# cosmodesi/desilike

Hardware: AMD Instinct MI355X
Metric: log-likelihood evals/sec (full-shape P_ell, 3x40 bins) (higher is better)
Workload: dtype f64; 1 GPU; BASELINE configs[1]: ShapeFit+Kaiser P_ell ell=(0,2,4) x 40 k-bins, dense window 120x1200 (n_kin=400/ell), 120x120 precision, 1024 batched param points per GPU per step; batch_per_gpu=1024, n_params=6, parallelism=walkers x1, collective=none, ranks=1

## Files before the change

desilike_amd/csrc/dl_api.hip:

```cpp
#include <hip/hip_runtime.h>
#include <chrono>
#include <thread>

#include <algorithm>
#include <cmath>
#include <cstdio>
#include <cstdlib>
#include <string>
#include <vector>

#include "../../include/desilike_amd.h"
#include "dl_host.hpp"
#include "dl_kernels.h"
#include "dl_ens_fold.h"
#include "dl_prior.h"
#include "dl_sample_solved.h"
#include "dl_data_batch.h"

static thread_local std::string g_last_error;
void dl_set_last_error(const char* msg) { g_last_error = msg ? msg : ""; }

struct DlWhitenHost {
    int n = 0;
    std::vector<int64_t> col_ptr;
    std::vector<int> row;
    std::vector<double> val;
    std::vector<int> white_row;
    std::vector<double> bias_full;
    void apply(const double* flatdata, double* bias_white, double* bias_wh) const {
        for (int i = 0; i < n; ++i) {
            double bsum = 0., dsum = 0.;
            for (int64_t e = col_ptr[i]; e < col_ptr[i + 1]; ++e) {
                const int j = row[e];
                const double lji = val[e];
                bsum += lji * (bias_full[j] - flatdata[j]);
                dsum += lji * flatdata[j];
            }
            bias_white[white_row[i]] = bsum;
            if (bias_wh) bias_wh[white_row[i]] = -dsum;
        }
    }
};

struct dl_ctx {
    int device = 0;
    int n_params = 0, n_obs = 0, n_data = 0;
    int n_white = 0;
    int N_pad = 0, K_pad = 0, K_live = 0, max_n_t = 0;
    bool any_transform = false;
    bool priors_general = false;
    int n_solved = 0, n_var = 0;
    DlMargDev marg;
    double* tconst_dev = nullptr;
    std::vector<DlObsHost> obs;
    std::vector<int> obs_row0;
    double* arena_dev = nullptr;
    std::vector<DlObsDev> obs_kernarg;
    DlObsDev* obs_array_dev = nullptr;
    double* priors_dev = nullptr;
    int32_t* gemm_counters = nullptr;
    int32_t* step_ready = nullptr;
    double* wt_white_dev = nullptr;
    double* wt_frag_dev = nullptr;
    std::vector<uint8_t> panel_ranges;
    double* bias_white_dev = nullptr;
    double* wt_full_dev = nullptr;
    double* bias_full_dev = nullptr;
    double* wh_dev = nullptr;
    double* bias_wh_dev = nullptr;
    double* flatdata_dev = nullptr;
    int32_t* transform_dev = nullptr;
    bool feat_ok = false;
    int64_t feat_ld = 0;
    std::vector<double*> gfrag_dev;
    std::vector<int> stk_steps;
    bool any_stacked = false;
    double* feat_ws = nullptr;
    int64_t cap = 0;
    double* power_ws = nullptr;
    double* ws_scratch = nullptr;
    int64_t ws_ld = 0;
    double* delta_ws = nullptr;
    double* flat_ws = nullptr;
    double* stencil_ws = nullptr;
    int64_t stage_cap = 0;
    double* theta_stage = nullptr;
    double* out_stage = nullptr;
    int32_t* status_stage = nullptr;
    double* host_stage = nullptr;
    hipStream_t host_stream = nullptr;
    double* host_stage_dev = nullptr;
    uint64_t* host_flag = nullptr;
    uint64_t* host_flag_dev = nullptr;
    uint64_t host_seq = 0;
    hipEvent_t host_event = nullptr;
    double *grad_wtT = nullptr, *grad_zero = nullptr, *grad_delta = nullptr, *grad_y = nullptr, *grad_phys = nullptr;
    int32_t* grad_status = nullptr;
    int64_t grad_cap = 0;
    double *fa_resid = nullptr, *fa_jac = nullptr, *fa_rows = nullptr;
    int64_t fa_cap = 0, fa_slab_rows = 0;
    double *ej_basis = nullptr, *ej_u = nullptr, *ej_c = nullptr, *ej_dc = nullptr, *ej_resid = nullptr, *ej_rows = nullptr;
    int64_t ej_cap = 0;
    double *eg_gt = nullptr, *eg_u = nullptr, *eg_v = nullptr, *eg_q = nullptr, *eg_gb = nullptr;
    double* eg_wt[3] = {nullptr, nullptr, nullptr};
    int eg_ngt = 0;
    int64_t eg_cap = 0;
    double *ss_solved = nullptr, *ss_hessian = nullptr, *ss_loglike = nullptr, *ss_logprior = nullptr;
    int32_t* ss_status = nullptr;
    int64_t ss_cap = 0;
    DlWhitenHost whiten;
    int n_data_batch = 0;
    double* data_bias_dev = nullptr;
    int32_t* data_index_ws = nullptr;
    hipStream_t last_stream = nullptr;
    bool has_last_stream = false;
    hipEvent_t order_event = nullptr;
    bool profile = false;
    static const int NPOOL = 256;
    std::vector<int8_t> prof_phase_of;
    std::vector<hipEvent_t> ev;
    int64_t prof_calls = 0;
    int64_t eval_calls = 0;
    int prof_every = 1;
    bool prof_rotate = false;
    int prof_only = 0;
    std::string last_error;
};

#define DL_HIP_CHECK(ctx, call)                                                                                  \
    do {                                                                                                         \
        hipError_t err__ = (call);                                                                               \
        if (err__ != hipSuccess) {                                                                               \
            std::string msg__ = std::string(#call) + ": " + hipGetErrorString(err__);                            \
            if (ctx) (ctx)->last_error = msg__;                                                                  \
            g_last_error = msg__;                                                                                \
            return 1;                                                                                            \
        }                                                                                                        \
    } while (0)

static int dl_order_streams(dl_ctx* ctx, hipStream_t stream) {
    if (ctx->has_last_stream && ctx->last_stream != stream) {
        if (!ctx->order_event) DL_HIP_CHECK(ctx, hipEventCreateWithFlags(&ctx->order_event, hipEventDisableTiming));
// ... 289 lines not shown
        std::vector<double> tconst((size_t)std::max(ns, 1) * ctx->N_pad, 0.);
        for (int s_ = 0; s_ < ns; ++s_) {
            std::vector<double> dvec(K, 0.);
            for (auto& ob : ctx->obs) {
                const DlObsDev& od = ob.dev;
                double* dst = &dvec[od.col_offset];
                if (ob.marg_sn0 == s_ && od.theory == 4)
                    for (int idx = 0; idx < od.n_in; ++idx) dst[idx] += 1. / od.nd;
                else if (ob.marg_sn0 == s_ && od.ell0 >= 0)
                    for (int i = 0; i < od.n_kin; ++i) dst[(size_t)od.ell0 * od.n_kin + i] += 1. / od.nd;
                for (int c = 0; c < od.n_pass; ++c)
                    if (ob.marg_pass[c] == s_) dst[od.n_in + c] += 1.;
                const auto& snm = cfg->F("obs" + std::to_string(&ob - &ctx->obs[0]) + ".sn_matrix");
                for (int c = 0; c < od.n_sn; ++c)
                    if (ob.marg_sn[c] == s_)
                        for (int idx = 0; idx < od.n_in; ++idx) dst[idx] += snm[(size_t)idx * od.n_sn + c] / od.nd;
            }
            for (int i = 0; i < ctx->n_white; ++i) {
                double sum = 0.;
                const double* wrow = &wt_white[(size_t)i * ctx->K_pad];
                for (int k = 0; k < K; ++k) sum += wrow[k] * dvec[k];
                tconst[(size_t)s_ * ctx->N_pad + i] = sum;
            }
        }
        if (dl_upload(ctx, &ctx->tconst_dev, tconst)) { dl_destroy(ctx); return 1; }
        ctx->marg.tconst = ctx->tconst_dev;
    }
    if (dl_upload(ctx, &ctx->arena_dev, arena.data)) { dl_destroy(ctx); return 1; }
    for (auto& gf : gfrag_host) {
        double* dev = nullptr;
        if (dl_upload(ctx, &dev, gf)) { dl_destroy(ctx); return 1; }
        ctx->gfrag_dev.push_back(dev);
    }
    ctx->obs_kernarg.resize(ctx->n_obs);
    for (int i = 0; i < ctx->n_obs; ++i) { ctx->obs[i].rebase(ctx->arena_dev); ctx->obs_kernarg[i] = ctx->obs[i].dev; }
    if (dl_upload(ctx, &ctx->obs_array_dev, ctx->obs_kernarg)) { dl_destroy(ctx); return 1; }
    {
        size_t nbytes = (16384 / 32 + 8 + 64) * sizeof(int32_t);
        if (hipMalloc((void**)&ctx->gemm_counters, nbytes) != hipSuccess || hipMemset(ctx->gemm_counters, 0, nbytes) != hipSuccess) { dl_fail(ctx, "dl_create: counter allocation failed"); dl_destroy(ctx); return 1; }
        ctx->step_ready = ctx->gemm_counters + (16384 / 32 + 8);
    }
    {
        std::vector<double> frag((size_t)ctx->N_pad * ctx->K_pad);
        const int nks = ctx->K_pad / 4;
        for (int nt = 0; nt < ctx->N_pad / 16; ++nt)
            for (int ks = 0; ks < nks; ++ks)
                for (int lane = 0; lane < 64; ++lane)
                    frag[((size_t)nt * nks + ks) * 64 + lane] = wt_white[(size_t)(16 * nt + (lane & 15)) * ctx->K_pad + 4 * ks + (lane >> 4)];
        if (dl_upload(ctx, &ctx->wt_frag_dev, frag)) { dl_destroy(ctx); return 1; }
    }
    if (dl_upload(ctx, &ctx->priors_dev, priors) || dl_upload(ctx, &ctx->wt_white_dev, wt_white) ||
        dl_upload(ctx, &ctx->bias_white_dev, bias_white) || dl_upload(ctx, &ctx->wt_full_dev, wt_full) || dl_upload(ctx, &ctx->bias_full_dev, bias_full) ||
        dl_upload(ctx, &ctx->wh_dev, wh) || dl_upload(ctx, &ctx->bias_wh_dev, bias_wh) || dl_upload(ctx, &ctx->flatdata_dev, flatdata) ||
        dl_upload(ctx, &ctx->transform_dev, transform)) {
        dl_destroy(ctx);
        return 1;
    }
    if (hipDeviceSynchronize() != hipSuccess) { dl_fail(ctx, "dl_create: hipDeviceSynchronize failed"); dl_destroy(ctx); return 1; }
    *out = ctx;
    return 0;
}

static double* dl_stk_basis_ws(dl_ctx* ctx, int i) {
    const DlObsDev& d = ctx->obs_kernarg[i];
    if (d.eng[0].type != 2 || ctx->power_ws == nullptr) return nullptr;
    const int64_t ldk = (int64_t)d.stk.n_trunks * d.eng[0].widths[d.eng[0].n_layers];
    return ldk <= (int64_t)(1 + ctx->n_var) * ctx->K_pad ? ctx->power_ws : nullptr;
}

void dl_destroy(dl_ctx* ctx) {
    if (!ctx) return;
    (void)hipSetDevice(ctx->device);
    for (double* p : {ctx->grad_wtT, ctx->grad_zero, ctx->grad_delta, ctx->grad_y, ctx->grad_phys}) if (p) (void)hipFree(p);
    for (double* p : {ctx->fa_resid, ctx->fa_jac, ctx->fa_rows}) if (p) (void)hipFree(p);
    for (double* p : {ctx->ej_basis, ctx->ej_u, ctx->ej_c, ctx->ej_dc, ctx->ej_resid, ctx->ej_rows}) if (p) (void)hipFree(p);
    for (double* p : {ctx->eg_gt, ctx->eg_u, ctx->eg_v, ctx->eg_q, ctx->eg_gb, ctx->eg_wt[0], ctx->eg_wt[1], ctx->eg_wt[2]}) if (p) (void)hipFree(p);
    if (ctx->grad_status) (void)hipFree(ctx->grad_status);
    for (double* p : {ctx->ss_solved, ctx->ss_hessian, ctx->ss_loglike, ctx->ss_logprior}) if (p) (void)hipFree(p);
    if (ctx->ss_status) (void)hipFree(ctx->ss_status);
    if (ctx->data_bias_dev) (void)hipFree(ctx->data_bias_dev);
    if (ctx->data_index_ws) (void)hipFree(ctx->data_index_ws);
    void* ptrs[] = {ctx->arena_dev, ctx->priors_dev, ctx->wt_white_dev, ctx->wt_frag_dev, ctx->bias_white_dev, ctx->wt_full_dev, ctx->bias_full_dev, ctx->wh_dev,
                    ctx->bias_wh_dev, ctx->flatdata_dev, ctx->transform_dev, ctx->tconst_dev, ctx->power_ws, ctx->delta_ws, ctx->flat_ws, ctx->stencil_ws, ctx->theta_stage, ctx->out_stage,
                    ctx->status_stage, ctx->gemm_counters, ctx->obs_array_dev, ctx->ws_scratch};
    for (void* p : ptrs) if (p) (void)hipFree(p);
    for (double* p : ctx->gfrag_dev) if (p) (void)hipFree(p);
    for (auto& ob : ctx->obs) if (ob.tns) { dl_tns_destroy(ob.tns); ob.tns = nullptr; }
    if (ctx->feat_ws) (void)hipFree(ctx->feat_ws);
    for (hipEvent_t e : ctx->ev) if (e) (void)hipEventDestroy(e);
    if (ctx->order_event) (void)hipEventDestroy(ctx->order_event);
    if (ctx->host_stage) (void)hipHostFree(ctx->host_stage);
    if (ctx->host_flag) (void)hipHostFree(ctx->host_flag);
    if (ctx->host_event) (void)hipEventDestroy(ctx->host_event);
    if (ctx->host_stream) (void)hipStreamDestroy(ctx->host_stream);
    delete ctx;
}

static bool dl_fisher_emu_in_scope(const dl_ctx* ctx);
static int64_t dl_fisher_emu_per_pass(const dl_ctx* ctx);

int64_t dl_info(const dl_ctx* ctx, const char* key) {
    if (!ctx || !key) return -1;
    std::string k(key);
    if (k == "fisher_analytic_pass") return dl_fisher_emu_in_scope(ctx) ? dl_fisher_emu_per_pass(ctx) : -1;
    if (k == "n_params") return ctx->n_params;
    if (k == "n_data") return ctx->n_data;
    if (k == "n_obs") return ctx->n_obs;
    if (k == "n_in_total") { int64_t t = 0; for (auto& o : ctx->obs) t += o.n_cols(); return t; }
    if (k == "K_pad") return ctx->K_pad;
    if (k == "N_pad") return ctx->N_pad;
    if (k == "n_solved") return ctx->n_solved;
    if (k == "n_data_batch") return ctx->n_data_batch;
    if (k == "device") return ctx->device;
    if (k == "ws_ld") return ctx->ws_ld;
    for (int i = 0; i < ctx->n_obs; ++i) {
        if (k == "n_in_obs" + std::to_string(i)) return ctx->obs[i].dev.n_in;
        if (k == "n_out_obs" + std::to_string(i)) return ctx->obs[i].n_out;
        if (k == "n_ell_obs" + std::to_string(i)) return ctx->obs[i].dev.n_ell;
        if (k == "n_kin_obs" + std::to_string(i)) return ctx->obs[i].dev.n_kin;
        if (k == "moment_form_obs" + std::to_string(i)) return ctx->obs[i].dev.moment_form;
    }
    return -1;
}

static const int64_t DL_CHUNK = 32768;

static int dl_reserve(dl_ctx* ctx, int64_t B) {
    int64_t need = std::min<int64_t>(B, DL_CHUNK);
    if (need <= ctx->cap) return 0;
    need = std::min<int64_t>(std::max<int64_t>(need, 1024), DL_CHUNK);
    if (ctx->cap > 0) DL_HIP_CHECK(ctx, hipDeviceSynchronize());
    for (double** p : {&ctx->power_ws, &ctx->delta_ws, &ctx->flat_ws, &ctx->feat_ws, &ctx->stencil_ws, &ctx->ws_scratch}) if (*p) { (void)hipFree(*p); *p = nullptr; }
    ctx->cap = 0;
    const size_t R = 1 + ctx->n_var;
    DL_HIP_CHECK(ctx, hipMalloc((void**)&ctx->power_ws, (size_t)need * R * ctx->K_pad * sizeof(double)));
    DL_HIP_CHECK(ctx, hipMalloc((void**)&ctx->delta_ws, std::max<size_t>(2 * (size_t)need * R, (size_t)need * R + 16384 + 2048) * ctx->N_pad * sizeof(double)));
    DL_HIP_CHECK(ctx, hipMalloc((void**)&ctx->flat_ws, (size_t)need * ctx->N_pad * sizeof(double)));
    if (ctx->feat_ok) DL_HIP_CHECK(ctx, hipMalloc((void**)&ctx->feat_ws, (size_t)need * ctx->feat_ld * sizeof(double)));
    DL_HIP_CHECK(ctx, hipMalloc((void**)&ctx->stencil_ws, (size_t)need * ctx->n_params * sizeof(double)));
    if (ctx->ws_ld > 0) {
        DL_HIP_CHECK(ctx, hipMalloc((void**)&ctx->ws_scratch, (size_t)need * ctx->ws_ld * sizeof(double)));
        DL_HIP_CHECK(ctx, hipMemset(ctx->ws_scratch, 0, (size_t)need * ctx->ws_ld * sizeof(double)));
        for (int i = 0; i < ctx->n_obs; ++i) {
            if (ctx->obs[i].dev.templ != 5) continue;
            ctx->obs_kernarg[i].coef_w = ctx->ws_scratch + ctx->obs[i].ws_col;
            ctx->obs_kernarg[i].n_band = (int32_t)ctx->ws_ld;
        }
        DL_HIP_CHECK(ctx, hipMemcpy(ctx->obs_array_dev, ctx->obs_kernarg.data(), ctx->obs_kernarg.size() * sizeof(DlObsDev), hipMemcpyHostToDevice));
    }
    DL_HIP_CHECK(ctx, hipMemset(ctx->power_ws, 0, (size_t)need * R * ctx->K_pad * sizeof(double)));
    DL_HIP_CHECK(ctx, hipMemset(ctx->delta_ws, 0, std::max<size_t>(2 * (size_t)need * R, (size_t)need * R + 16384 + 2048) * ctx->N_pad * sizeof(double)));
    DL_HIP_CHECK(ctx, hipMemset(ctx->flat_ws, 0, (size_t)need * ctx->N_pad * sizeof(double)));
    if (ctx->feat_ok) DL_HIP_CHECK(ctx, hipMemset(ctx->feat_ws, 0, (size_t)need * ctx->feat_ld * sizeof(double)));
    DL_HIP_CHECK(ctx, hipMemset(ctx->stencil_ws, 0, (size_t)need * ctx->n_params * sizeof(double)));
    DL_HIP_CHECK(ctx, hipDeviceSynchronize());
    ctx->cap = need;
    return 0;
}

struct DlDataEval {
    const int32_t* index;
    double* out;
};

static int dl_eval_impl(dl_ctx* ctx, const double* theta_dev, int64_t B, double* loglike_dev, double* logprior_dev, double* flattheory_dev, int32_t* status_dev,
                        double* solved_dev, void* hip_stream, int post_mode, double* hessian_dev = nullptr, const DlDataEval* data = nullptr) {
    if (!ctx) { g_last_error = "dl_eval_batch: null context"; return 1; }
    if (B < 0 || (B > 0 && !theta_dev)) return dl_fail(ctx, "dl_eval_batch: invalid batch");
    if (B == 0) return 0;
    hipStream_t stream = (hipStream_t)hip_stream;
    dl_prof_events.start = dl_prof_events.stop = nullptr;
    DL_HIP_CHECK(ctx, hipSetDevice(ctx->device));
    if (dl_order_streams(ctx, stream)) return 1;
    if (dl_reserve(ctx, B)) return 1;
    const int n = ctx->n_data, P = ctx->n_params, R = 1 + ctx->n_var;
    for (int64_t b0 = 0; b0 < B; b0 += DL_CHUNK) {
        int64_t nb = std::min<int64_t>(DL_CHUNK, B - b0);
        const double* th = theta_dev + (size_t)b0 * P;
        bool prof = ctx->profile && b0 == 0 && (ctx->eval_calls % ctx->prof_every == ctx->prof_every / 2);
        hipEvent_t* ev = prof ? &ctx->ev[(size_t)(ctx->prof_calls % dl_ctx::NPOOL) * 6] : nullptr;
        const int64_t pc = ctx->prof_calls;
        const int only = !ctx->prof_rotate ? -1 : ctx->prof_only;
        if (prof) ctx->prof_phase_of[(size_t)(pc % dl_ctx::NPOOL)] = (int8_t)only;
        auto prof_phase = [&](int k) {
            const bool on = ev && k >= 0 && (only < 0 || only == k);
            dl_prof_events.start = on ? ev[2 * k] : nullptr;
            dl_prof_events.stop = on ? ev[2 * k + 1] : nullptr;
        };
        bool need_flat = ctx->any_transform || flattheory_dev != nullptr;
        const bool feat_path = ctx->feat_ok && !need_flat;
        const bool emu_fused_env = !dl_options().no_emu_fused;
        const bool emu_fused = emu_fused_env || ctx->any_stacked;
        const int64_t chi2_max_rows = dl_options().chi2_max_rows;
        const bool chi2_path = !data && !feat_path && !ctx->any_transform && ctx->n_solved == 0 && nb <= chi2_max_rows;
        const int xcd_local = dl_options().xcd_local;
        const bool chi2_fused_env_early = dl_options().chi2_fused;
        const bool chi2_fused_early = chi2_fused_env_early && !ctx->priors_general;
        const int xcd_block = !xcd_local ? 0 : chi2_path ? (chi2_fused_early ? 32 : dl_chi2_gemm_row_tile(nb, ctx->N_pad)) : (xcd_local > 1 && !feat_path && !ctx->any_transform && ctx->n_solved == 0 && ctx->N_pad == 128) ? 64 : 0;
        const bool step_kernel_allowed = dl_options().step_kernel;
        if (step_kernel_allowed && chi2_path && !need_flat && ctx->n_obs == 1 && !ctx->priors_general && ctx->K_pad % 128 == 0 &&
            dl_step_lds_bytes(ctx->obs_kernarg[0], nb, ctx->N_pad) != 0) {
            prof_phase(0);
            dl_launch_step(ctx->obs_kernarg[0], th, P, nb, ctx->power_ws, ctx->K_pad, ctx->wt_white_dev, ctx->K_pad, ctx->bias_white_dev, ctx->delta_ws, ctx->K_pad, ctx->K_live,
                           ctx->gemm_counters, ctx->step_ready, 8, ctx->priors_dev, loglike_dev ? loglike_dev + b0 : nullptr, logprior_dev ? logprior_dev + b0 : nullptr,
                           status_dev ? status_dev + b0 : nullptr, post_mode, stream, ctx->panel_ranges.empty() ? nullptr : ctx->panel_ranges.data());
            prof_phase(-1);
            if (prof) ctx->prof_calls++;
            continue;
        }
        prof_phase(0);
        if (!(feat_path && emu_fused))
            dl_launch_fullshape(ctx->obs_kernarg.data(), ctx->n_obs, th, P, nb, ctx->power_ws, ctx->K_pad, nullptr, 0, stream, feat_path ? ctx->feat_ws : nullptr, ctx->feat_ld,
                                xcd_block, ctx->obs_array_dev);
        prof_phase(1);
        int n_slabs = 1, cps = 0;
        int64_t slab_stride = 0;
        const double* fin_bias = nullptr;
        if (need_flat) {
            dl_launch_window_gemm(ctx->power_ws, (int64_t)R * ctx->K_pad, ctx->wt_full_dev, ctx->K_pad, ctx->bias_full_dev, ctx->flat_ws, ctx->N_pad, nb, ctx->N_pad,
                                  ctx->N_pad, ctx->K_pad, 1, stream);
            if (ctx->any_transform) dl_launch_transform(ctx->flat_ws, ctx->N_pad, ctx->flatdata_dev, ctx->transform_dev, n, nb, stream);
            if (flattheory_dev)
                DL_HIP_CHECK(ctx, hipMemcpy2DAsync(flattheory_dev + (size_t)b0 * n, (size_t)n * sizeof(double), ctx->flat_ws, (size_t)ctx->N_pad * sizeof(double),
                                                   (size_t)n * sizeof(double), (size_t)nb, hipMemcpyDeviceToDevice, stream));
        }
        bool gram_done = false, finalized_in_kernel = false, stacked_rows_done = false;
        const bool gram_epilogue = !dl_options().no_gram_epilogue;
        if (!data && feat_path && emu_fused && gram_epilogue && ctx->n_obs == 1 && ctx->N_pad == 128) {
            DlGramFinalize fin = {ctx->priors_dev, loglike_dev ? loglike_dev + b0 : nullptr, logprior_dev ? logprior_dev + b0 : nullptr, status_dev ? status_dev + b0 : nullptr,
                                  solved_dev ? solved_dev + (size_t)b0 * ctx->n_solved : nullptr, hessian_dev ? hessian_dev + (size_t)b0 * ctx->n_solved * ctx->n_solved : nullptr,
                                  post_mode, false};
            if (ctx->stk_steps[0]) {
                prof_phase(0);
                const bool chains_done = dl_launch_stk_chains(ctx->obs_kernarg[0], th, P, nb, dl_stk_basis_ws(ctx, 0), stream);
                prof_phase(1);
                dl_launch_emulated_stacked(ctx->obs_kernarg[0], th, P, nb, ctx->gfrag_dev[0], ctx->delta_ws, ctx->N_pad, ctx->N_pad, 0, ctx->stk_steps[0], stream, &fin, ctx->bias_white_dev,
                                           &ctx->marg, ctx->n_white, dl_stk_basis_ws(ctx, 0), chains_done);
                gram_done = fin.done;
                stacked_rows_done = !fin.done;
            } else gram_done = dl_launch_emulated_feature_gram(ctx->obs_kernarg[0], th, P, nb, ctx->gfrag_dev[0], ctx->bias_white_dev, ctx->marg, ctx->n_white, ctx->delta_ws, stream, &fin);
            if (gram_done) fin_bias = ctx->bias_white_dev;
            finalized_in_kernel = gram_done && fin.done;
        }
        if (feat_path && !gram_done) {
            for (int i = 0; i < ctx->n_obs; ++i) {
                if (i == 0 && stacked_rows_done) continue;
                if (ctx->stk_steps[i]) dl_launch_emulated_stacked(ctx->obs_kernarg[i], th, P, nb, ctx->gfrag_dev[i], ctx->delta_ws, ctx->N_pad, ctx->N_pad, i > 0, ctx->stk_steps[i], stream, nullptr, nullptr, nullptr, 0, dl_stk_basis_ws(ctx, i));
                else if (emu_fused) dl_launch_emulated_feature(ctx->obs_kernarg[i], th, P, nb, ctx->gfrag_dev[i], ctx->delta_ws, ctx->N_pad, ctx->N_pad, i > 0, stream);
                else dl_launch_feature_gemm(ctx->feat_ws, ctx->feat_ld, ctx->obs_kernarg[i].feat_off, ctx->obs_kernarg[i].nb_pad, R, ctx->gfrag_dev[i], ctx->delta_ws, ctx->N_pad,
                                            ctx->N_pad, nb, i > 0, stream);
            }
            fin_bias = ctx->bias_white_dev;
        }
        int cps_probe = 0;
        const bool chi2_big_allowed = !dl_options().no_chi2_big;
        const bool chi2_big = !data && !feat_path && !ctx->any_transform && ctx->n_solved == 0 && !chi2_path && ctx->K_pad % 32 == 0 && chi2_big_allowed &&
                              dl_gemm_tiled_splits(nb, ctx->N_pad, ctx->K_pad, &cps_probe) == 1;
        int part_tiles = ctx->N_pad / 16;
        const bool chi2_fused_env = dl_options().chi2_fused;
        const bool chi2_fused = chi2_fused_env && !ctx->priors_general;
        if (chi2_path) {
            if (nb > 16384) { prof_phase(-1); return dl_fail(ctx, "dl_eval_batch: DL_CHI2_GEMM_MAX above 16384 rows"); }
            dl_launch_chi2_gemm(ctx->power_ws, ctx->K_pad, ctx->wt_white_dev, ctx->K_pad, ctx->bias_white_dev, ctx->delta_ws, nb, ctx->N_pad, ctx->K_pad,
                                chi2_fused ? ctx->gemm_counters : nullptr, th, P, ctx->priors_dev, loglike_dev ? loglike_dev + b0 : nullptr,
                                logprior_dev ? logprior_dev + b0 : nullptr, status_dev ? status_dev + b0 : nullptr, post_mode, stream,
                                ctx->panel_ranges.empty() ? nullptr : ctx->panel_ranges.data(), ctx->K_live, nullptr, 0, ctx->wt_frag_dev);
        } else if (chi2_big) {
            dl_launch_window_gemm_dma_chi2(ctx->power_ws, ctx->K_pad, ctx->wt_white_dev, ctx->K_pad, ctx->bias_white_dev, ctx->delta_ws, nb, ctx->N_pad, ctx->K_pad, stream, ctx->n_white);
            part_tiles = dl_gemm_dma_chi2_parts(ctx->N_pad);
        } else if (feat_path) {
        } else if (ctx->any_transform) {
            dl_launch_window_gemm(ctx->flat_ws, ctx->N_pad, ctx->wh_dev, ctx->N_pad, ctx->bias_wh_dev, ctx->delta_ws, ctx->N_pad, nb, ctx->N_pad, ctx->N_pad, ctx->N_pad,
                                  1, stream);
        } else {
            n_slabs = dl_gemm_tiled_splits(nb * R, ctx->N_pad, ctx->K_pad, &cps);
            slab_stride = (int64_t)nb * R * ctx->N_pad;
            fin_bias = ctx->bias_white_dev;
            dl_launch_window_gemm_tiled(ctx->power_ws, ctx->K_pad, ctx->wt_white_dev, ctx->K_pad, ctx->delta_ws, slab_stride, ctx->N_pad, nb * R, ctx->N_pad, ctx->K_pad, n_slabs, cps,
                                        stream, ctx->n_white);
        }
        prof_phase(2);
        if (data)
            dl_launch_data_finalize(ctx->delta_ws, ctx->N_pad, ctx->n_white, n_slabs, slab_stride, ctx->data_bias_dev, ctx->N_pad, ctx->n_data_batch,
                                    data->index ? data->index + b0 : nullptr, th, P, ctx->priors_dev, nb, data->out + (size_t)b0 * (data->index ? 1 : ctx->n_data_batch),
                                    status_dev ? status_dev + b0 : nullptr, stream);
        else if (chi2_path && chi2_fused) {
        } else if (finalized_in_kernel) {
        } else if (chi2_path || chi2_big)
            dl_launch_finalize_part(ctx->delta_ws, part_tiles, th, P, ctx->priors_dev, nb, loglike_dev ? loglike_dev + b0 : nullptr, logprior_dev ? logprior_dev + b0 : nullptr,
                                    status_dev ? status_dev + b0 : nullptr, post_mode, stream);
        else if (ctx->n_solved > 0)
            dl_launch_finalize_marg(ctx->delta_ws, ctx->N_pad, ctx->n_white, R, n_slabs, slab_stride, fin_bias, ctx->marg, th, P, ctx->priors_dev, nb, loglike_dev ? loglike_dev + b0 : nullptr,
                                    logprior_dev ? logprior_dev + b0 : nullptr, status_dev ? status_dev + b0 : nullptr,
                                    solved_dev ? solved_dev + (size_t)b0 * ctx->n_solved : nullptr,
                                    hessian_dev ? hessian_dev + (size_t)b0 * ctx->n_solved * ctx->n_solved : nullptr, post_mode, stream, feat_path && ctx->n_obs == 1,
                                    gram_done ? ctx->delta_ws : nullptr);
        else
            dl_launch_finalize(ctx->delta_ws, ctx->N_pad, ctx->n_white, n_slabs, slab_stride, fin_bias, th, P, ctx->priors_dev, nb, loglike_dev ? loglike_dev + b0 : nullptr, logprior_dev ? logprior_dev + b0 : nullptr,
                               status_dev ? status_dev + b0 : nullptr, post_mode, stream);
        prof_phase(-1);
        if (prof) ctx->prof_calls++;
    }
    if (ctx->profile) ctx->eval_calls++;
    DL_HIP_CHECK(ctx, hipGetLastError());
    return 0;
}

int dl_eval_batch(dl_ctx* ctx, const double* theta_dev, int64_t B, double* loglike_dev, double* logprior_dev, double* flattheory_dev, int32_t* status_dev,
                  double* solved_dev, void* hip_stream) {
    return dl_eval_impl(ctx, theta_dev, B, loglike_dev, logprior_dev, flattheory_dev, status_dev, solved_dev, hip_stream, 0);
}

int dl_eval_batch_derived(dl_ctx* ctx, const double* theta_dev, int64_t B, double* loglike_dev, double* logprior_dev, int32_t* status_dev, double* solved_dev,
                          double* hessian_dev, void* hip_stream) {
    if (ctx && hessian_dev && ctx->n_solved == 0) return dl_fail(ctx, "dl_eval_batch_derived: no analytically solved parameter in this likelihood");
    return dl_eval_impl(ctx, theta_dev, B, loglike_dev, logprior_dev, nullptr, status_dev, solved_dev, hip_stream, 0, hessian_dev);
}

int dl_sample_solved(dl_ctx* ctx, const double* theta_dev, int64_t B, int64_t index0, int32_t size, uint64_t seed, double* solved_dev, double* loglike_dev,
                     double* logprior_dev, int32_t* status_dev, void* hip_stream) {
    if (!ctx) { g_last_error = "dl_sample_solved: null context"; return 1; }
    if (ctx->n_solved == 0) return 2;
    if (B < 0 || (B > 0 && !theta_dev) || index0 < 0) return dl_fail(ctx, "dl_sample_solved: invalid batch");
    if (size < 1) return dl_fail(ctx, "dl_sample_solved: size must be at least 1");
    if (B > 0 && (!solved_dev || !loglike_dev || !logprior_dev)) return dl_fail(ctx, "dl_sample_solved: null output");
    if (B == 0) return 0;
    hipStream_t stream = (hipStream_t)hip_stream;
    DL_HIP_CHECK(ctx, hipSetDevice(ctx->device));
    const int ns = ctx->n_solved, P = ctx->n_params;
    const int64_t need = std::min<int64_t>(B, DL_CHUNK);
    if (need > ctx->ss_cap) {
        if (ctx->ss_cap > 0) DL_HIP_CHECK(ctx, hipDeviceSynchronize());
        for (double** p : {&ctx->ss_solved, &ctx->ss_hessian, &ctx->ss_loglike, &ctx->ss_logprior}) if (*p) { (void)hipFree(*p); *p = nullptr; }
        if (ctx->ss_status) { (void)hipFree(ctx->ss_status); ctx->ss_status = nullptr; }
        ctx->ss_cap = 0;
        const int64_t cap = std::min<int64_t>(std::max<int64_t>(need, 1024), DL_CHUNK);
        DL_HIP_CHECK(ctx, hipMalloc((void**)&ctx->ss_solved, (size_t)cap * ns * sizeof(double)));
        DL_HIP_CHECK(ctx, hipMalloc((void**)&ctx->ss_hessian, (size_t)cap * ns * ns * sizeof(double)));
        DL_HIP_CHECK(ctx, hipMalloc((void**)&ctx->ss_loglike, (size_t)cap * sizeof(double)));
        DL_HIP_CHECK(ctx, hipMalloc((void**)&ctx->ss_logprior, (size_t)cap * sizeof(double)));
        DL_HIP_CHECK(ctx, hipMalloc((void**)&ctx->ss_status, (size_t)cap * sizeof(int32_t)));
        DL_HIP_CHECK(ctx, hipDeviceSynchronize());
        ctx->ss_cap = cap;
    }
    for (int64_t b0 = 0; b0 < B; b0 += DL_CHUNK) {
        const int64_t nb = std::min<int64_t>(DL_CHUNK, B - b0);
        if (dl_eval_impl(ctx, theta_dev + (size_t)b0 * P, nb, ctx->ss_loglike, ctx->ss_logprior, nullptr, ctx->ss_status, ctx->ss_solved, hip_stream, 0, ctx->ss_hessian))
            return 1;
        dl_launch_sample_solved(ctx->marg, ctx->ss_hessian, ctx->ss_solved, ctx->ss_loglike, ctx->ss_logprior, ctx->ss_status, nb, index0 + b0, size, seed,
                                solved_dev + (size_t)b0 * size * ns, loglike_dev + (size_t)b0 * size, logprior_dev + (size_t)b0 * size,
                                status_dev ? status_dev + b0 : nullptr, stream);
    }
    DL_HIP_CHECK(ctx, hipGetLastError());
    return 0;
}

int dl_eval_logposterior(dl_ctx* ctx, const double* theta_dev, int64_t B, double* logposterior_dev, int32_t* status_dev, void* hip_stream) {
    if (ctx && B > 0 && !logposterior_dev) return dl_fail(ctx, "dl_eval_logposterior: null output");
    return dl_eval_impl(ctx, theta_dev, B, logposterior_dev, nullptr, nullptr, status_dev, nullptr, hip_stream, 1);
}

static int dl_eval_fisher_impl(dl_ctx* ctx, const double* centers_dev, const double* steps_dev, int64_t B, const int32_t* data_index_dev, double* hessian_dev, double* gradient_dev,
                               double* offset_dev, void* hip_stream) {
    if (!ctx) { g_last_error = "dl_eval_fisher: null context"; return 1; }
    if (B < 0 || (B > 0 && (!centers_dev || !steps_dev))) return dl_fail(ctx, "dl_eval_fisher: invalid argument");
    if (ctx->n_solved > 0) return dl_fail(ctx, "dl_eval_fisher: the context has analytically solved parameters: create it with these parameters varied (the reference does the same, fisher.py:688-695)");
    const int P = ctx->n_params, n = ctx->n_data, S = 1 + 2 * P;
    if (P > 31) return dl_fail(ctx, "dl_eval_fisher: at most 31 varied parameters");
    if (dl_fisher_waves(ctx->n_white, P, nullptr, nullptr) < 1) return dl_fail(ctx, "dl_eval_fisher: too many parameters for the LDS-resident Gram product");
    if (B == 0) return 0;
    hipStream_t stream = (hipStream_t)hip_stream;
// ... 100 lines not shown
static int64_t dl_fisher_emu_per_pass(const dl_ctx* ctx) {
    const int64_t per_centre = std::max<int64_t>((int64_t)(1 + dl_emu_jac_n_xv(ctx->obs_kernarg[0])) * DL_FG_NM * ctx->N_pad, (int64_t)(1 + ctx->n_params) * ctx->N_pad);
    return std::max<int64_t>(64, std::min<int64_t>(2048, ((int64_t)16 << 20) / per_centre) / 64 * 64);
}

static int dl_eval_fisher_analytic_emu(dl_ctx* ctx, const double* centers_dev, int64_t B, double* hessian_dev, double* gradient_dev, double* offset_dev, hipStream_t stream) {
    const int P = ctx->n_params, Np = ctx->N_pad;
    const DlObsDev& o = ctx->obs_kernarg[0];
    const int64_t R = 1 + dl_emu_jac_n_xv(o), K = (int64_t)DL_FG_NM * Np;
    dl_prof_events.start = dl_prof_events.stop = nullptr;
    const int64_t per_pass = dl_fisher_emu_per_pass(ctx);
    const int64_t need = std::min<int64_t>(B, per_pass);
    if (need > ctx->ej_cap) {
        if (ctx->ej_cap > 0) DL_HIP_CHECK(ctx, hipDeviceSynchronize());
        for (double** p : {&ctx->ej_basis, &ctx->ej_u, &ctx->ej_c, &ctx->ej_dc, &ctx->ej_resid, &ctx->ej_rows}) if (*p) { (void)hipFree(*p); *p = nullptr; }
        ctx->ej_cap = 0;
        const int64_t cap = std::min<int64_t>(std::max<int64_t>((need + 63) / 64 * 64, 256), per_pass);
        DL_HIP_CHECK(ctx, hipMalloc((void**)&ctx->ej_basis, (size_t)cap * R * o.nb_pad * sizeof(double)));
        DL_HIP_CHECK(ctx, hipMalloc((void**)&ctx->ej_u, (size_t)cap * R * K * sizeof(double)));
        DL_HIP_CHECK(ctx, hipMalloc((void**)&ctx->ej_c, (size_t)cap * DL_FG_MONO_LD * sizeof(double)));
        DL_HIP_CHECK(ctx, hipMalloc((void**)&ctx->ej_dc, (size_t)cap * P * DL_FG_MONO_LD * sizeof(double)));
        DL_HIP_CHECK(ctx, hipMalloc((void**)&ctx->ej_resid, (size_t)cap * Np * sizeof(double)));
        DL_HIP_CHECK(ctx, hipMalloc((void**)&ctx->ej_rows, (size_t)cap * P * Np * sizeof(double)));
        DL_HIP_CHECK(ctx, hipDeviceSynchronize());
        ctx->ej_cap = cap;
    }
    for (int64_t b0 = 0; b0 < B; b0 += per_pass) {
        const int64_t nc = std::min<int64_t>(per_pass, B - b0);
        const double* th = centers_dev + (size_t)b0 * P;
        dl_launch_emu_jac_tangent(o, th, P, nc, ctx->ej_basis, ctx->ej_c, ctx->ej_dc, stream);
        dl_launch_emu_grad_u(ctx->ej_basis, o.nb_pad, 0, o.nb_pad, ctx->gfrag_dev[0], ctx->ej_u, Np, Np, nc * R, stream);
        dl_launch_emu_jac_rows(o, ctx->ej_u, Np, ctx->ej_c, ctx->ej_dc, ctx->bias_white_dev, P, ctx->n_white, Np, ctx->ej_resid, Np, ctx->ej_rows, Np, nc, stream);
        dl_launch_fisher_rows(ctx->ej_resid, Np, ctx->ej_rows, Np, ctx->n_white, 1, 0, P, nc, hessian_dev ? hessian_dev + (size_t)b0 * P * P : nullptr,
                              gradient_dev ? gradient_dev + (size_t)b0 * P : nullptr, offset_dev ? offset_dev + b0 : nullptr, stream);
    }
    DL_HIP_CHECK(ctx, hipGetLastError());
    return 0;
}

int dl_eval_fisher_analytic(dl_ctx* ctx, const double* centers_dev, int64_t B, double* hessian_dev, double* gradient_dev, double* offset_dev, void* hip_stream) {
    if (!ctx) { g_last_error = "dl_eval_fisher_analytic: null context"; return 1; }
    if (B < 0 || (B > 0 && !centers_dev)) return dl_fail(ctx, "dl_eval_fisher_analytic: invalid argument");
    const int P = ctx->n_params, Np = ctx->N_pad, Kp = ctx->K_pad;
    if (dl_fisher_emu_in_scope(ctx)) {
        if (B == 0) return 0;
        DL_HIP_CHECK(ctx, hipSetDevice(ctx->device));
        if (dl_order_streams(ctx, (hipStream_t)hip_stream)) return 1;
        return dl_eval_fisher_analytic_emu(ctx, centers_dev, B, hessian_dev, gradient_dev, offset_dev, (hipStream_t)hip_stream);
    }
    if (ctx->feat_ok || ctx->any_transform || ctx->n_solved != 0 || P > 31 || !dl_grad_applicable(ctx->obs_kernarg.data(), ctx->n_obs) ||
        dl_fisher_waves(ctx->n_white, P, nullptr, nullptr) < 1) return 2;
    if (B == 0) return 0;
    hipStream_t stream = (hipStream_t)hip_stream;
    dl_prof_events.start = dl_prof_events.stop = nullptr;
    DL_HIP_CHECK(ctx, hipSetDevice(ctx->device));
    if (dl_order_streams(ctx, stream)) return 1;
    const int64_t per_pass = std::max<int64_t>(64, std::min<int64_t>(2048, ((int64_t)16 << 20) / ((int64_t)(1 + P) * std::max(Kp, Np))) / 64 * 64);
    const int64_t need = std::min<int64_t>(B, per_pass);
    if (dl_reserve(ctx, need)) return 1;
    if (need > ctx->fa_cap) {
        if (ctx->fa_cap > 0) DL_HIP_CHECK(ctx, hipDeviceSynchronize());
        for (double** p : {&ctx->fa_resid, &ctx->fa_jac, &ctx->fa_rows}) if (*p) { (void)hipFree(*p); *p = nullptr; }
        ctx->fa_cap = 0;
        const int64_t cap = std::min<int64_t>(std::max<int64_t>((need + 63) / 64 * 64, 256), per_pass);
        const size_t rows = ((size_t)cap * P + 63) / 64 * 64, slab_rows = std::max<size_t>(2 * rows, rows + 16384 + 2048);
        DL_HIP_CHECK(ctx, hipMalloc((void**)&ctx->fa_resid, (size_t)cap * Np * sizeof(double)));
        DL_HIP_CHECK(ctx, hipMalloc((void**)&ctx->fa_jac, rows * Kp * sizeof(double)));
        DL_HIP_CHECK(ctx, hipMalloc((void**)&ctx->fa_rows, slab_rows * Np * sizeof(double)));
        DL_HIP_CHECK(ctx, hipMemset(ctx->fa_jac, 0, rows * Kp * sizeof(double)));
        DL_HIP_CHECK(ctx, hipDeviceSynchronize());
        ctx->fa_cap = cap;
        ctx->fa_slab_rows = (int64_t)slab_rows;
    }
    const int xcd_local = dl_options().xcd_local;
    for (int64_t b0 = 0; b0 < B; b0 += per_pass) {
        int cps = 0;
        const int64_t nr = std::min<int64_t>(per_pass, B - b0) * P;
        if ((int64_t)dl_gemm_tiled_splits(nr, Np, Kp, &cps) * nr > ctx->fa_slab_rows) return dl_fail(ctx, "dl_eval_fisher_analytic: the split-K slabs of the window product exceed their buffer");
    }
    for (int64_t b0 = 0; b0 < B; b0 += per_pass) {
        const int64_t nc = std::min<int64_t>(per_pass, B - b0), nr = nc * P;
        const double* th = centers_dev + (size_t)b0 * P;
        dl_launch_fullshape(ctx->obs_kernarg.data(), ctx->n_obs, th, P, nc, ctx->power_ws, Kp, nullptr, 0, stream, nullptr, 0, xcd_local ? dl_chi2_gemm_row_tile(nc, Np) : 0, ctx->obs_array_dev);
        dl_launch_chi2_gemm(ctx->power_ws, Kp, ctx->wt_white_dev, Kp, ctx->bias_white_dev, ctx->delta_ws, nc, Np, Kp, nullptr, th, P, ctx->priors_dev, nullptr, nullptr, nullptr, 1, stream,
                            ctx->panel_ranges.empty() ? nullptr : ctx->panel_ranges.data(), ctx->K_live, ctx->fa_resid, Np, ctx->wt_frag_dev);
        dl_launch_fullshape_jac(ctx->obs_kernarg.data(), ctx->n_obs, ctx->obs_array_dev, th, P, nc, ctx->K_live, Kp, ctx->fa_jac, Kp, stream);
        int cps = 0;
        const int n_slabs = dl_gemm_tiled_splits(nr, Np, Kp, &cps);
        const int64_t slab_stride = nr * (int64_t)Np;
        dl_launch_window_gemm_tiled(ctx->fa_jac, Kp, ctx->wt_white_dev, Kp, ctx->fa_rows, slab_stride, Np, nr, Np, Kp, n_slabs, cps, stream, ctx->n_white);
        dl_launch_fisher_rows(ctx->fa_resid, Np, ctx->fa_rows, Np, ctx->n_white, n_slabs, slab_stride, P, nc, hessian_dev ? hessian_dev + (size_t)b0 * P * P : nullptr,
                              gradient_dev ? gradient_dev + (size_t)b0 * P : nullptr, offset_dev ? offset_dev + b0 : nullptr, stream);
    }
    DL_HIP_CHECK(ctx, hipGetLastError());
    return 0;
}

static int dl_eval_logposterior_grad_emu(dl_ctx* ctx, const double* theta_dev, int64_t B, double* logposterior_dev, double* grad_dev, int32_t* status_dev, hipStream_t stream) {
    const int64_t per_pass = 2048;
    const int P = ctx->n_params, Np = ctx->N_pad;
    const DlObsDev& o = ctx->obs_kernarg[0];
    dl_prof_events.start = dl_prof_events.stop = nullptr;
    const int64_t K = (int64_t)DL_FG_NM * Np;
    if (!ctx->eg_gt) {
        const int Kp = ctx->K_pad, ngt = (o.n_basis + 127) / 128 * 128;
        std::vector<double> w((size_t)Np * Kp), gt((size_t)ngt * K, 0.);
        DL_HIP_CHECK(ctx, hipMemcpy(w.data(), ctx->wt_white_dev, w.size() * sizeof(double), hipMemcpyDeviceToHost));
        for (int h = 0; h < o.n_basis; ++h)
            for (int m = 0; m < DL_FG_NM; ++m)
                for (int j = 0; j < Np; ++j) gt[(size_t)h * K + (size_t)m * Np + j] = w[(size_t)j * Kp + o.col_offset + (size_t)h * DL_N_MONO + m];
        DL_HIP_CHECK(ctx, hipMalloc((void**)&ctx->eg_gt, gt.size() * sizeof(double)));
        DL_HIP_CHECK(ctx, hipMemcpy(ctx->eg_gt, gt.data(), gt.size() * sizeof(double), hipMemcpyHostToDevice));
        ctx->eg_ngt = ngt;
        for (int ie = 0; ie < 3; ++ie) {
            const DlObsDev::Engine& e = o.eng[ie];
            if (e.type != 0) continue;
            size_t n = 0, nt = 0;
            for (int l = 0; l < e.n_layers; ++l) { n += (size_t)e.widths[l] * e.widths[l + 1] + e.widths[l + 1]; nt += (size_t)e.widths[l] * e.widths[l + 1]; }
            std::vector<double> wh(n), wt(nt);
            DL_HIP_CHECK(ctx, hipMemcpy(wh.data(), e.weights, n * sizeof(double), hipMemcpyDeviceToHost));
            size_t off = 0, offt = 0;
            for (int l = 0; l < e.n_layers; ++l) {
                const int nin = e.widths[l], nout = e.widths[l + 1];
                for (int i = 0; i < nin; ++i)
                    for (int q = 0; q < nout; ++q) wt[offt + (size_t)q * nin + i] = wh[off + (size_t)i * nout + q];
                off += (size_t)nin * nout + nout;
                offt += (size_t)nin * nout;
            }
            DL_HIP_CHECK(ctx, hipMalloc((void**)&ctx->eg_wt[ie], nt * sizeof(double)));
            DL_HIP_CHECK(ctx, hipMemcpy(ctx->eg_wt[ie], wt.data(), nt * sizeof(double), hipMemcpyHostToDevice));
        }
    }
    const int64_t need = std::min<int64_t>(B, per_pass);
    if (dl_reserve(ctx, need)) return 1;
    if (need > ctx->eg_cap || !ctx->grad_status) {
        DL_HIP_CHECK(ctx, hipDeviceSynchronize());
        for (double** p : {&ctx->eg_u, &ctx->eg_v, &ctx->eg_q, &ctx->eg_gb}) if (*p) { (void)hipFree(*p); *p = nullptr; }
        if (ctx->grad_status) { (void)hipFree(ctx->grad_status); ctx->grad_status = nullptr; }
        ctx->eg_cap = 0;
        ctx->grad_cap = 0;
        const int64_t cap = std::max<int64_t>((need + 63) / 64 * 64, 256);
        DL_HIP_CHECK(ctx, hipMalloc((void**)&ctx->eg_u, (size_t)cap * K * sizeof(double)));
        DL_HIP_CHECK(ctx, hipMalloc((void**)&ctx->eg_v, (size_t)cap * K * sizeof(double)));
        DL_HIP_CHECK(ctx, hipMalloc((void**)&ctx->eg_q, (size_t)cap * (1 + ctx->n_var) * DL_N_MONO * sizeof(double)));
        DL_HIP_CHECK(ctx, hipMalloc((void**)&ctx->eg_gb, std::max<size_t>(2 * (size_t)cap, (size_t)cap + 16384 + 2048) * ctx->eg_ngt * sizeof(double)));
        DL_HIP_CHECK(ctx, hipMalloc((void**)&ctx->grad_status, (size_t)cap * sizeof(int32_t)));
        DL_HIP_CHECK(ctx, hipMemset(ctx->eg_v, 0, (size_t)cap * K * sizeof(double)));
        DL_HIP_CHECK(ctx, hipDeviceSynchronize());
        ctx->eg_cap = cap;
    }
    for (int64_t b0 = 0; b0 < B; b0 += per_pass) {
        const int64_t nb = std::min<int64_t>(per_pass, B - b0);
        const double* th = theta_dev + (size_t)b0 * P;
        int32_t* st = status_dev ? status_dev + b0 : ctx->grad_status;
        dl_launch_fullshape(ctx->obs_kernarg.data(), 1, th, P, nb, ctx->power_ws, ctx->K_pad, nullptr, 0, stream, ctx->feat_ws, ctx->feat_ld, 0, nullptr);
        dl_launch_emu_grad_u(ctx->feat_ws, ctx->feat_ld, o.feat_off, o.nb_pad, ctx->gfrag_dev[0], ctx->eg_u, Np, Np, nb, stream);
        dl_launch_emu_grad_adjoint(ctx->feat_ws, ctx->feat_ld, o.feat_off, o.nb_pad, ctx->n_var, ctx->eg_u, Np, Np, ctx->bias_white_dev, ctx->marg, th, P, ctx->priors_dev,
                                   logposterior_dev + b0, st, ctx->eg_v, ctx->eg_q, nb, stream);
        int cps = 0;
        const int n_slabs = dl_gemm_tiled_splits(nb, ctx->eg_ngt, (int)K, &cps);
        const int64_t slab_stride = nb * (int64_t)ctx->eg_ngt;
        dl_launch_window_gemm_tiled(ctx->eg_v, K, ctx->eg_gt, K, ctx->eg_gb, slab_stride, ctx->eg_ngt, nb, ctx->eg_ngt, (int)K, n_slabs, cps, stream, 0);
        dl_launch_emu_grad_backprop(o, th, P, ctx->priors_dev, ctx->eg_gb, ctx->eg_ngt, n_slabs, slab_stride, ctx->eg_q, st, ctx->eg_wt, grad_dev + (size_t)b0 * P, nb, stream);
    }
    DL_HIP_CHECK(ctx, hipGetLastError());
    return 0;
}

int dl_eval_logposterior_grad(dl_ctx* ctx, const double* theta_dev, int64_t B, double* logposterior_dev, double* grad_dev, int32_t* status_dev, void* hip_stream) {
    if (!ctx) { g_last_error = "dl_eval_logposterior_grad: null context"; return 1; }
    if (B < 0 || (B > 0 && (!theta_dev || !logposterior_dev || !grad_dev))) return dl_fail(ctx, "dl_eval_logposterior_grad: invalid argument");
    const bool emu = ctx->feat_ok && !ctx->any_transform && !ctx->priors_general && ctx->n_obs == 1 && !ctx->any_stacked &&
                     dl_emu_grad_applicable(ctx->obs_kernarg[0], ctx->N_pad, ctx->n_solved);
    if (emu) {
        if (B == 0) return 0;
        DL_HIP_CHECK(ctx, hipSetDevice(ctx->device));
        if (dl_order_streams(ctx, (hipStream_t)hip_stream)) return 1;
        return dl_eval_logposterior_grad_emu(ctx, theta_dev, B, logposterior_dev, grad_dev, status_dev, (hipStream_t)hip_stream);
    }
    if (ctx->feat_ok || ctx->any_transform || ctx->n_solved != 0 || ctx->priors_general || !dl_grad_applicable(ctx->obs_kernarg.data(), ctx->n_obs)) return 2;
    if (B == 0) return 0;
    hipStream_t stream = (hipStream_t)hip_stream;
    dl_prof_events.start = dl_prof_events.stop = nullptr;
    DL_HIP_CHECK(ctx, hipSetDevice(ctx->device));
    if (dl_order_streams(ctx, stream)) return 1;
    const int64_t per_pass = 2048;
    if (dl_reserve(ctx, std::min<int64_t>(B, per_pass))) return 1;
    const int P = ctx->n_params, Np = ctx->N_pad, Kp = ctx->K_pad;
    if (!ctx->grad_wtT) {
        std::vector<double> w((size_t)Np * Kp), wt((size_t)Kp * Np);
        DL_HIP_CHECK(ctx, hipMemcpy(w.data(), ctx->wt_white_dev, w.size() * sizeof(double), hipMemcpyDeviceToHost));
        for (int j = 0; j < Np; ++j) for (int k = 0; k < Kp; ++k) wt[(size_t)k * Np + j] = -w[(size_t)j * Kp + k];
        DL_HIP_CHECK(ctx, hipMalloc((void**)&ctx->grad_wtT, wt.size() * sizeof(double)));
        DL_HIP_CHECK(ctx, hipMemcpy(ctx->grad_wtT, wt.data(), wt.size() * sizeof(double), hipMemcpyHostToDevice));
        DL_HIP_CHECK(ctx, hipDeviceSynchronize());
    }
    const int64_t need = std::min<int64_t>(B, per_pass);
    if (need > ctx->grad_cap) {
        if (ctx->grad_cap > 0) DL_HIP_CHECK(ctx, hipDeviceSynchronize());
        for (double** p : {&ctx->grad_delta, &ctx->grad_y, &ctx->grad_phys}) if (*p) { (void)hipFree(*p); *p = nullptr; }
        if (ctx->grad_status) { (void)hipFree(ctx->grad_status); ctx->grad_status = nullptr; }
        ctx->grad_cap = 0;
        const int64_t cap = std::max<int64_t>((need + 63) / 64 * 64, 256);
        DL_HIP_CHECK(ctx, hipMalloc((void**)&ctx->grad_delta, (size_t)cap * Np * sizeof(double)));
        DL_HIP_CHECK(ctx, hipMalloc((void**)&ctx->grad_y, (size_t)cap * Kp * sizeof(double)));
        DL_HIP_CHECK(ctx, hipMalloc((void**)&ctx->grad_phys, (size_t)cap * ctx->n_obs * 8 * sizeof(double)));
        DL_HIP_CHECK(ctx, hipMalloc((void**)&ctx->grad_status, (size_t)cap * sizeof(int32_t)));
        DL_HIP_CHECK(ctx, hipMemset(ctx->grad_delta, 0, (size_t)cap * Np * sizeof(double)));
        DL_HIP_CHECK(ctx, hipDeviceSynchronize());
        ctx->grad_cap = cap;
    }
    const int xcd_local = dl_options().xcd_local;
    for (int64_t b0 = 0; b0 < B; b0 += per_pass) {
        const int64_t nb = std::min<int64_t>(per_pass, B - b0);
        const double* th = theta_dev + (size_t)b0 * P;
        int32_t* st = status_dev ? status_dev + b0 : ctx->grad_status;
        dl_launch_fullshape(ctx->obs_kernarg.data(), ctx->n_obs, th, P, nb, ctx->power_ws, ctx->K_pad, nullptr, 0, stream, nullptr, 0, xcd_local ? dl_chi2_gemm_row_tile(nb, Np) : 0, ctx->obs_array_dev,
                            false);
        dl_launch_chi2_gemm(ctx->power_ws, Kp, ctx->wt_white_dev, Kp, ctx->bias_white_dev, ctx->delta_ws, nb, Np, Kp, nullptr, th, P, ctx->priors_dev, nullptr, nullptr, nullptr, 1, stream,
                            ctx->panel_ranges.empty() ? nullptr : ctx->panel_ranges.data(), ctx->K_live, ctx->grad_delta, Np, ctx->wt_frag_dev);
        dl_launch_finalize_part(ctx->delta_ws, Np / 16, th, P, ctx->priors_dev, nb, logposterior_dev + b0, nullptr, st, 1, stream);
        dl_launch_window_gemm_tiled(ctx->grad_delta, Np, ctx->grad_wtT, Np, ctx->grad_y, 0, Kp, nb, Kp, Np, 1, Np / 16, stream, 0);
        dl_launch_fullshape_grad(ctx->obs_kernarg.data(), ctx->n_obs, ctx->obs_array_dev, th, P, nb, ctx->grad_y, Kp, ctx->grad_phys, ctx->priors_dev, st, grad_dev + (size_t)b0 * P, stream);
    }
    DL_HIP_CHECK(ctx, hipGetLastError());
    return 0;
}

int dl_eval_theory(dl_ctx* ctx, const double* theta_dev, int64_t B, int32_t iobs, double* power_dev, double* tables_dev, void* hip_stream) {
    if (!ctx) { g_last_error = "dl_eval_theory: null context"; return 1; }
    if (iobs < 0 || iobs >= ctx->n_obs) return dl_fail(ctx, "dl_eval_theory: observable index out of range");
    if (B < 0 || (B > 0 && (!theta_dev || !power_dev))) return dl_fail(ctx, "dl_eval_theory: invalid argument");
    if (B == 0) return 0;
    hipStream_t stream = (hipStream_t)hip_stream;
    DL_HIP_CHECK(ctx, hipSetDevice(ctx->device));
    const bool ws = ctx->obs_kernarg[iobs].templ == 5;
    if (ws && dl_reserve(ctx, B)) return 1;
    DlObsDev tmp = ctx->obs_kernarg[iobs];
    tmp.col_offset = 0;
    tmp.n_pass = 0;
    tmp.n_var = 0;
    for (int c = 0; c < DL_N_VPARS; ++c) tmp.vp_slot[c] = -1;
    for (int c = 0; c < DL_MAX_EFT; ++c) tmp.marg_ct_slot[c][0] = tmp.marg_ct_slot[c][1] = -1;
    if (dl_order_streams(ctx, stream)) return 1;
    for (int64_t b0 = 0, step = ws ? ctx->cap : B; b0 < B; b0 += step)
        dl_launch_fullshape(&tmp, 1, theta_dev + (size_t)b0 * ctx->n_params, ctx->n_params, std::min(step, B - b0), power_dev + (size_t)b0 * tmp.n_in, tmp.n_in,
                            tables_dev ? tables_dev + (size_t)b0 * 3 * tmp.n_in : nullptr, 3 * (int64_t)tmp.n_in, stream);
    DL_HIP_CHECK(ctx, hipGetLastError());
    return 0;
}

int dl_eval_tns_tables(dl_ctx* ctx, const double* theta_dev, int64_t B, int32_t iobs, double* tables_dev, void* hip_stream) {
    if (!ctx) { g_last_error = "dl_eval_tns_tables: null context"; return 1; }
    if (iobs < 0 || iobs >= ctx->n_obs) return dl_fail(ctx, "dl_eval_tns_tables: observable index out of range");
    if (ctx->obs[iobs].dev.theory != 4) return dl_fail(ctx, "dl_eval_tns_tables: the observable's theory is not the TNS model");
    if (B < 0 || (B > 0 && (!theta_dev || !tables_dev))) return dl_fail(ctx, "dl_eval_tns_tables: invalid argument");
    if (B == 0) return 0;
    hipStream_t stream = (hipStream_t)hip_stream;
    DL_HIP_CHECK(ctx, hipSetDevice(ctx->device));
    if (dl_order_streams(ctx, stream)) return 1;
    if (dl_tns_tables(ctx->obs_kernarg[iobs], theta_dev, ctx->n_params, B, tables_dev, stream)) return dl_fail(ctx, std::string("dl_eval_tns_tables: ") + dl_last_error(nullptr));
    DL_HIP_CHECK(ctx, hipGetLastError());
    return 0;
}

static int dl_stage_reserve(dl_ctx* ctx, int64_t B) {
    if (!ctx->host_stream) DL_HIP_CHECK(ctx, hipStreamCreateWithFlags(&ctx->host_stream, hipStreamNonBlocking));
    if (B <= ctx->stage_cap) return 0;
    for (void* p : {(void*)ctx->theta_stage, (void*)ctx->out_stage}) if (p) (void)hipFree(p);
    if (ctx->host_stage) (void)hipHostFree(ctx->host_stage);
    ctx->theta_stage = ctx->out_stage = ctx->host_stage = nullptr; ctx->status_stage = nullptr; ctx->stage_cap = 0;
    int64_t cap = std::max<int64_t>(B, 64);
    DL_HIP_CHECK(ctx, hipMalloc((void**)&ctx->theta_stage, (size_t)cap * ctx->n_params * sizeof(double)));
    DL_HIP_CHECK(ctx, hipMalloc((void**)&ctx->out_stage, (size_t)cap * 3 * sizeof(double)));
    DL_HIP_CHECK(ctx, hipHostMalloc((void**)&ctx->host_stage, (size_t)cap * (ctx->n_params + 3) * sizeof(double), hipHostMallocMapped));
    DL_HIP_CHECK(ctx, hipHostGetDevicePointer((void**)&ctx->host_stage_dev, ctx->host_stage, 0));
    if (!ctx->host_flag) {
        DL_HIP_CHECK(ctx, hipHostMalloc((void**)&ctx->host_flag, 64, hipHostMallocMapped));
        DL_HIP_CHECK(ctx, hipHostGetDevicePointer((void**)&ctx->host_flag_dev, ctx->host_flag, 0));
        *ctx->host_flag = 0;
        DL_HIP_CHECK(ctx, hipEventCreateWithFlags(&ctx->host_event, hipEventDisableTiming));
    }
    ctx->stage_cap = cap;
    return 0;
}

__global__ void dl_host_flag_kernel(uint64_t* flag, uint64_t seq) {
    __threadfence_system();
    __hip_atomic_store(flag, seq, __ATOMIC_RELEASE, __HIP_MEMORY_SCOPE_SYSTEM);
}

static int dl_host_mode() { return dl_options().host_mode >= 0 ? dl_options().host_mode : 3; }

static int dl_eval_host_impl(dl_ctx* ctx, const double* theta, int64_t B, double* loglike, double* logprior, double* flattheory, int32_t* status, double* solved,
                             double* logposterior) {
    DL_HIP_CHECK(ctx, hipSetDevice(ctx->device));
    if (dl_stage_reserve(ctx, B)) return 1;
    hipStream_t stream = ctx->host_stream;
    const int P = ctx->n_params;
    int mode = dl_host_mode();
    if (mode == 3 && ctx->host_seq && (ctx->host_seq & 7) == 0) (void)hipStreamQuery(stream);
    double *flat_dev = nullptr, *solved_dev = nullptr;
// ... 114 lines not shown
int dl_profile_enable(dl_ctx* ctx, int enable) {
    if (!ctx) { g_last_error = "dl_profile_enable: null context"; return 1; }
    DL_HIP_CHECK(ctx, hipSetDevice(ctx->device));
    if ((enable & 0xffff) && ctx->ev.empty()) {
        ctx->ev.assign((size_t)dl_ctx::NPOOL * 6, nullptr);
        for (auto& e : ctx->ev) DL_HIP_CHECK(ctx, hipEventCreate(&e));
    }
    ctx->prof_phase_of.assign(dl_ctx::NPOOL, -1);
    ctx->prof_rotate = (enable & (1 << 16)) != 0;
    ctx->prof_only = (enable >> 17) & 3;
    if (ctx->prof_only > 2) ctx->prof_only = 0;
    enable &= 0xffff;
    ctx->profile = enable != 0;
    ctx->prof_every = enable > 1 ? enable : 1;
    ctx->prof_calls = 0;
    ctx->eval_calls = 0;
    return 0;
}

int dl_profile_read(dl_ctx* ctx, double* ms, int32_t n) {
    if (!ctx || !ms || n < 4) return dl_fail(ctx, "dl_profile_read: need room for 4 values");
    if (ctx->ev.empty() || ctx->prof_calls == 0) return dl_fail(ctx, "dl_profile_read: no profiled call recorded");
    int64_t ncalls = std::min<int64_t>(ctx->prof_calls, dl_ctx::NPOOL);
    std::vector<double> samples[4];
    for (int64_t c = 0; c < ncalls; ++c) {
        hipEvent_t* ev = &ctx->ev[(size_t)c * 6];
        const int only = ctx->prof_phase_of.empty() ? -1 : ctx->prof_phase_of[(size_t)c];
        int first = -1, last = -1;
        for (int k = 0; k < 3; ++k) {
            if (only >= 0 && only != k) continue;
            (void)hipEventSynchronize(ev[2 * k + 1]);
            float t = 0;
            if (hipEventElapsedTime(&t, ev[2 * k], ev[2 * k + 1]) != hipSuccess) { (void)hipGetLastError(); continue; }
            if (first < 0) first = k;
            last = k;
            samples[k].push_back(t);
        }
        float t = 0;
        if (only < 0 && first >= 0 && hipEventElapsedTime(&t, ev[2 * first], ev[2 * last + 1]) == hipSuccess) samples[3].push_back(t);
        else (void)hipGetLastError();
    }
    for (int i = 0; i < 4; ++i) if (samples[i].empty()) samples[i].push_back(0.);
    if (n >= 9) for (int i = 0; i < 3; ++i) ms[6 + i] = (samples[i].size() == 1 && samples[i][0] == 0.) ? 0. : (double)samples[i].size();
    for (int i = 0; i < 4; ++i) {
        std::sort(samples[i].begin(), samples[i].end());
        const size_t m = samples[i].size();
        ms[i] = (m & 1) ? samples[i][m / 2] : 0.5 * (samples[i][m / 2 - 1] + samples[i][m / 2]);
    }
    if (n >= 5) ms[4] = 0.;
    if (n >= 6) ms[5] = (double)ncalls;
    return 0;
}

}

static bool dl_fold_applicable(const dl_ctx* ctx, int64_t B) {
    const int64_t chi2_max_rows = dl_options().chi2_max_rows;
    if (ctx->feat_ok || ctx->any_transform || ctx->n_solved != 0 || B > chi2_max_rows || B > DL_CHUNK || ctx->n_params > 32) return false;
    for (auto& ob : ctx->obs) {
        const DlObsDev& oh = ob.dev;
        const bool generic = !oh.uniform_knots || !(oh.toeplitz || oh.fixed_spline);
        if (oh.theory >= 2 || generic || oh.n_ct > 0 || oh.n_sn > 0 || (oh.n_ell <= 3) != (ctx->obs[0].dev.n_ell <= 3)) return false;
    }
    return ctx->n_obs >= 1 && ctx->n_obs <= 8;
}

int dl_internal_fold_info(dl_ctx* ctx, int64_t B, int* n_tiles, const double** priors) {
    if (!ctx || !n_tiles || !priors || B <= 0) return 1;
    if (!dl_fold_applicable(ctx, B)) return 2;
    *n_tiles = ctx->N_pad / 16;
    *priors = ctx->priors_dev;
    return 0;
}

int dl_internal_eval_fold(dl_ctx* ctx, const DlEnsFold& fold, int64_t B, double* part_out, hipStream_t stream) {
    if (!ctx || !part_out || B <= 0) return 1;
    if (!dl_fold_applicable(ctx, B)) return 2;
    dl_prof_events.start = dl_prof_events.stop = nullptr;
    DL_HIP_CHECK(ctx, hipSetDevice(ctx->device));
    if (dl_order_streams(ctx, stream)) return 1;
    if (dl_reserve(ctx, B)) return 1;
    const int xcd_local = dl_options().xcd_local;
    if (!dl_launch_fullshape_ens(ctx->obs_kernarg.data(), ctx->n_obs, ctx->obs_array_dev, fold, B, ctx->power_ws, ctx->K_pad, xcd_local ? dl_chi2_gemm_row_tile(B, ctx->N_pad) : 0, stream)) return 2;
    dl_launch_chi2_gemm(ctx->power_ws, ctx->K_pad, ctx->wt_white_dev, ctx->K_pad, ctx->bias_white_dev, part_out, B, ctx->N_pad, ctx->K_pad, nullptr, nullptr, ctx->n_params,
                        ctx->priors_dev, nullptr, nullptr, nullptr, 1, stream, ctx->panel_ranges.empty() ? nullptr : ctx->panel_ranges.data(), ctx->K_live, nullptr, 0, ctx->wt_frag_dev);
    DL_HIP_CHECK(ctx, hipGetLastError());
    return 0;
}

int dl_internal_eval_partials(dl_ctx* ctx, const double* theta_dev, int64_t B, const double** part, int* n_tiles, const double** priors, hipStream_t stream) {
    if (!ctx || !theta_dev || !part || !n_tiles || !priors || B <= 0) return 1;
    const int64_t chi2_max_rows = dl_options().chi2_max_rows;
    if (ctx->feat_ok || ctx->any_transform || ctx->n_solved != 0 || B > chi2_max_rows || B > DL_CHUNK) return 2;
    for (auto& ob : ctx->obs) if (ob.dev.theory == 3) return 2;
    dl_prof_events.start = dl_prof_events.stop = nullptr;
    DL_HIP_CHECK(ctx, hipSetDevice(ctx->device));
    if (dl_order_streams(ctx, stream)) return 1;
    if (dl_reserve(ctx, B)) return 1;
    const int xcd_local = dl_options().xcd_local;
    dl_launch_fullshape(ctx->obs_kernarg.data(), ctx->n_obs, theta_dev, ctx->n_params, B, ctx->power_ws, ctx->K_pad, nullptr, 0, stream, nullptr, 0, xcd_local ? dl_chi2_gemm_row_tile(B, ctx->N_pad) : 0, ctx->obs_array_dev);
    dl_launch_chi2_gemm(ctx->power_ws, ctx->K_pad, ctx->wt_white_dev, ctx->K_pad, ctx->bias_white_dev, ctx->delta_ws, B, ctx->N_pad, ctx->K_pad, nullptr, theta_dev, ctx->n_params,
                        ctx->priors_dev, nullptr, nullptr, nullptr, 1, stream, ctx->panel_ranges.empty() ? nullptr : ctx->panel_ranges.data(), ctx->K_live, nullptr, 0, ctx->wt_frag_dev);
    *part = ctx->delta_ws;
    *n_tiles = ctx->N_pad / 16;
    *priors = ctx->priors_dev;
    DL_HIP_CHECK(ctx, hipGetLastError());
    return 0;
}
```

desilike_amd/csrc/dl_chi2_gemm.h:

```cpp
#pragma once
#include "dl_scalar_prefetch.h"
#include <hip/hip_runtime.h>
#include <stdint.h>

typedef double dl_cg_double2 __attribute__((ext_vector_type(2)));
typedef double dl_cg_double4 __attribute__((ext_vector_type(4)));

#define DL_CG_M 32
#define DL_CG_N 16
#define DL_CG_KP 128
#define DL_CG_LD (DL_CG_KP + 2)
#define DL_CG_ROWS (DL_CG_M + DL_CG_N)
#ifndef DL_CG_WAVES
#define DL_CG_WAVES 16
#endif
#define DL_CG_VPT (DL_CG_ROWS / DL_CG_WAVES)
#define DL_CG_NBUF 3
#define DL_CG_LDS_BYTES (DL_CG_NBUF * DL_CG_ROWS * DL_CG_LD * 8)

struct DlChi2Fin {
    int32_t* counters;
    const double* theta;
    const double* priors;
    double* loglike;
    double* logprior;
    int32_t* status;
    int32_t n_params, post_mode;
    unsigned long long* stamps;
    int32_t* ready;
};

#define DL_CG_MAX_TILES 32
struct DlChi2Panels {
    uint32_t range[DL_CG_MAX_TILES];
};

#define DL_CG_STAMP(slot, fn) if (fin.stamps != nullptr && tid == 0) fin.stamps[(size_t)blockIdx.x * 8 + (slot)] = fn();
template <int MT, bool RESID>
__device__ __forceinline__ void dl_chi2_gemm_finish(dl_cg_double4 acc0, dl_cg_double4 acc1, double bj, double* __restrict__ part, int M, int n_tiles, const DlChi2Fin& fin,
                                                    double* __restrict__ resid, int64_t ldr, double* lds, int mb, int nt, double fin_lp, int fin_nan) {
    const int tid = threadIdx.x, lane = tid & 63, wave = __builtin_amdgcn_readfirstlane(tid >> 6);
    const int r16 = lane & 15, g = lane >> 4;
    constexpr int MTILES = MT / 16;
    const int m0 = mb * MT, n0 = nt * DL_CG_N;
    DL_CG_STAMP(2, __builtin_amdgcn_s_memtime)
    __syncthreads();
    double* red = lds;
#pragma unroll
    for (int r = 0; r < 4; ++r) { red[((wave * 2 + 0) * 4 + r) * 64 + lane] = acc0[r]; if (MTILES > 1) red[((wave * 2 + 1) * 4 + r) * 64 + lane] = acc1[r]; }
    __syncthreads();
    if (wave < 4 * MTILES) {
        const int t = wave % MTILES, r = wave / MTILES;
        double v = bj;
#pragma unroll
        for (int w = 0; w < DL_CG_WAVES; ++w) v += red[((w * 2 + t) * 4 + r) * 64 + lane];
        if (RESID) { const int rrow = m0 + 16 * t + g + 4 * r; if (rrow < M) resid[(size_t)rrow * ldr + n0 + r16] = v; }
        double sq = v * v;
        sq += __shfl_xor(sq, 1, 64);
        sq += __shfl_xor(sq, 2, 64);
        sq += __shfl_xor(sq, 4, 64);
        sq += __shfl_xor(sq, 8, 64);
        const int row = m0 + 16 * t + g + 4 * r;
        if (r16 == 0 && row < M) __hip_atomic_store(part + (size_t)row * n_tiles + nt, sq, __ATOMIC_RELAXED, __HIP_MEMORY_SCOPE_AGENT);
    }
    DL_CG_STAMP(3, __builtin_amdgcn_s_memtime) DL_CG_STAMP(4, __builtin_amdgcn_s_memtime) DL_CG_STAMP(5, __builtin_amdgcn_s_memtime) DL_CG_STAMP(7, __builtin_amdgcn_s_memrealtime)
    if (fin.counters == nullptr) return;
    __asm__ volatile("s_waitcnt vmcnt(0)" : : : "memory");
    __syncthreads();
    if (wave != 0) return;
    int done = 0;
    if (lane == 0) done = __hip_atomic_fetch_add(fin.counters + mb, 1, __ATOMIC_RELAXED, __HIP_MEMORY_SCOPE_AGENT);
    done = __builtin_amdgcn_readfirstlane(done);
    if (done != n_tiles - 1) return;
    if (lane == 0) __hip_atomic_store(fin.counters + mb, 0, __ATOMIC_RELAXED, __HIP_MEMORY_SCOPE_AGENT);
    if (lane == 0 && fin.ready != nullptr) __hip_atomic_store(fin.ready + mb, 0, __ATOMIC_RELAXED, __HIP_MEMORY_SCOPE_AGENT);
    const int row = m0 + lane;
    if (lane < MT && row < M) {
        double chi2 = 0.;
        for (int t = 0; t < n_tiles; ++t) chi2 += __hip_atomic_load(part + (size_t)row * n_tiles + t, __ATOMIC_RELAXED, __HIP_MEMORY_SCOPE_AGENT);
        const double inf = __builtin_huge_val();
        const double lp = fin_lp, ll = -0.5 * chi2;
        int st = 0;
        if (fin_nan) st = 3;
        else if (lp == -inf) st = 1;
        else if (!(ll == ll) || ll == inf || ll == -inf) st = 2;
        if (fin.loglike) fin.loglike[row] = fin.post_mode ? (st == 0 ? ll + lp : -inf) : ll;
        if (fin.logprior) fin.logprior[row] = lp;
        if (fin.status) fin.status[row] = st;
    }
}

template <bool DO_LOAD, bool DO_MMA, int MT, bool RESID, class Wait>
__device__ __forceinline__ void dl_chi2_gemm_tile(const double* __restrict__ A, int64_t lda, const double* __restrict__ Wt, int64_t ldw, const double* __restrict__ bias,
                                                  double* __restrict__ part, int M, int K_pad, int n_tiles, const DlChi2Fin& fin, const DlChi2Panels& panels, int k_live,
                                                  double* __restrict__ resid, int64_t ldr, double* lds, int mb, int nt, Wait&& wait) {
    const int tid = threadIdx.x, lane = tid & 63, wave = __builtin_amdgcn_readfirstlane(tid >> 6);
    const int r16 = lane & 15, g = lane >> 4;
    constexpr int ROWS = MT + DL_CG_N, VPT = ROWS / DL_CG_WAVES, MTILES = MT / 16;
    const int m0 = mb * MT, n0 = nt * DL_CG_N;
    if (m0 >= M) return;
    DL_CG_STAMP(0, __builtin_amdgcn_s_memtime) DL_CG_STAMP(6, __builtin_amdgcn_s_memrealtime)
    int p_lo = 0, p_hi = K_pad / DL_CG_KP;
    const uint32_t range = panels.range[nt < DL_CG_MAX_TILES ? nt : 0];
    if (nt < DL_CG_MAX_TILES && (range >> 8) != 0) { p_lo = (int)(range & 0xffu); p_hi = (int)(range >> 8); }
    const char* src[VPT];
#pragma unroll
    for (int i = 0; i < VPT; ++i) {
        int row = wave + DL_CG_WAVES * i;
        const double* base;
        if (row < MT) { int ar = m0 + row; if (ar > M - 1) ar = M - 1; base = A + (size_t)ar * lda; }
        else base = Wt + (size_t)(n0 + row - MT) * ldw;
        src[i] = reinterpret_cast<const char*>(base) + 16 * lane + (size_t)p_lo * (DL_CG_KP * 8);
    }
    const double bj = bias[n0 + r16];
    const int n_panels = p_hi - p_lo;
    constexpr int BUF = ROWS * DL_CG_LD, NJ = DL_CG_KP / 4 / DL_CG_WAVES;
#define DL_CG_DMA(p)                                                                                                                 \
    {   const size_t off = (size_t)(p) * (DL_CG_KP * 8);                                                                             \
        double* dst = lds + ((p) % DL_CG_NBUF) * BUF + wave * DL_CG_LD;                                                              \
        _Pragma("unroll") for (int i = 0; i < VPT; ++i)                                                                               \
            __builtin_amdgcn_global_load_lds((const __attribute__((address_space(1))) void*)(src[i] + off),                          \
                                             (__attribute__((address_space(3))) void*)(dst + DL_CG_WAVES * i * DL_CG_LD), 16, 0, 0); }
    dl_cg_double4 acc0 = {0., 0., 0., 0.}, acc1 = {0., 0., 0., 0.};
    const double* la = lds + r16 * DL_CG_LD + g;
    wait();
    if (DO_LOAD) { DL_CG_DMA(0) if (n_panels > 1) { DL_CG_DMA(1) } }
    double fin_lp = 0.;
    int fin_nan = 0;
    if (fin.counters != nullptr && wave == 0 && lane < MT && m0 + lane < M) {
        const double inf = __builtin_huge_val();
        for (int p = 0; p < fin.n_params; ++p) {
            double x = fin.theta[(size_t)(m0 + lane) * fin.n_params + p];
            const double* pr = fin.priors + 5 * p;
            if (x != x) fin_nan = 1;
            bool isin = (pr[1] <= x) && (x <= pr[2]);
            double v = 0.;
            if (pr[0] == 1.) { double t = x - pr[3]; v = -0.5 * (t * t) / (pr[4] * pr[4]); }
            fin_lp += isin ? v : -inf;
        }
    }
    if (n_panels > 1) __asm__ volatile("s_waitcnt vmcnt(%0)" : : "n"(VPT) : "memory");
    else __asm__ volatile("s_waitcnt vmcnt(0)" : : : "memory");
    __builtin_amdgcn_s_barrier();
    DL_CG_STAMP(1, __builtin_amdgcn_s_memtime)
#define DL_CG_MULTIPLY(p)                                                                                                            \
    {   const double* lb = la + ((p) % DL_CG_NBUF) * BUF;                                                                            \
        double a0[NJ], a1[NJ], bb[NJ];                                                                                               \
        _Pragma("unroll") for (int j = 0; j < NJ; ++j) {                                                                             \
            const int ks = wave + DL_CG_WAVES * j; a0[j] = lb[4 * ks]; a1[j] = MTILES > 1 ? lb[16 * DL_CG_LD + 4 * ks] : 0.; bb[j] = lb[MT * DL_CG_LD + 4 * ks]; } \
        if (DO_MMA) { _Pragma("unroll") for (int j = 0; j < NJ; ++j) {                                                               \
            acc0 = __builtin_amdgcn_mfma_f64_16x16x4f64(a0[j], bb[j], acc0, 0, 0, 0);                                                \
            if (MTILES > 1) acc1 = __builtin_amdgcn_mfma_f64_16x16x4f64(a1[j], bb[j], acc1, 0, 0, 0); } } }
#define DL_CG_MULTIPLY_LIM(p, lim)                                                                                                   \
    {   const double* lb = la + ((p) % DL_CG_NBUF) * BUF;                                                                            \
        _Pragma("unroll") for (int j = 0; j < NJ; ++j) {                                                                             \
            const int ks = wave + DL_CG_WAVES * j;                                                                                   \
            if (DO_MMA && ks < (lim)) {                                                                                              \
                const double a0 = lb[4 * ks], a1 = MTILES > 1 ? lb[16 * DL_CG_LD + 4 * ks] : 0., bb = lb[MT * DL_CG_LD + 4 * ks];    \
                acc0 = __builtin_amdgcn_mfma_f64_16x16x4f64(a0, bb, acc0, 0, 0, 0);                                                  \
                if (MTILES > 1) acc1 = __builtin_amdgcn_mfma_f64_16x16x4f64(a1, bb, acc1, 0, 0, 0); } } }
    int p = 0;
    for (; p + 2 < n_panels; ++p) {
        if (DO_LOAD) { DL_CG_DMA(p + 2) }
        DL_CG_MULTIPLY(p)
        __asm__ volatile("s_waitcnt vmcnt(%0) lgkmcnt(0)" : : "n"(VPT) : "memory");
        __builtin_amdgcn_s_barrier();
    }
    if (p + 1 < n_panels) {
        DL_CG_MULTIPLY(p)
        __asm__ volatile("s_waitcnt vmcnt(0) lgkmcnt(0)" : : : "memory");
        __builtin_amdgcn_s_barrier();
        ++p;
    }
    {
        int lim = (k_live - (p_lo + p) * DL_CG_KP + 3) / 4;
        lim = lim < 0 ? 0 : (lim > DL_CG_KP / 4 ? DL_CG_KP / 4 : lim);
        DL_CG_MULTIPLY_LIM(p, lim)
    }
#undef DL_CG_MULTIPLY
#undef DL_CG_MULTIPLY_LIM
#undef DL_CG_DMA
    dl_chi2_gemm_finish<MT, RESID>(acc0, acc1, bj, part, M, n_tiles, fin, resid, ldr, lds, mb, nt, fin_lp, fin_nan);
}

#define DL_CG_PMAX 12
template <bool DO_LOAD, bool DO_MMA, int MT, bool RESID>
__device__ __forceinline__ void dl_chi2_gemm_tile_bf(const double* __restrict__ A, int64_t lda, const double* __restrict__ wfrag, const double* __restrict__ bias,
                                                     double* __restrict__ part, int M, int K_pad, int n_tiles, const DlChi2Fin& fin, const DlChi2Panels& panels, int k_live,
                                                     double* __restrict__ resid, int64_t ldr, double* lds, int mb, int nt) {
    const int tid = threadIdx.x, lane = tid & 63, wave = __builtin_amdgcn_readfirstlane(tid >> 6);
    const int r16 = lane & 15, g = lane >> 4;
    constexpr int VPT = MT / DL_CG_WAVES, MTILES = MT / 16;
    static_assert(VPT >= 1 && DL_CG_KP / 4 / DL_CG_WAVES == 2, "16 waves: one or two row pieces and two k-steps per wave and panel");
    const int m0 = mb * MT, n0 = nt * DL_CG_N;
    if (m0 >= M) return;
    DL_CG_STAMP(0, __builtin_amdgcn_s_memtime) DL_CG_STAMP(6, __builtin_amdgcn_s_memrealtime)
    int p_lo = 0, p_hi = K_pad / DL_CG_KP;
    const uint32_t range = panels.range[nt < DL_CG_MAX_TILES ? nt : 0];
    if (nt < DL_CG_MAX_TILES && (range >> 8) != 0) { p_lo = (int)(range & 0xffu); p_hi = (int)(range >> 8); }
    const int n_panels = p_hi - p_lo;
    const double* bsrc = wfrag + ((size_t)nt * (K_pad / 4) + (size_t)p_lo * (DL_CG_KP / 4) + wave) * 64 + lane;
    double bq[DL_CG_PMAX][2];
#pragma unroll
    for (int q = 0; q < DL_CG_PMAX; ++q) {
        const double* bp = bsrc + (size_t)(q < n_panels ? q : n_panels - 1) * (DL_CG_KP / 4 * 64);
        bq[q][0] = bp[0]; bq[q][1] = bp[DL_CG_WAVES * 64];
    }
    const char* src[VPT];
#pragma unroll
    for (int i = 0; i < VPT; ++i) {
        int ar = m0 + wave + DL_CG_WAVES * i; if (ar > M - 1) ar = M - 1;
        src[i] = reinterpret_cast<const char*>(A + (size_t)ar * lda) + 16 * lane + (size_t)p_lo * (DL_CG_KP * 8);
    }
    const double bj = bias[n0 + r16];
    constexpr int BUF = MT * DL_CG_LD;
#define DL_CG_DMA_A(p)                                                                                                               \
    {   const size_t off = (size_t)(p) * (DL_CG_KP * 8);                                                                             \
        double* dst = lds + ((p) % DL_CG_NBUF) * BUF + wave * DL_CG_LD;                                                              \
        _Pragma("unroll") for (int i = 0; i < VPT; ++i)                                                                               \
            __builtin_amdgcn_global_load_lds((const __attribute__((address_space(1))) void*)(src[i] + off),                          \
                                             (__attribute__((address_space(3))) void*)(dst + DL_CG_WAVES * i * DL_CG_LD), 16, 0, 0); }
    dl_cg_double4 acc0 = {0., 0., 0., 0.}, acc1 = {0., 0., 0., 0.};
    const double* la = lds + r16 * DL_CG_LD + g;
    if (DO_LOAD) { DL_CG_DMA_A(0) if (n_panels > 1) { DL_CG_DMA_A(1) } }
    double fin_lp = 0.;
    int fin_nan = 0;
    if (fin.counters != nullptr && wave == 0 && lane < MT && m0 + lane < M) {
        const double inf = __builtin_huge_val();
        for (int p = 0; p < fin.n_params; ++p) {
            double x = fin.theta[(size_t)(m0 + lane) * fin.n_params + p];
            const double* pr = fin.priors + 5 * p;
            if (x != x) fin_nan = 1;
            bool isin = (pr[1] <= x) && (x <= pr[2]);
            double v = 0.;
            if (pr[0] == 1.) { double t = x - pr[3]; v = -0.5 * (t * t) / (pr[4] * pr[4]); }
            fin_lp += isin ? v : -inf;
        }
    }
    if (n_panels > 1) __asm__ volatile("s_waitcnt vmcnt(%0)" : : "n"(VPT) : "memory");
    else __asm__ volatile("s_waitcnt vmcnt(0)" : : : "memory");
    __builtin_amdgcn_s_barrier();
    DL_CG_STAMP(1, __builtin_amdgcn_s_memtime)
    int lim = (k_live - (p_lo + n_panels - 1) * DL_CG_KP + 3) / 4;
    lim = lim < 0 ? 0 : (lim > DL_CG_KP / 4 ? DL_CG_KP / 4 : lim);
#pragma unroll
    for (int p = 0; p < DL_CG_PMAX; ++p) {
        if (p < n_panels) {
        if (DO_LOAD && p + 2 < n_panels) { DL_CG_DMA_A(p + 2) }
        const double* lb = la + (p % DL_CG_NBUF) * BUF;
        const int klim = p + 1 < n_panels ? DL_CG_KP / 4 : lim;
#pragma unroll
        for (int j = 0; j < 2; ++j) {
            const int ks = wave + DL_CG_WAVES * j;
            if (DO_MMA && ks < klim) {
                const double a0 = lb[4 * ks], a1 = MTILES > 1 ? lb[16 * DL_CG_LD + 4 * ks] : 0.;
                acc0 = __builtin_amdgcn_mfma_f64_16x16x4f64(a0, bq[p][j], acc0, 0, 0, 0);
                if (MTILES > 1) acc1 = __builtin_amdgcn_mfma_f64_16x16x4f64(a1, bq[p][j], acc1, 0, 0, 0);
            }
        }
        if (p + 1 < n_panels) {
            if (p + 2 < n_panels) __asm__ volatile("s_waitcnt vmcnt(%0) lgkmcnt(0)" : : "n"(VPT) : "memory");
            else __asm__ volatile("s_waitcnt vmcnt(0) lgkmcnt(0)" : : : "memory");
            __builtin_amdgcn_s_barrier();
        }
        }
    }
#undef DL_CG_DMA_A
    dl_chi2_gemm_finish<MT, RESID>(acc0, acc1, bj, part, M, n_tiles, fin, resid, ldr, lds, mb, nt, fin_lp, fin_nan);
}

template <bool DO_LOAD, bool DO_MMA, int MT = DL_CG_M, bool RESID = false>
__global__ __launch_bounds__(64 * DL_CG_WAVES) void dl_chi2_gemm_bf_kernel(const double* __restrict__ A, int64_t lda, const double* __restrict__ wfrag, const double* __restrict__ bias,
                                                              double* __restrict__ part, int M, int K_pad, int n_tiles, DlChi2Fin fin, DlChi2Panels panels, int k_live,
                                                              double* __restrict__ resid, int64_t ldr) {
    extern __shared__ __attribute__((aligned(16))) double lds[];
    dl_kernarg_prefetch<256>();
    const int L = blockIdx.x;
    const int xcd = L & 7, rest = L >> 3;
    const int nt = rest % n_tiles, mb = xcd + 8 * (rest / n_tiles);
    dl_chi2_gemm_tile_bf<DO_LOAD, DO_MMA, MT, RESID>(A, lda, wfrag, bias, part, M, K_pad, n_tiles, fin, panels, k_live, resid, ldr, lds, mb, nt);
}

template <bool DO_LOAD, bool DO_MMA, int MT = DL_CG_M, bool RESID = false>
__global__ __launch_bounds__(64 * DL_CG_WAVES) void dl_chi2_gemm_kernel(const double* __restrict__ A, int64_t lda, const double* __restrict__ Wt, int64_t ldw,
                                                           const double* __restrict__ bias, double* __restrict__ part, int M, int K_pad, int n_tiles, DlChi2Fin fin,
                                                           DlChi2Panels panels, int k_live, double* __restrict__ resid, int64_t ldr) {
    extern __shared__ __attribute__((aligned(16))) double lds[];
    dl_kernarg_prefetch<256>();
    const int L = blockIdx.x;
    const int xcd = L & 7, rest = L >> 3;
    const int nt = rest % n_tiles, mb = xcd + 8 * (rest / n_tiles);
    dl_chi2_gemm_tile<DO_LOAD, DO_MMA, MT, RESID>(A, lda, Wt, ldw, bias, part, M, K_pad, n_tiles, fin, panels, k_live, resid, ldr, lds, mb, nt, []() {});
}
```

desilike_amd/csrc/dl_kernels.h:

```cpp
#pragma once
#include <hip/hip_runtime.h>
#include <hip/hip_ext.h>
#include <stdint.h>

#include "dl_fullshape.h"

struct DlProfEvents { hipEvent_t start = nullptr, stop = nullptr; };
extern thread_local DlProfEvents dl_prof_events;
#define DL_LAUNCH(kernel, grid, block, shm, stream, ...)                                                                                       \
    do {                                                                                                                                       \
        if (dl_prof_events.start) hipExtLaunchKernelGGL(kernel, grid, block, shm, stream, dl_prof_events.start, dl_prof_events.stop, 0, __VA_ARGS__); \
        else hipLaunchKernelGGL(kernel, grid, block, shm, stream, __VA_ARGS__);                                                                \
    } while (0)

struct DlOptions {
    bool no_merged_theory, no_emu_batch, no_fused_solve, no_gram_plain, no_scaled_row0, ef_no_early_theta, fm_no_lane_solve;
    bool chi2_bfrag;
    bool no_stk_split;
    int stk_overlap;
    bool ens_global, ens_force_comm, ens_no_defer, ens_no_fold, ens_stamps, ens_fold_stamps;
    bool no_emu_fused, no_gram_epilogue, step_kernel, chi2_fused, no_chi2_big;
    bool fs_no_moments;
    bool fs_mu_prio;
    int xcd_local;
    long long chi2_max_rows;
    int cg_mt;
    int host_mode;
};
const DlOptions& dl_options();

#define DL_ST_OK 0
#define DL_ST_OUT_OF_PRIOR 1
#define DL_ST_NONFINITE 2
#define DL_ST_NAN_INPUT 3

void dl_launch_fullshape(const DlObsDev* obs_host, int n_obs, const double* theta, int n_params, int64_t B, double* power, int64_t ld_power, double* tables,
                         int64_t ld_tables, hipStream_t stream, double* feat = nullptr, int64_t feat_ld = 0, int xcd_block = 0,
                         const DlObsDev* obs_dev = nullptr,
                         bool moments = true);
void dl_launch_window_gemm(const double* A, int64_t lda, const double* Wt, int64_t ldw, const double* bias, double* C, int64_t ldc, int64_t M, int N_valid, int N_pad,
                           int K_pad, int bias_period, hipStream_t stream);

#define DL_MARG_NJ 8
struct DlMargDev {
    int32_t n_s, n_marg;
    int32_t is_marg[DL_MAX_SOLVED];
    int32_t var_slot[DL_MAX_SOLVED];
    double x0[DL_MAX_SOLVED], loc[DL_MAX_SOLVED], prec[DL_MAX_SOLVED];
    const double* tconst;
};
void dl_launch_finalize_marg(const double* dtilde, int64_t ld, int n, int rows_per_point, int n_slabs, int64_t slab_stride, const double* bias, const DlMargDev& mg,
                             const double* theta, int n_params, const double* priors, int64_t B, double* loglike, double* logprior, int32_t* status, double* solved,
                             double* hessian , int post_mode, hipStream_t stream, bool xcd_tile16 = false,
                             const double* gram = nullptr);
void dl_launch_transform(double* flat, int64_t ld, const double* data, const int32_t* transform, int n, int64_t B, hipStream_t stream);
int dl_gemm_tiled_splits(int64_t M, int N_pad, int K_pad, int* chunks_per_split);
void dl_launch_window_gemm_tiled(const double* A, int64_t lda, const double* Wt, int64_t ldw, double* slabs, int64_t slab_stride, int64_t ldc, int64_t M, int N_pad, int K_pad,
                                 int n_splits, int chunks_per_split, hipStream_t stream, int n_live = 0);
void dl_launch_finalize(const double* dtilde, int64_t ld, int n, int n_slabs, int64_t slab_stride, const double* bias, const double* theta, int n_params,
                        const double* priors, int64_t B, double* loglike, double* logprior, int32_t* status, int post_mode, hipStream_t stream);
int dl_chi2_gemm_row_tile(int64_t M, int N_pad);
void dl_launch_chi2_gemm(const double* A, int64_t lda, const double* Wt, int64_t ldw, const double* bias, double* part, int64_t M, int N_pad, int K_pad, int32_t* counters,
                         const double* theta, int n_params, const double* priors, double* loglike, double* logprior, int32_t* status, int post_mode, hipStream_t stream,
                         const uint8_t* panel_ranges = nullptr, int k_live = 0, double* resid = nullptr, int64_t ldr = 0, const double* wfrag = nullptr);
void dl_launch_finalize_part(const double* part, int n_tiles, const double* theta, int n_params, const double* priors, int64_t B, double* loglike, double* logprior,
                             int32_t* status, int post_mode, hipStream_t stream);
#ifndef DL_FG_NM
#define DL_FG_NM 19
#define DL_FG_MONO_LD 20
#endif
void dl_launch_feature_gemm(const double* feat, int64_t feat_ld, int64_t feat_off, int nb_pad, int R, const double* gfrag, double* out, int64_t ldo, int N_pad, int64_t B,
                            int accumulate, hipStream_t stream);
int dl_gemm_dma_chi2_parts(int N_pad);
void dl_launch_window_gemm_dma_chi2(const double* A, int64_t lda, const double* Wt, int64_t ldw, const double* bias, double* part, int64_t M, int N_pad, int K_pad, hipStream_t stream, int n_live = 0);
void dl_launch_emulated_feature(const DlObsDev& obs, const double* theta, int n_params, int64_t B, const double* gfrag, double* out, int64_t ldo, int N_pad, int accumulate,
                                hipStream_t stream);
size_t dl_step_lds_bytes(const DlObsDev& obs, int64_t B, int N_pad);
void dl_launch_step(const DlObsDev& obs, const double* theta, int n_params, int64_t B, double* power, int64_t ld_power, const double* Wt, int64_t ldw, const double* bias,
                    double* part, int K_pad, int k_live, int32_t* counters, int32_t* ready, int32_t target, const double* priors, double* loglike, double* logprior, int32_t* status,
                    int post_mode, hipStream_t stream, const uint8_t* panel_ranges);
bool dl_emulated_stacked_ok(const DlObsDev& obs);
struct DlGramFinalize;
void dl_launch_emulated_stacked(const DlObsDev& obs, const double* theta, int n_params, int64_t B, const double* gfrag, double* out, int64_t ldo, int N_pad, int accumulate,
                                int steps_per_block, hipStream_t stream, DlGramFinalize* fin = nullptr, const double* bias = nullptr, const DlMargDev* mg = nullptr, int n_valid = 0,
                                double* basis_ws = nullptr, bool chains_done = false);
bool dl_launch_stk_chains(const DlObsDev& obs, const double* theta, int n_params, int64_t B, double* basis_ws, hipStream_t stream);
struct DlGramFinalize {
    const double* priors;
    double *loglike, *logprior;
    int32_t* status;
    double *solved, *hessian;
    int post_mode;
    bool done;
};
bool dl_launch_emulated_feature_gram(const DlObsDev& obs, const double* theta, int n_params, int64_t B, const double* gfrag, const double* bias, const DlMargDev& mg, int n_valid,
                                     double* gram, hipStream_t stream, DlGramFinalize* fin = nullptr);
void dl_launch_fisher_stencil(const double* centers, const double* steps, int P, int64_t B, double* theta, hipStream_t stream);
int dl_fisher_waves(int n, int P, size_t* shm_bytes, int* chunk);
void dl_launch_fisher(const double* rows, int64_t ld, int n, int n_slabs, int64_t slab_stride, const double* bias, const double* steps, int P, int64_t B, double* hessian,
                      double* gradient, double* offset, hipStream_t stream,
                      const int32_t* data_index = nullptr, int64_t ldb = 0);
struct dl_ctx;
int dl_internal_eval_partials(dl_ctx* ctx, const double* theta_dev, int64_t B, const double** part, int* n_tiles, const double** priors, hipStream_t stream);
struct DlEnsFold;
int dl_internal_fold_info(dl_ctx* ctx, int64_t B, int* n_tiles, const double** priors);
int dl_internal_eval_fold(dl_ctx* ctx, const DlEnsFold& fold, int64_t B, double* part_out, hipStream_t stream);
bool dl_launch_fullshape_ens(const DlObsDev* obs_host, int n_obs, const DlObsDev* obs_dev, const DlEnsFold& f, int64_t B, double* power, int64_t ld_power, int xcd_block, hipStream_t stream);
bool dl_grad_applicable(const DlObsDev* obs_host, int n_obs);
void dl_launch_fullshape_grad(const DlObsDev* obs_host, int n_obs, const DlObsDev* obs_dev, const double* theta, int n_params, int64_t B, const double* Y, int64_t ldy, double* gphys,
                              const double* priors, const int32_t* status, double* grad, hipStream_t stream);
void dl_launch_fullshape_jac(const DlObsDev* obs_host, int n_obs, const DlObsDev* obs_dev, const double* theta, int n_params, int64_t B, int k_live, int k_pad, double* jac, int64_t ldj,
                             hipStream_t stream);
void dl_launch_fisher_rows(const double* resid, int64_t ldr, const double* drows, int64_t ld, int n, int n_slabs, int64_t slab_stride, int P, int64_t B, double* hessian,
                           double* gradient, double* offset, hipStream_t stream);
bool dl_emu_grad_applicable(const DlObsDev& obs, int N_pad, int n_solved);
void dl_launch_emu_grad_u(const double* feat, int64_t feat_ld, int64_t feat_off, int nb_pad, const double* gfrag, double* U, int64_t ldu, int N_pad, int64_t B, hipStream_t stream);
void dl_launch_emu_grad_adjoint(const double* feat, int64_t feat_ld, int64_t feat_off, int nb_pad, int n_var, const double* U, int64_t ldu, int N_pad, const double* bias,
                                const DlMargDev& mg, const double* theta, int n_params, const double* priors, double* logpost, int32_t* status, double* V, double* Q,
                                int64_t B, hipStream_t stream);
void dl_launch_emu_grad_backprop(const DlObsDev& obs, const double* theta, int n_params, const double* priors, const double* gb, int64_t ldg, int n_slabs, int64_t slab_stride,
                                 const double* Q, const int32_t* status, const double* const* wT , double* grad, int64_t B,
                                 hipStream_t stream);
bool dl_emu_jac_applicable(const DlObsDev& obs, int N_pad, int n_params);
int dl_emu_jac_n_xv(const DlObsDev& obs);
void dl_launch_emu_jac_tangent(const DlObsDev& obs, const double* theta, int n_params, int64_t B, double* basis_rows, double* cmono, double* dmono, hipStream_t stream);
void dl_launch_emu_jac_rows(const DlObsDev& obs, const double* U, int64_t ldu, const double* cmono, const double* dmono, const double* bias, int n_params, int n_live, int N_pad,
                            double* resid, int64_t ldr, double* rows, int64_t ld, int64_t B, hipStream_t stream);
void dl_set_last_error(const char* msg);
```

desilike_amd/csrc/dl_kernels.hip:

```cpp
#include <hip/hip_runtime.h>

#include <algorithm>
#include <cstdio>
#include <cstdlib>
#include <cstring>
#include <vector>

#include "dl_fullshape.h"
#include "dl_wigglesplit.h"
#include <mutex>
#include "dl_kernels.h"
#include "dl_tns.h"
#include "dl_emu_batch.h"
#include "dl_emu_stacked.h"
#include "dl_emu_stacked_ov.h"
#include "dl_emu_stacked_split.h"
#include "dl_finalize_part.h"
#include "dl_marg_solve.h"
#include "dl_scalar_prefetch.h"
#include "dl_ens_fold.h"
#include "dl_fullshape_grad.h"
#include "dl_fullshape_jac.h"

thread_local DlProfEvents dl_prof_events;

__device__ __forceinline__ void dl_obs_prefetch(const void* p) {
    if (__builtin_amdgcn_readfirstlane(threadIdx.x) >= 64) return;
    dl_scalar_prefetch<0, (offsetof(DlObsDev, ct_in) + 63) / 64 * 64, offsetof(DlObsDev, coef_w) / 64 * 64, (sizeof(DlObsDev) + 63) / 64 * 64>(p);
}

static DlOptions g_options;
static std::once_flag g_options_once;
static void dl_options_read() {
    auto on = [](const char* name) { return std::getenv(name) != nullptr; };
    DlOptions& o = g_options;
    o.no_merged_theory = on("DL_NO_MERGED_THEORY"); o.no_emu_batch = on("DL_NO_EMU_BATCH"); o.no_fused_solve = on("DL_NO_FUSED_SOLVE"); o.no_gram_plain = on("DL_NO_GRAM_PLAIN");
    o.no_scaled_row0 = on("DL_NO_SCALED_ROW0"); o.ef_no_early_theta = on("DL_EF_NO_EARLY_THETA"); o.fm_no_lane_solve = on("DL_FM_NO_LANE_SOLVE");
    o.no_stk_split = on("DL_NO_STK_SPLIT");
    o.stk_overlap = std::getenv("DL_STK_OVERLAP") ? atoi(std::getenv("DL_STK_OVERLAP")) : 0;
    o.ens_global = on("DL_ENS_GLOBAL"); o.ens_force_comm = on("DL_ENS_FORCE_COMM"); o.ens_no_defer = on("DL_ENS_NO_DEFER"); o.ens_no_fold = on("DL_ENS_NO_FOLD");
    o.ens_stamps = on("DL_ENS_STAMPS"); o.ens_fold_stamps = on("DL_ENS_FOLD_STAMPS");
    o.cg_mt = std::getenv("DL_CG_MT") ? atoi(std::getenv("DL_CG_MT")) : 0;
    o.host_mode = std::getenv("DL_HOST_MODE") ? atoi(std::getenv("DL_HOST_MODE")) : -1;
    auto flag = [](const char* name) { const char* v = std::getenv(name); return v != nullptr && atoi(v) != 0; };
    o.no_emu_fused = on("DL_NO_EMU_FUSED"); o.no_gram_epilogue = on("DL_NO_GRAM_EPILOGUE"); o.no_chi2_big = on("DL_NO_CHI2_BIG");
    o.fs_no_moments = flag("DL_FS_NO_MOMENTS");
    o.fs_mu_prio = std::getenv("DL_FS_MU_PRIO") ? atoi(std::getenv("DL_FS_MU_PRIO")) != 0 : true;
    o.step_kernel = flag("DL_STEP_KERNEL"); o.chi2_fused = flag("DL_CHI2_FUSED"); o.chi2_bfrag = flag("DL_CHI2_BFRAG");
    o.xcd_local = std::getenv("DL_XCD_LOCAL") ? atoi(std::getenv("DL_XCD_LOCAL")) : 1;
    o.chi2_max_rows = std::getenv("DL_CHI2_GEMM_MAX") ? atoll(std::getenv("DL_CHI2_GEMM_MAX")) : 2048;
}
const DlOptions& dl_options() {
    std::call_once(g_options_once, dl_options_read);
    return g_options;
}
extern "C" void dl_options_refresh(void) { (void)dl_options(); dl_options_read(); }

__device__ __forceinline__ int dl_fs_point_of_wg(int wg, int xblk) { return xblk ? xblk * ((wg & 7) + 8 * ((wg >> 3) / xblk)) + ((wg >> 3) % xblk) : wg; }

#define DL_FS_FLAG_PRIO (1 << 16)
#define DL_FS_STAMP_SLOTS 10
#define DL_HWREG_HW_ID ((31 << 11) | 4)
#define DL_HWREG_XCC_ID ((31 << 11) | 20)
static int dl_fs_launch_flags(int xblk, int stop_after) { return stop_after != 0 ? stop_after : (xblk << 8) | (dl_options().fs_mu_prio ? DL_FS_FLAG_PRIO : 0); }

template <bool FAST, int NL, bool EFT, bool DENSE, bool TH_ROW = false, bool SUB = false, int NT = DL_FS_THREADS, bool MOM = false>
__device__ __forceinline__ void dl_fullshape_body(const DlObsDev& o, const double* __restrict__ theta, int n_params, double* __restrict__ power,
                                                  int64_t ld_power, double* __restrict__ tables, int64_t ld_tables, int stop_after, unsigned long long* __restrict__ stamps,
                                                  const double* th_row = nullptr,
                                                  double* lds_sub = nullptr, int tid_sub = 0, int b_sub = 0) {
    extern __shared__ __attribute__((aligned(16))) double lds_wg[];
    double* lds = SUB ? lds_sub : lds_wg;
    const int flags = (SUB || (stop_after & ~0xff) == 0 || stop_after < 0) ? 0 : stop_after;
    const int xblk = (flags >> 8) & 0xff;
    stop_after = (SUB || flags) ? 0 : stop_after;
    const int b = SUB ? b_sub : dl_fs_point_of_wg(blockIdx.x, xblk);
    const int tid = SUB ? tid_sub : (int)threadIdx.x, nthr = NT;
#define DL_STAMP(slot) if (stamps != nullptr && tid == 0) stamps[(size_t)blockIdx.x * DL_FS_STAMP_SLOTS + (slot)] = __builtin_amdgcn_s_memtime();
#define DL_STAMP_HWID(slot) stamps[(size_t)blockIdx.x * DL_FS_STAMP_SLOTS + (slot)] = ((unsigned long long)__builtin_amdgcn_s_getreg(DL_HWREG_XCC_ID) << 32) | __builtin_amdgcn_s_getreg(DL_HWREG_HW_ID);
    DL_STAMP(0)
    if (stamps != nullptr && tid == 0) { stamps[(size_t)blockIdx.x * DL_FS_STAMP_SLOTS + 6] = __builtin_amdgcn_s_memrealtime(); DL_STAMP_HWID(8) }
    if (FAST && stamps != nullptr && tid == NT - 64) { DL_STAMP_HWID(9) }
    const bool toep = !o.fixed_spline && (FAST || o.toeplitz);
    static_assert(!MOM || (FAST && !EFT && !DENSE), "the moment form belongs to the pair evaluation");
    const DlFsShared s = MOM ? dl_fs_shared_carve_mom(lds, o) : dl_fs_shared_carve(lds, o.n_t, o.n_in, dl_fs_n_dd0(o), toep);
    const bool direct = MOM && dl_fs_mom_direct(o);
    const double* th = TH_ROW ? th_row : theta + (size_t)b * n_params;
    if (stop_after == -1) return;
    double lk_pref[DL_P3_PREF];
#pragma unroll
    for (int it = 0; it < DL_P3_PREF; ++it) lk_pref[it] = (tid + it * nthr < o.n_kin) ? o.lkin[tid + it * nthr] : 0.;
    if (FAST) {
        constexpr int KT = NT - 64;
        const bool mu_wave = tid >= KT;
        constexpr bool PRIO = !SUB && !EFT && !DENSE && NT == DL_FS_THREADS;
        const bool mu_prio = PRIO && (flags & DL_FS_FLAG_PRIO) && __builtin_amdgcn_readfirstlane(tid) >= KT;
        if (mu_prio) __builtin_amdgcn_s_setprio(2);
        const int m = tid - KT;
        const bool mu_lane = mu_wave && m < o.n_mu, scalar_lane = (tid == nthr - 1);
        DlMuCarry c;
        double dlt_pref[DL_TOEP_PREF];
#pragma unroll
        for (int it = 0; it < DL_TOEP_PREF; ++it) dlt_pref[it] = (!MOM && toep && !mu_wave && tid + it * KT < o.n_t - 1) ? o.dlt[tid + it * KT] : 0.;
        const bool knot_rec = MOM && (o.moment_form & 2);
        double kr[DL_KNOT_PREF][2];
#pragma unroll
        for (int it = 0; it < DL_KNOT_PREF; ++it) {
            const bool live = knot_rec && !mu_wave && tid + it * KT < o.n_t;
            const double2 r = live ? *reinterpret_cast<const double2*>(o.knot_rec + 2 * (size_t)(tid + it * KT)) : make_double2(0., 0.);
            kr[it][0] = r.x; kr[it][1] = r.y;
        }
        if (mu_wave) dl_fs_mu_partA(o, th, mu_lane ? m : 0, c);
        else if (knot_rec) dl_fs_knots_rec(tid, KT, o, th, s, kr);
        else dl_fs_knots<!MOM>(tid, KT, o, th, s, b);
        if (o.fixed_spline && mu_wave) {
            dl_fs_mu_partB(c);
            if (mu_lane) dl_fs_mu_partC(o, s, m, c, false);
            if (scalar_lane) dl_fs_scalars(o, th, s, c, false);
        }
        __syncthreads();
        DL_STAMP(1)
        if (stop_after == 1) return;
        if (toep) {
            if (mu_wave) dl_fs_mu_partB(c);
            else dl_fs_phase2_fir<MOM>(tid, KT, o, s);
            __syncthreads();
            DL_STAMP(2)
            if (stop_after == 2) return;
            if (mu_wave) {
                if (mu_lane) dl_fs_mu_partC(o, s, m, c, false);
                if (scalar_lane) dl_fs_scalars(o, th, s, c, false);
            } else if (MOM) { if (tid < 64) dl_fs_mom_fixup(tid, o, s); }
            else dl_fs_phase2d_toep(tid, KT, o, s, dlt_pref);
            __syncthreads();
            DL_STAMP(3)
            if (stop_after == 5) return;
        }
        if (mu_prio) __builtin_amdgcn_s_setprio(0);
    } else {
        dl_fs_phase01<true>(tid, nthr, o, th, s, b);
        __syncthreads();
        if (stop_after == 1) return;
        if (toep) {
            double dlt_pref[DL_TOEP_PREF];
#pragma unroll
            for (int it = 0; it < DL_TOEP_PREF; ++it) dlt_pref[it] = (tid + it * nthr < o.n_t - 1) ? o.dlt[tid + it * nthr] : 0.;
            dl_fs_phase2_fir(tid, nthr, o, s);
            __syncthreads();
            if (stop_after == 2) return;
            dl_fs_phase2d_toep(tid, nthr, o, s, dlt_pref);
            __syncthreads();
            if (stop_after == 5) return;
        } else if (!o.fixed_spline) {
            dl_fs_phase2a(tid, nthr, o, s);
            __syncthreads();
            if (stop_after == 2) return;
            dl_fs_phase2b_dot(tid, nthr, o, s);
            __syncthreads();
            dl_fs_phase2b(tid, nthr, o, s);
            __syncthreads();
            if (stop_after == 3) return;
            dl_fs_phase2c_dot(tid, nthr, o, s);
            __syncthreads();
            dl_fs_phase2c(tid, nthr, o, s);
            __syncthreads();
            if (stop_after == 4) return;
            dl_fs_phase2d(tid, nthr, o, s);
            __syncthreads();
            if (stop_after == 5) return;
        }
    }
    double* prow = power + (size_t)b * (1 + o.n_var) * ld_power + o.col_offset;
    double* trow = tables ? tables + (size_t)b * ld_tables : nullptr;
    if (FAST && !EFT && !DENSE) dl_fs_phase3_pair<NL, EFT, MOM>(tid, nthr, o, s, lk_pref, direct ? prow : nullptr);
    else dl_fs_phase3<FAST, NL, EFT>(tid, nthr, o, s, trow, lk_pref);
    if (!direct) {
        __syncthreads();
        DL_STAMP(4)
        dl_fs_phase4(tid, nthr, o, s, th, prow, ld_power);
    } else {
        DL_STAMP(4)
    }
    DL_STAMP(5)
    if (stamps != nullptr && tid == 0) stamps[(size_t)blockIdx.x * DL_FS_STAMP_SLOTS + 7] = __builtin_amdgcn_s_memrealtime();
#undef DL_STAMP
#undef DL_STAMP_HWID
}

template <bool FAST, int NL, bool EFT, bool DENSE = false, bool MOM = false>
__global__ __launch_bounds__(DL_FS_THREADS, DENSE ? 5 : 4) void dl_fullshape_kernel(const DlObsDev o, const double* __restrict__ theta, int n_params, double* __restrict__ power,
                                                                     int64_t ld_power, double* __restrict__ tables, int64_t ld_tables, int stop_after, unsigned long long* __restrict__ stamps) {
    dl_obs_prefetch((const void*)__builtin_amdgcn_kernarg_segment_ptr());
    dl_fullshape_body<FAST, NL, EFT, DENSE, false, false, DL_FS_THREADS, MOM>(o, theta, n_params, power, ld_power, tables, ld_tables, stop_after, stamps);
}

static bool dl_fs_use_moments(const DlObsDev* obs_host, int n_obs) {
    if (dl_options().fs_no_moments) return false;
    for (int i = 0; i < n_obs; ++i)
        if (!(obs_host[i].moment_form & 1) || obs_host[i].n_ct > 0 || obs_host[i].n_sn > 0) return false;
    return true;
}
static size_t dl_fs_fast_shared_bytes(const DlObsDev& oh, bool mom) { return (mom ? dl_fs_mom_shared_doubles(oh) : dl_fs_shared_doubles_obs(oh, true)) * sizeof(double); }

template <int NL, bool MOM = false>
__global__ __launch_bounds__(512, 2) void dl_fullshape_wide_kernel(const DlObsDev o, const double* __restrict__ theta, int n_params, double* __restrict__ power,
                                                                 int64_t ld_power, int stop_after, unsigned long long* __restrict__ stamps) {
    dl_obs_prefetch((const void*)__builtin_amdgcn_kernarg_segment_ptr());
    dl_fullshape_body<true, NL, false, false, false, false, 512, MOM>(o, theta, n_params, power, ld_power, nullptr, 0, stop_after, stamps);
}


__device__ __forceinline__ void dl_png_build_moments(int tid, int nthr, const DlObsDev& o, const DlFsShared& s, bool toep) {
    if (toep) {
        dl_fs_phase2_fir(tid, nthr, o, s);
    } else {
        dl_fs_phase2a(tid, nthr, o, s);
        __syncthreads();
        dl_fs_phase2b_dot(tid, nthr, o, s);
        __syncthreads();
        dl_fs_phase2b(tid, nthr, o, s);
        __syncthreads();
        dl_fs_phase2c_dot(tid, nthr, o, s);
        __syncthreads();
        dl_fs_phase2c(tid, nthr, o, s);
    }
    __syncthreads();
}

__global__ __launch_bounds__(DL_FS_THREADS, 2) void dl_png_kernel(DlObsDev o, const double* __restrict__ theta, int n_params, double* __restrict__ power, int64_t ld_power) {
    extern __shared__ __attribute__((aligned(16))) double lds[];
    const int tid = threadIdx.x, nthr = DL_FS_THREADS, n_t = o.n_t;
    const int64_t b = blockIdx.x;
    const double* th = theta + (size_t)b * n_params;
    const bool toep = o.toeplitz;
    const DlFsShared s = dl_fs_shared_carve(lds, n_t, o.n_in, -1, toep);
    double* tabs = s.coef;
    double* murec = lds + dl_fs_shared_doubles(n_t, o.n_in);
    double* sc = murec + 8 * DL_PNG_MAX_MU;
    dl_png_setup(tid, nthr, o, th, murec, sc);
    dl_png_knots(tid, nthr, o, th, s, true);
    __syncthreads();
    dl_png_build_moments(tid, nthr, o, s, toep);
    dl_png_keep_spline(tid, nthr, o, s, toep, tabs, tabs + n_t);
    __syncthreads();
    dl_png_knots(tid, nthr, o, th, s, false);
    __syncthreads();
    dl_png_build_moments(tid, nthr, o, s, toep);
    dl_png_keep_spline(tid, nthr, o, s, toep, tabs + 2 * n_t, tabs + 3 * n_t);
    __syncthreads();
    dl_png_eval(tid, nthr, o, tabs, murec, sc, s.out);
    __syncthreads();
    double* prow = power + (size_t)b * (1 + o.n_var) * ld_power + o.col_offset;
    for (int idx = tid; idx < o.n_in; idx += nthr) prow[idx] = s.out[idx];
}

template <bool FAST, int NL, bool EFT, bool DENSE = false, bool MOM = false>
__global__ __launch_bounds__(DL_FS_THREADS, DENSE ? 5 : 4) void dl_fullshape_multi_kernel(const DlObsDev* __restrict__ obs, const double* __restrict__ theta, int n_params,
                                                                           double* __restrict__ power, int64_t ld_power, int stop_after) {
    dl_fullshape_body<FAST, NL, EFT, DENSE, false, false, DL_FS_THREADS, MOM>(obs[blockIdx.y], theta, n_params, power, ld_power, nullptr, 0, stop_after, nullptr);
}

#define DL_ENS_MAXP 32
#define DL_ENS_SLOTS_PER_WG 8
#define DL_EF_STAMP(slot) if (f.stamps != nullptr && publish && threadIdx.x == 0) { __builtin_amdgcn_s_waitcnt(0); f.stamps[(size_t)b * 8 + (slot)] = __builtin_amdgcn_s_memtime(); }
__device__ __forceinline__ void dl_ens_propose(const DlEnsFold& f, int b, bool publish, double* __restrict__ th_out, double* __restrict__ scratch) {
#pragma clang fp contract(off)
    const int lane = threadIdx.x & 63;
    DL_EF_STAMP(1)
    const int half = f.nw / 2, P = f.P;
    const DlPhilox r = dl_philox4x32((uint32_t)f.it_prop, (uint32_t)((unsigned long long)f.it_prop >> 32), (uint32_t)b, DL_ENS_STREAM_MOVE + f.half_prop, f.k0, f.k1);
    const double u = dl_uniform53(r.x[0], r.x[1]);
    const double t = (f.a - 1.) * u + 1.;
    const double zz = (t * t) / f.a;
    const int ic = dl_ens_split_at(f.split_prop, (1 - f.half_prop) * half + (int)(r.x[2] % (uint32_t)half));
    const int is = dl_ens_split_at(f.split_prop, f.half_prop * half + b);
    const int sA = dl_ens_pending_slot(f.pend, is, half), sB = dl_ens_pending_slot(f.pend, ic, half);
    const int p = lane < P ? lane : P - 1;
    DL_EF_STAMP(2)
    const double x_old = f.coords[(size_t)is * P + p], c_old = f.coords[(size_t)ic * P + p];
    const double x_new = f.pend.half >= 0 ? f.pend.prop[(size_t)(sA >= 0 ? sA : 0) * P + p] : 0., c_new = f.pend.half >= 0 ? f.pend.prop[(size_t)(sB >= 0 ? sB : 0) * P + p] : 0.;
    bool ax = false, ac = false;
    if (sA >= 0 || sB >= 0) {
        const DlEnsDecision2 d = dl_ens_decide2(f.pend, f.priors, P, f.n_tiles, f.offset, f.k0, f.k1, sA, f.logp[is], sB, f.logp[ic], scratch);
        ax = d.acc[0]; ac = d.acc[1];
    }
    DL_EF_STAMP(3)
    if (lane < P) {
        const double c = ac ? c_new : c_old, x = ax ? x_new : x_old;
        const double q = c - (c - x) * zz;
        th_out[lane] = q;
        if (publish) f.prop_out[(size_t)b * P + lane] = q;
    }
    if (publish && lane == 0) f.factors_out[b] = (P - 1.) * log(zz);
    DL_EF_STAMP(4)
}

__device__ __forceinline__ void dl_ens_write_state(const DlEnsFold& f, int e, double* __restrict__ scratch) {
#pragma clang fp contract(off)
    const int lane = threadIdx.x & 63, wave = threadIdx.x >> 6;
    const int half = f.nw / 2, P = f.P, hl = lane & 31, hb = lane >> 5;
    const int s0 = DL_ENS_SLOTS_PER_WG * e + 2 * wave, s1 = s0 + 1;
    if (s0 >= half) return;
    const bool two = s1 < half;
    const int w0 = dl_ens_split_at(f.pend.split, f.pend.half * half + s0), w1 = two ? dl_ens_split_at(f.pend.split, f.pend.half * half + s1) : w0;
    const double lw0 = f.logp[w0], lw1 = f.logp[w1];
    const int s = hb ? s1 : s0, w = hb ? w1 : w0;
    const int n = dl_ens_split_at(f.pend.split, (1 - f.pend.half) * half + (hb && !two ? s0 : s));
    const int p = hl < P ? hl : P - 1;
    const double v_old = f.coords[(size_t)w * P + p], v_new = f.pend.prop[(size_t)(hb && !two ? s0 : s) * P + p], v_n = f.coords[(size_t)n * P + p];
    const double ln = f.logp[n];
    const DlEnsDecision2 d = dl_ens_decide2(f.pend, f.priors, P, f.n_tiles, f.offset, f.k0, f.k1, s0, lw0, two ? s1 : -1, lw1, scratch + DL_ENS_SCRATCH * wave);
    if (hb && !two) return;
    const bool acc = hb ? d.acc[1] : d.acc[0];
    const double lp = hb ? d.lp[1] : d.lp[0], lw = hb ? lw1 : lw0;
    if (hl < P) {
        const double v = acc ? v_new : v_old;
        f.coords_out[(size_t)w * P + hl] = v; f.coords_out[(size_t)n * P + hl] = v_n;
        if (f.chain != nullptr) { f.chain[(size_t)w * P + hl] = v; f.chain[(size_t)n * P + hl] = v_n; }
    }
    if (hl == 0) {
        const double lv = acc ? lp : lw;
        f.logp_out[w] = lv; f.logp_out[n] = ln;
        if (acc) f.nacc[w] += 1;
        if (f.chain_logp != nullptr) { f.chain_logp[w] = lv; f.chain_logp[n] = ln; }
    }
}

template <int NL, bool DENSE = false, bool MOM = false>
__global__ __launch_bounds__(DL_FS_THREADS, DENSE ? 5 : 3) void dl_fullshape_ens_kernel(const DlObsDev* __restrict__ obs, const DlEnsFold f, double* __restrict__ power, int64_t ld_power,
                                                                         int flags, int B) {
    __shared__ double dl_ens_theta[DL_ENS_MAXP];
    __shared__ double dl_ens_scratch[DL_ENS_SCRATCH * (DL_FS_THREADS / 64)];
    const unsigned long long t_entry = __builtin_amdgcn_s_memtime();
    dl_kernarg_prefetch<(sizeof(DlEnsFold) + 8 + 63) / 64 * 64 + 64>();
    if ((int)blockIdx.x >= B) {
        if (blockIdx.y == 0 && f.pend.half >= 0) dl_ens_write_state(f, (int)blockIdx.x - B, dl_ens_scratch);
        return;
    }
    if (threadIdx.x < 64) dl_ens_propose(f, dl_fs_point_of_wg(blockIdx.x, (flags >> 8) & 0xff), blockIdx.y == 0, dl_ens_theta, dl_ens_scratch);
    else if (threadIdx.x < 128) {
        dl_scalar_prefetch<0, (offsetof(DlObsDev, ct_in) + 63) / 64 * 64, offsetof(DlObsDev, coef_w) / 64 * 64, (sizeof(DlObsDev) + 63) / 64 * 64>((const void*)(obs + blockIdx.y));
    }
// ... 179 lines not shown

void dl_launch_fullshape_jac(const DlObsDev* obs_host, int n_obs, const DlObsDev* obs_dev, const double* theta, int n_params, int64_t B, int k_live, int k_pad, double* jac, int64_t ldj,
                             hipStream_t stream) {
    size_t shm = 0;
    bool nl3 = true;
    for (int i = 0; i < n_obs; ++i) { shm = std::max(shm, dl_fs_jac_shared_doubles(obs_host[i], n_params) * sizeof(double)); nl3 = nl3 && obs_host[i].n_ell <= 3; }
    auto launch = [&](auto kernel) {
        if (shm > 48 * 1024) (void)hipFuncSetAttribute((const void*)kernel, hipFuncAttributeMaxDynamicSharedMemorySize, (int)shm);
        DL_LAUNCH(kernel, dim3((unsigned)B, (unsigned)n_obs), dim3(DL_FS_THREADS), shm, stream, obs_dev, theta, n_params, k_live, k_pad, jac, ldj);
    };
    if (nl3) launch(dl_fullshape_jac_kernel<3, 2>); else launch(dl_fullshape_jac_kernel<DL_MAX_ELL, 1>);
}

template <int MODEL, bool PS = false>
__global__ __launch_bounds__(512) void dl_bao_kernel(const DlObsDev o, const double* __restrict__ theta, int n_params, double* __restrict__ power, int64_t ld_power) {
    extern __shared__ __attribute__((aligned(16))) double lds[];
    const int b = blockIdx.x, tid = threadIdx.x, nthr = blockDim.x;
    const double* th = theta + (size_t)b * n_params;
    dl_bao_phaseA(tid, nthr, o, th, lds);
    if (PS) {
        const DlPsShared ps = dl_bao_ps_carve(lds, o.n_t, o.n_in);
        dl_bao_ps_knots(tid, nthr, o, th, ps);
        __syncthreads();
        dl_bao_ps_fir(tid, nthr, o, ps);
        __syncthreads();
        const double end = dl_bao_ps_end_moment(tid, o, ps);
        __syncthreads();
        dl_bao_ps_end_store(tid, o, ps, end);
        __syncthreads();
        dl_bao_ps_end_relations(tid, o, ps);
    }
    __syncthreads();
    dl_bao_phaseB_m<MODEL, PS>(tid, nthr, o, lds);
    __syncthreads();
    dl_store_with_pass(tid, nthr, o, th, lds + DL_BAO_PT, power + (size_t)b * (1 + o.n_var) * ld_power + o.col_offset);
}

static int dl_bao_threads(int n_kin, int64_t B) {
    static const int forced = getenv("DL_BAO_THREADS") ? atoi(getenv("DL_BAO_THREADS")) : 0;
    if (forced >= 64 && forced <= 512 && forced % 64 == 0) return forced;
    int t = (n_kin + 63) / 64 * 64;
    t = t > 256 ? 256 : t;
    if (B >= 4096) t = 64;
    else if (B >= 2048 && t > 128) t = 128;
    return t;
}

__global__ __launch_bounds__(DL_FS_THREADS) void dl_emulated_kernel(const DlObsDev o, const double* __restrict__ theta, int n_params, double* __restrict__ power, int64_t ld_power,
                                                                   double* __restrict__ feat, int64_t feat_ld) {
    extern __shared__ __attribute__((aligned(16))) double lds[];
    const int b = blockIdx.x;
    dl_emu_point(o, theta + (size_t)b * n_params, lds, power + (size_t)b * (1 + o.n_var) * ld_power + o.col_offset, ld_power,
                 feat ? feat + (size_t)b * feat_ld + o.feat_off : nullptr);
}

__global__ __launch_bounds__(DL_WS_THREADS) void dl_ws_template_kernel(const double* __restrict__ tab, const DlInput qbao_in, const DlInput dm_in, const double* __restrict__ theta,
                                                                       int n_params, double* __restrict__ scratch, int64_t ld) {
    extern __shared__ __attribute__((aligned(16))) double lds[];
    const int tid = threadIdx.x;
    const double* th = theta + (size_t)blockIdx.x * n_params;
    const double qbao = dl_get(qbao_in, th), dm = dl_get(dm_in, th);
    const DlWsTab t = dl_ws_open(tab);
    const DlWsShared s = dl_ws_carve(lds, t.n_i, DL_WS_THREADS);
    double carry = 0.;
    for (int phase = 0; phase < DL_WS_PHASES; ++phase) {
        dl_ws_point_phase(phase, tid, DL_WS_THREADS, qbao, dm, t, s, carry, scratch + (size_t)blockIdx.x * ld);
        __syncthreads();
    }
}

static void dl_launch_ws_templates(const DlObsDev* obs_host, int n_obs, const double* theta, int n_params, int64_t B, hipStream_t stream) {
    for (int i = 0; i < n_obs; ++i) {
        if (obs_host[i].templ != 5) continue;
        bool done = false;
        for (int j = 0; j < i; ++j) done = done || (obs_host[j].templ == 5 && dl_ws_scratch(obs_host[j]) == dl_ws_scratch(obs_host[i]));
        if (done) continue;
        const size_t shm = dl_ws_shared_doubles(dl_ws_n_inner(obs_host[i]), DL_WS_THREADS) * sizeof(double);
        if (shm > 48 * 1024) (void)hipFuncSetAttribute((const void*)dl_ws_template_kernel, hipFuncAttributeMaxDynamicSharedMemorySize, (int)shm);
        DL_LAUNCH(dl_ws_template_kernel, dim3((unsigned)B), dim3(DL_WS_THREADS), shm, stream, dl_ws_tab(obs_host[i]), dl_ws_qbao(obs_host[i]), obs_host[i].dm, theta, n_params,
                  const_cast<double*>(dl_ws_scratch(obs_host[i])), dl_ws_scratch_ld(obs_host[i]));
    }
}

void dl_launch_fullshape(const DlObsDev* obs_host, int n_obs, const double* theta, int n_params, int64_t B, double* power, int64_t ld_power, double* tables,
                         int64_t ld_tables, hipStream_t stream, double* feat, int64_t feat_ld, int xcd_block, const DlObsDev* obs_dev, bool moments) {
    dl_launch_ws_templates(obs_host, n_obs, theta, n_params, B, stream);
    static const int stop_after = getenv("DL_FS_STOP") ? atoi(getenv("DL_FS_STOP")) : 0;
    static const char* stamp_file = getenv("DL_FS_STAMPS");
    static unsigned long long* stamps_dev = nullptr;
    static int stamp_launches = 0;
    if (stamp_file && !stamps_dev) { (void)hipMalloc((void**)&stamps_dev, (size_t)65536 * DL_FS_STAMP_SLOTS * sizeof(unsigned long long)); }
    unsigned long long* stamps = (stamp_file && B >= 256 && B <= 65536 && stamp_launches >= 30 && stamp_launches < 34) ? stamps_dev : nullptr;
    if (stamp_file && B >= 256) stamp_launches++;
    const bool merge = !dl_options().no_merged_theory;
    if (merge && obs_dev != nullptr && n_obs > 1 && n_obs <= 8 && tables == nullptr && feat == nullptr && stop_after == 0 && !stamp_file) {
        bool same = true, eft0 = obs_host[0].n_ct > 0 || obs_host[0].n_sn > 0, nl3 = obs_host[0].n_ell <= 3;
        size_t shmem = 0;
        for (int i = 0; i < n_obs && same; ++i) {
            const DlObsDev& oh = obs_host[i];
            const bool generic = !oh.uniform_knots || !(oh.toeplitz || oh.fixed_spline);
            if (oh.theory >= 2 || generic || (oh.n_ct > 0 || oh.n_sn > 0) != eft0 || (oh.n_ell <= 3) != nl3) same = false;
        }
        if (same && !eft0) {
            static const int64_t dense_min = getenv("DL_FS_DENSE_MIN") ? atoll(getenv("DL_FS_DENSE_MIN")) : 4096;
            const bool dense = B * n_obs > dense_min, mom = moments && !dense && dl_fs_use_moments(obs_host, n_obs);
            for (int i = 0; i < n_obs; ++i) shmem = std::max(shmem, dl_fs_fast_shared_bytes(obs_host[i], mom));
            auto launch = [&](auto kernel) {
                if (shmem > 48 * 1024) (void)hipFuncSetAttribute((const void*)kernel, hipFuncAttributeMaxDynamicSharedMemorySize, (int)shmem);
                const int flags = dl_fs_launch_flags((xcd_block > 0 && B % (8 * xcd_block) == 0) ? xcd_block : 0, 0);
                DL_LAUNCH(kernel, dim3((unsigned)B, (unsigned)n_obs), dim3(DL_FS_THREADS), shmem, stream, obs_dev, theta, n_params, power, ld_power, flags);
            };
            if (nl3) { if (dense) launch(dl_fullshape_multi_kernel<true, 3, false, true>); else if (mom) launch(dl_fullshape_multi_kernel<true, 3, false, false, true>); else launch(dl_fullshape_multi_kernel<true, 3, false>); }
            else { if (dense) launch(dl_fullshape_multi_kernel<true, 5, false, true>); else if (mom) launch(dl_fullshape_multi_kernel<true, 5, false, false, true>); else launch(dl_fullshape_multi_kernel<true, 5, false>); }
            return;
        }
    }
    for (int i = 0; i < n_obs; ++i) {
        if (obs_host[i].theory == 5) {
            const size_t shm = dl_png_shared_doubles(obs_host[i].n_t, obs_host[i].n_in) * sizeof(double);
            if (shm > 48 * 1024) (void)hipFuncSetAttribute((const void*)dl_png_kernel, hipFuncAttributeMaxDynamicSharedMemorySize, (int)shm);
            DL_LAUNCH(dl_png_kernel, dim3((unsigned)B), dim3(DL_FS_THREADS), shm, stream, obs_host[i], theta, n_params, power, ld_power);
            continue;
        }
        if (obs_host[i].theory == 4) {
            dl_launch_tns(obs_host[i], theta, n_params, B, power, ld_power, stream);
            continue;
        }
        if (obs_host[i].theory == 3 && feat != nullptr && !dl_options().no_emu_batch) {
            size_t shm = dl_eb_shared_doubles(obs_host[i]) * sizeof(double);
            if (shm > 48 * 1024) (void)hipFuncSetAttribute((const void*)dl_emulated_batch_kernel, hipFuncAttributeMaxDynamicSharedMemorySize, (int)shm);
            DL_LAUNCH(dl_emulated_batch_kernel, dim3((unsigned)((B + DL_EB_PTS - 1) / DL_EB_PTS)), dim3(256), shm, stream, obs_host[i], theta, n_params, B, feat, feat_ld);
            continue;
        }
        if (obs_host[i].theory == 3) {
            size_t shm = dl_emu_shared_doubles_obs(obs_host[i]) * sizeof(double);
            DL_LAUNCH(dl_emulated_kernel, dim3((unsigned)B), dim3(DL_FS_THREADS), shm, stream, obs_host[i], theta, n_params, power, ld_power, feat, feat_ld);
            continue;
        }
        if (obs_host[i].theory == 2) {
            const bool ps = obs_host[i].templ == 4;
            size_t shm = (ps ? dl_bao_ps_shared_doubles(obs_host[i].n_t, obs_host[i].n_in) : dl_bao_shared_doubles(obs_host[i].n_in)) * sizeof(double);
            auto launch_bao = [&](auto kernel) {
                if (shm > 48 * 1024) (void)hipFuncSetAttribute((const void*)kernel, hipFuncAttributeMaxDynamicSharedMemorySize, (int)shm);
                DL_LAUNCH(kernel, dim3((unsigned)B), dim3((unsigned)dl_bao_threads(obs_host[i].n_kin, B)), shm, stream, obs_host[i], theta, n_params, power, ld_power);
            };
            const int model = obs_host[i].bao_mode >> 4;
            if (ps) {
                if (model == 0) launch_bao(dl_bao_kernel<0, true>);
                else if (model & 32) launch_bao(dl_bao_kernel<3, true>);
                else if (model & 16) launch_bao(dl_bao_kernel<2, true>);
                else launch_bao(dl_bao_kernel<1, true>);
            }
            else if (model == 0) launch_bao(dl_bao_kernel<0>);
            else if (model & 32) launch_bao(dl_bao_kernel<3>);
            else if (model & 16) launch_bao(dl_bao_kernel<2>);
            else launch_bao(dl_bao_kernel<1>);
            continue;
        }
        const DlObsDev& oh = obs_host[i];
        const bool generic = tables || !oh.uniform_knots || !(oh.toeplitz || oh.fixed_spline);
        static const int64_t dense_min = getenv("DL_FS_DENSE_MIN") ? atoll(getenv("DL_FS_DENSE_MIN")) : 4096;
        bool nl3 = oh.n_ell <= 3, eft = oh.n_ct > 0 || oh.n_sn > 0;
        static const int wide_env = getenv("DL_FS_WIDE") ? atoi(getenv("DL_FS_WIDE")) : -1;
        const bool wide = !generic && !eft && tables == nullptr && (wide_env == 1 || (wide_env != 0 && B * n_obs <= 256));
        const bool mom = moments && !generic && !eft && (wide || B <= dense_min) && dl_fs_use_moments(&oh, 1);
        size_t shmem = generic ? dl_fs_shared_doubles_obs(oh, false) * sizeof(double) : dl_fs_fast_shared_bytes(oh, mom);
        auto launch = [&](auto kernel) {
            if (shmem > 48 * 1024) (void)hipFuncSetAttribute((const void*)kernel, hipFuncAttributeMaxDynamicSharedMemorySize, (int)shmem);
            const int flags = dl_fs_launch_flags((xcd_block > 0 && B % (8 * xcd_block) == 0) ? xcd_block : 0, stop_after);
            DL_LAUNCH(kernel, dim3((unsigned)B), dim3(DL_FS_THREADS), shmem, stream, obs_host[i], theta, n_params, power, ld_power, tables, ld_tables, flags, stamps);
            if (stamps) {
                (void)hipStreamSynchronize(stream);
                std::vector<unsigned long long> h((size_t)B * DL_FS_STAMP_SLOTS);
                (void)hipMemcpy(h.data(), stamps, h.size() * sizeof(unsigned long long), hipMemcpyDeviceToHost);
                if (FILE* f = fopen(stamp_file, "a")) {
                    for (int64_t w = 0; w < B; ++w) { for (int q = 0; q < DL_FS_STAMP_SLOTS; ++q) fprintf(f, "%llu ", h[(size_t)w * DL_FS_STAMP_SLOTS + q]); fprintf(f, "\n"); }
                    fprintf(f, "#\n");
                    fclose(f);
                }
            }
        };
        if (wide) {
            auto launch_wide = [&](auto kernel) {
                if (shmem > 48 * 1024) (void)hipFuncSetAttribute((const void*)kernel, hipFuncAttributeMaxDynamicSharedMemorySize, (int)shmem);
                const int flags = dl_fs_launch_flags((xcd_block > 0 && B % (8 * xcd_block) == 0) ? xcd_block : 0, stop_after);
                DL_LAUNCH(kernel, dim3((unsigned)B), dim3(512), shmem, stream, obs_host[i], theta, n_params, power, ld_power, flags, stamps);
            };
            if (nl3) { if (mom) launch_wide(dl_fullshape_wide_kernel<3, true>); else launch_wide(dl_fullshape_wide_kernel<3>); }
            else { if (mom) launch_wide(dl_fullshape_wide_kernel<5, true>); else launch_wide(dl_fullshape_wide_kernel<5>); }
            continue;
        }
        if (generic) launch(dl_fullshape_kernel<false, 5, true>);
        else if (nl3 && !eft) { if (B > dense_min) launch(dl_fullshape_kernel<true, 3, false, true>); else if (mom) launch(dl_fullshape_kernel<true, 3, false, false, true>); else launch(dl_fullshape_kernel<true, 3, false>); }
        else if (nl3) launch(dl_fullshape_kernel<true, 3, true>);
        else if (!eft) { if (B > dense_min) launch(dl_fullshape_kernel<true, 5, false, true>); else if (mom) launch(dl_fullshape_kernel<true, 5, false, false, true>); else launch(dl_fullshape_kernel<true, 5, false>); }
        else launch(dl_fullshape_kernel<true, 5, true>);
    }
}

typedef double dl_double4 __attribute__((ext_vector_type(4)));
typedef double dl_double2 __attribute__((ext_vector_type(2)));

#define DL_GEMM_WAVES 8

struct DlGemmFrag {
    dl_double2 a[4], b0[4], b1[4];
};

__device__ __forceinline__ void dl_gemm_load(DlGemmFrag& f, const double* ap, const double* b0p, const double* b1p, int kc) {
    const dl_double2* a2 = reinterpret_cast<const dl_double2*>(ap + (size_t)kc * 32);
    const dl_double2* b02 = reinterpret_cast<const dl_double2*>(b0p + (size_t)kc * 32);
    const dl_double2* b12 = reinterpret_cast<const dl_double2*>(b1p + (size_t)kc * 32);
#pragma unroll
    for (int q = 0; q < 4; ++q) { f.a[q] = a2[4 * q]; f.b0[q] = b02[4 * q]; f.b1[q] = b12[4 * q]; }
}

__device__ __forceinline__ void dl_gemm_mma(const DlGemmFrag& f, dl_double4& acc0, dl_double4& acc1) {
#pragma unroll
    for (int q = 0; q < 4; ++q) {
        acc0 = __builtin_amdgcn_mfma_f64_16x16x4f64(f.a[q].x, f.b0[q].x, acc0, 0, 0, 0);
        acc1 = __builtin_amdgcn_mfma_f64_16x16x4f64(f.a[q].x, f.b1[q].x, acc1, 0, 0, 0);
        acc0 = __builtin_amdgcn_mfma_f64_16x16x4f64(f.a[q].y, f.b0[q].y, acc0, 0, 0, 0);
        acc1 = __builtin_amdgcn_mfma_f64_16x16x4f64(f.a[q].y, f.b1[q].y, acc1, 0, 0, 0);
    }
}

__global__ __launch_bounds__(64 * DL_GEMM_WAVES) void dl_window_gemm_kernel(const double* __restrict__ A, int64_t lda, const double* __restrict__ Wt, int64_t ldw,
                                                                            const double* __restrict__ bias, double* __restrict__ C, int64_t ldc, int M, int N_valid,
                                                                            int K_pad, int bias_period) {
    __shared__ __attribute__((aligned(16))) double red[DL_GEMM_WAVES - 1][2][4][64];
    const int lane = threadIdx.x & 63, wave = threadIdx.x >> 6;
    const int r16 = lane & 15, g = lane >> 4;
    const int m0 = blockIdx.x * 16, n0 = blockIdx.y * 32;
    int arow = m0 + r16;
    if (arow > M - 1) arow = M - 1;
    const double* ap = A + (size_t)arow * lda + g * 2;
    const double* b0p = Wt + (size_t)(n0 + r16) * ldw + g * 2;
    const double* b1p = Wt + (size_t)(n0 + 16 + r16) * ldw + g * 2;
    dl_double4 acc0 = {0., 0., 0., 0.}, acc1 = {0., 0., 0., 0.};
    const int nchunks = K_pad / 32;
    DlGemmFrag f0, f1;
    int kc = wave;
    if (kc < nchunks) dl_gemm_load(f0, ap, b0p, b1p, kc);
    for (; kc < nchunks; kc += 2 * DL_GEMM_WAVES) {
        int kn = kc + DL_GEMM_WAVES;
        if (kn < nchunks) dl_gemm_load(f1, ap, b0p, b1p, kn);
        dl_gemm_mma(f0, acc0, acc1);
        if (kn < nchunks) {
            int kn2 = kn + DL_GEMM_WAVES;
            if (kn2 < nchunks) dl_gemm_load(f0, ap, b0p, b1p, kn2);
            dl_gemm_mma(f1, acc0, acc1);
        }
    }
    if (wave > 0) {
#pragma unroll
        for (int r = 0; r < 4; ++r) { red[wave - 1][0][r][lane] = acc0[r]; red[wave - 1][1][r][lane] = acc1[r]; }
    }
    __syncthreads();
    if (wave == 0) {
#pragma unroll
        for (int r = 0; r < 4; ++r) {
            double s0 = acc0[r], s1 = acc1[r];
#pragma unroll
            for (int w = 0; w < DL_GEMM_WAVES - 1; ++w) { s0 += red[w][0][r][lane]; s1 += red[w][1][r][lane]; }
            int row = m0 + g + 4 * r;
            if (row < M) {
                bool wb = (row % bias_period) == 0;
                if (n0 + r16 < N_valid) C[(size_t)row * ldc + n0 + r16] = wb ? s0 + bias[n0 + r16] : s0;
                if (n0 + 16 + r16 < N_valid) C[(size_t)row * ldc + n0 + 16 + r16] = wb ? s1 + bias[n0 + 16 + r16] : s1;
            }
        }
    }
}

void dl_launch_window_gemm(const double* A, int64_t lda, const double* Wt, int64_t ldw, const double* bias, double* C, int64_t ldc, int64_t M, int N_valid, int N_pad,
                           int K_pad, int bias_period, hipStream_t stream) {
    dim3 grid((unsigned)((M + 15) / 16), (unsigned)(N_pad / 32));
    DL_LAUNCH(dl_window_gemm_kernel, grid, dim3(64 * DL_GEMM_WAVES), 0, stream, A, lda, Wt, ldw, bias, C, ldc, (int)M, N_valid, K_pad, bias_period);
}

// ... 227 lines not shown
        };
        if (R <= 1) launch_b(dl_emulated_stacked_gemm_kernel<1>); else if (R <= 4) launch_b(dl_emulated_stacked_gemm_kernel<4>); else if (R <= 6) launch_b(dl_emulated_stacked_gemm_kernel<6>); else launch_b(dl_emulated_stacked_gemm_kernel<8>);
    } else if (overlap) { if (R <= 1) launch_ov(dl_emulated_stacked_ov_kernel<1, DL_STKO_TMAX>); else if (R <= 4) launch_ov(dl_emulated_stacked_ov_kernel<4, DL_STKO_TMAX>); else if (R <= 6) launch_ov(dl_emulated_stacked_ov_kernel<6, DL_STKO_TMAX>); else launch_ov(dl_emulated_stacked_ov_kernel<8, DL_STKO_TMAX>); }
    else if (wide) { if (R <= 1) launch(dl_emulated_stacked_kernel<8, 1>); else if (R <= 4) launch(dl_emulated_stacked_kernel<8, 4>); else if (R <= 6) launch(dl_emulated_stacked_kernel<8, 6>); else launch(dl_emulated_stacked_kernel<8, 8>); }
    else { if (R <= 1) launch(dl_emulated_stacked_kernel<4, 1>); else if (R <= 4) launch(dl_emulated_stacked_kernel<4, 4>); else if (R <= 6) launch(dl_emulated_stacked_kernel<4, 6>); else launch(dl_emulated_stacked_kernel<4, 8>); }
    if (stamps) {
        (void)hipStreamSynchronize(stream);
        std::vector<unsigned long long> h((size_t)grid * slots);
        (void)hipMemcpy(h.data(), stamps, h.size() * sizeof(unsigned long long), hipMemcpyDeviceToHost);
        if (FILE* f = fopen(stamp_file, "a")) {
            for (unsigned w = 0; w < grid; ++w) { for (int q = 0; q < slots; ++q) fprintf(f, "%llu ", h[(size_t)w * slots + q]); fprintf(f, "\n"); }
            fprintf(f, "#\n");
            fclose(f);
        }
    }
}

bool dl_launch_emulated_feature_gram(const DlObsDev& obs, const double* theta, int n_params, int64_t B, const double* gfrag, const double* bias, const DlMargDev& mg, int n_valid,
                                     double* gram, hipStream_t stream, DlGramFinalize* fin) {
    const int R = 1 + obs.n_var;
    if (obs.eng[0].type == 2) return false;
    if (R > 6 || mg.n_s < 0 || mg.n_s > 15 || n_valid > 128) return false;
    if (mg.n_s == 0 && (fin == nullptr || dl_options().no_fused_solve || dl_options().no_gram_plain)) return false;
    DlEfGramArgs ga;
    std::memset(&ga, 0, sizeof(ga));
    ga.xr = 1 + mg.n_s; ga.gram = gram;
    ga.row_of[0] = 0; ga.cst[0] = bias;
    for (int s = 0; s < mg.n_s; ++s) {
        const int slot = mg.var_slot[s];
        if (slot >= 0) {
            if (1 + slot >= R) return false;
            ga.row_of[1 + slot] = 1 + s; ga.cst[1 + slot] = mg.tconst + (size_t)s * 128;
        } else { ga.const_row[ga.n_const] = 1 + s; ga.const_ptr[ga.n_const] = mg.tconst + (size_t)s * 128; ga.n_const++; }
    }
    for (int r = 1; r < R; ++r) if (ga.cst[r] == nullptr) return false;
    for (int r = 0; r < 6; ++r) ga.nz[r][0] = ga.nz[r][1] = -1;
    for (int c = 4; c < DL_N_VPARS; ++c) {
        const int slot = obs.vp_slot[c];
        if (slot >= 0 && 1 + slot < 6) dl_velocileptors_row_support(obs, c, ga.nz[1 + slot]);
    }
    ga.scaled = DL_FG_NM == 19 && obs.mono_mode != 0 && obs.eng[0].type == 0 && obs.n_basis == 65 && obs.nb_pad == 72 && !dl_options().no_scaled_row0;
    for (int r = 1; r < 6; ++r)
        for (int z = 0; z < 2; ++z) if (ga.nz[r][z] >= 0 && ga.nz[r][z] < 12) ga.scaled = 0;
    ga.no_early = dl_options().ef_no_early_theta;
    const size_t shm = dl_ef_gram_shared_doubles(obs, ga.xr) * sizeof(double);
    if (shm > 146 * 1024) return false;
    (void)hipFuncSetAttribute((const void*)dl_emulated_feature_gram_kernel, hipFuncAttributeMaxDynamicSharedMemorySize, (int)shm);
    static const char* stamp_file = getenv("DL_EF_STAMPS");
    static unsigned long long* stamps_dev = nullptr;
    static int stamp_launches = 0;
    const unsigned grid = (unsigned)((B + DL_EB_PTS - 1) / DL_EB_PTS);
    if (stamp_file && !stamps_dev) (void)hipMalloc((void**)&stamps_dev, (size_t)8192 * 16 * sizeof(unsigned long long));
    ga.stamps = (stamp_file && grid <= 8192 && stamp_launches >= 30 && stamp_launches < 34) ? stamps_dev : nullptr;
    if (stamp_file) stamp_launches++;
    if (ga.stamps) (void)hipMemsetAsync(ga.stamps, 0, (size_t)grid * 16 * sizeof(unsigned long long), stream);
    DlEfSolve sv;
    std::memset(&sv, 0, sizeof(sv));
    if (fin != nullptr && ga.xr <= 8 && !dl_options().no_fused_solve) {
        sv.enabled = 1; sv.post_mode = fin->post_mode & 0xff; sv.priors = fin->priors; sv.loglike = fin->loglike; sv.logprior = fin->logprior; sv.status = fin->status;
        sv.solved = fin->solved; sv.hessian = fin->hessian; sv.mg = mg;
        fin->done = true;
    }
    DL_LAUNCH(dl_emulated_feature_gram_kernel, dim3(grid, 1), dim3(512), shm, stream, theta, n_params, B, gfrag, obs, ga, sv);
    if (ga.stamps) {
        (void)hipStreamSynchronize(stream);
        std::vector<unsigned long long> h((size_t)grid * 16);
        (void)hipMemcpy(h.data(), ga.stamps, h.size() * sizeof(unsigned long long), hipMemcpyDeviceToHost);
        if (FILE* f = fopen(stamp_file, "a")) {
            for (unsigned w = 0; w < grid; ++w) { for (int q = 0; q < 16; ++q) fprintf(f, "%llu ", h[(size_t)w * 16 + q]); fprintf(f, "\n"); }
            fprintf(f, "#\n");
            fclose(f);
        }
    }
    return true;
}

int dl_chi2_gemm_row_tile(int64_t M, int N_pad) {
    const int forced = dl_options().cg_mt;
    if (forced == 16 || forced == 32) return forced;
    return ((M + DL_CG_M - 1) / DL_CG_M) * (N_pad / DL_CG_N) <= 128 ? 16 : DL_CG_M;
}

void dl_launch_chi2_gemm(const double* A, int64_t lda, const double* Wt, int64_t ldw, const double* bias, double* part, int64_t M, int N_pad, int K_pad, int32_t* counters,
                         const double* theta, int n_params, const double* priors, double* loglike, double* logprior, int32_t* status, int post_mode, hipStream_t stream,
                         const uint8_t* panel_ranges, int k_live, double* resid, int64_t ldr, const double* wfrag) {
    const int n_tiles = N_pad / DL_CG_N;
    const int mt = counters == nullptr ? dl_chi2_gemm_row_tile(M, N_pad) : DL_CG_M;
    const int64_t mblocks = (M + mt - 1) / mt;
    const unsigned grid = (unsigned)(8 * n_tiles * ((mblocks + 7) / 8));
    static bool optin = false;
    if (!optin) {
        (void)hipFuncSetAttribute((const void*)dl_chi2_gemm_kernel<true, true>, hipFuncAttributeMaxDynamicSharedMemorySize, DL_CG_LDS_BYTES);
        (void)hipFuncSetAttribute((const void*)dl_chi2_gemm_kernel<true, true, 16>, hipFuncAttributeMaxDynamicSharedMemorySize, DL_CG_LDS_BYTES);
        (void)hipFuncSetAttribute((const void*)dl_chi2_gemm_kernel<true, true, DL_CG_M, true>, hipFuncAttributeMaxDynamicSharedMemorySize, DL_CG_LDS_BYTES);
        (void)hipFuncSetAttribute((const void*)dl_chi2_gemm_kernel<true, true, 16, true>, hipFuncAttributeMaxDynamicSharedMemorySize, DL_CG_LDS_BYTES);
        optin = true;
    }
    DlChi2Fin fin;
    fin.counters = counters; fin.theta = theta; fin.priors = priors; fin.loglike = loglike; fin.logprior = logprior; fin.status = status;
    fin.n_params = n_params; fin.post_mode = post_mode; fin.ready = nullptr;
    static const char* stamp_file = getenv("DL_CG_STAMPS");
    static unsigned long long* stamps_dev = nullptr;
    static int stamp_launches = 0;
    if (stamp_file && !stamps_dev) (void)hipMalloc((void**)&stamps_dev, (size_t)65536 * 8 * sizeof(unsigned long long));
    fin.stamps = (stamp_file && grid <= 65536 && M >= 256 && stamp_launches >= 30 && stamp_launches < 34) ? stamps_dev : nullptr;
    if (stamp_file && M >= 256) stamp_launches++;
    DlChi2Panels panels;
    std::memset(&panels, 0, sizeof(panels));
    if (panel_ranges != nullptr && n_tiles <= DL_CG_MAX_TILES)
        for (int t = 0; t < n_tiles; ++t) panels.range[t] = (uint32_t)panel_ranges[2 * t] | ((uint32_t)panel_ranges[2 * t + 1] << 8);
    double* const no_resid = nullptr;
    int max_live = K_pad / DL_CG_KP;
    if (panel_ranges != nullptr && n_tiles <= DL_CG_MAX_TILES) {
        max_live = 0;
        for (int t = 0; t < n_tiles; ++t) max_live = std::max(max_live, panel_ranges[2 * t + 1] != 0 ? (int)panel_ranges[2 * t + 1] - (int)panel_ranges[2 * t] : K_pad / DL_CG_KP);
    }
    if (wfrag != nullptr && dl_options().chi2_bfrag && max_live <= DL_CG_PMAX) {
        const int kl = k_live > 0 ? k_live : K_pad;
        const size_t shm = std::max((size_t)DL_CG_NBUF * mt * DL_CG_LD * 8, (size_t)DL_CG_WAVES * 2 * 4 * 64 * 8);
        auto go = [&](auto kernel, double* rs, int64_t lr) {
            (void)hipFuncSetAttribute((const void*)kernel, hipFuncAttributeMaxDynamicSharedMemorySize, (int)shm);
            DL_LAUNCH(kernel, dim3(grid), dim3(64 * DL_CG_WAVES), shm, stream, A, lda, wfrag, bias, part, (int)M, K_pad, n_tiles, fin, panels, kl, rs, lr);
        };
        if (resid != nullptr) { if (mt == 16) go(dl_chi2_gemm_bf_kernel<true, true, 16, true>, resid, ldr); else go(dl_chi2_gemm_bf_kernel<true, true, DL_CG_M, true>, resid, ldr); }
        else { if (mt == 16) go(dl_chi2_gemm_bf_kernel<true, true, 16, false>, no_resid, (int64_t)0); else go(dl_chi2_gemm_bf_kernel<true, true, DL_CG_M, false>, no_resid, (int64_t)0); }
    } else if (resid != nullptr) {
        if (mt == 16) DL_LAUNCH((dl_chi2_gemm_kernel<true, true, 16, true>), dim3(grid), dim3(64 * DL_CG_WAVES), DL_CG_NBUF * (16 + DL_CG_N) * DL_CG_LD * 8, stream, A, lda, Wt, ldw, bias, part, (int)M, K_pad, n_tiles, fin, panels, k_live > 0 ? k_live : K_pad, resid, ldr);
        else DL_LAUNCH((dl_chi2_gemm_kernel<true, true, DL_CG_M, true>), dim3(grid), dim3(64 * DL_CG_WAVES), DL_CG_LDS_BYTES, stream, A, lda, Wt, ldw, bias, part, (int)M, K_pad, n_tiles, fin, panels, k_live > 0 ? k_live : K_pad, resid, ldr);
    } else if (mt == 16) DL_LAUNCH((dl_chi2_gemm_kernel<true, true, 16>), dim3(grid), dim3(64 * DL_CG_WAVES), DL_CG_NBUF * (16 + DL_CG_N) * DL_CG_LD * 8, stream, A, lda, Wt, ldw, bias, part, (int)M, K_pad, n_tiles, fin, panels, k_live > 0 ? k_live : K_pad, no_resid, (int64_t)0);
    else DL_LAUNCH((dl_chi2_gemm_kernel<true, true>), dim3(grid), dim3(64 * DL_CG_WAVES), DL_CG_LDS_BYTES, stream, A, lda, Wt, ldw, bias, part, (int)M, K_pad, n_tiles, fin, panels, k_live > 0 ? k_live : K_pad, no_resid, (int64_t)0);
    if (fin.stamps) {
        (void)hipStreamSynchronize(stream);
        std::vector<unsigned long long> h((size_t)grid * 8);
        (void)hipMemcpy(h.data(), fin.stamps, h.size() * sizeof(unsigned long long), hipMemcpyDeviceToHost);
        if (FILE* f = fopen(stamp_file, "a")) {
            for (unsigned w = 0; w < grid; ++w) { for (int q = 0; q < 8; ++q) fprintf(f, "%llu ", h[(size_t)w * 8 + q]); fprintf(f, "\n"); }
            fprintf(f, "#\n");
            fclose(f);
        }
    }
}

template <int NL>
__global__ __launch_bounds__(1024) void dl_step_kernel(const DlObsDev o, const double* __restrict__ theta, int n_params, double* __restrict__ power, int64_t ld_power,
                                                       const double* __restrict__ Wt, int64_t ldw, const double* __restrict__ bias, double* __restrict__ part, int M, int K_pad,
                                                       DlChi2Fin fin, DlChi2Panels panels, int k_live, int32_t* __restrict__ ready, int32_t target, int lds_per_point) {
    extern __shared__ __attribute__((aligned(16))) double lds[];
    const int L = blockIdx.x, xcd = L & 7, j = L >> 3;
    const int q = j >> 3, c = j & 7, mb = xcd + 8 * q;
    const int sub = threadIdx.x >> 8, tid = threadIdx.x & 255;
    unsigned long long* st = fin.stamps != nullptr ? fin.stamps + (size_t)blockIdx.x * 8 : nullptr;
    if (st != nullptr && threadIdx.x == 0) { st[0] = __builtin_amdgcn_s_memtime(); st[6] = __builtin_amdgcn_s_memrealtime(); }
    dl_fullshape_body<true, NL, false, false, false, true>(o, theta, n_params, power, ld_power, nullptr, 0, 0, nullptr, nullptr, lds + (size_t)sub * lds_per_point, tid, 32 * mb + 4 * c + sub);
    if (st != nullptr && threadIdx.x == 0) st[1] = __builtin_amdgcn_s_memtime();
    __asm__ volatile("s_waitcnt vmcnt(0)" : : : "memory");
    __syncthreads();
    if (threadIdx.x == 0) __hip_atomic_fetch_add(ready + mb, 1, __ATOMIC_RELAXED, __HIP_MEMORY_SCOPE_AGENT);
    if (st != nullptr && threadIdx.x == 0) st[2] = __builtin_amdgcn_s_memtime();
    DlChi2Fin f2 = fin;
    f2.stamps = nullptr;
    dl_chi2_gemm_tile<true, true, DL_CG_M, false>(power, ld_power, Wt, ldw, bias, part, M, K_pad, 8, f2, panels, k_live, nullptr, 0, lds, mb, c, [&]() {
        if (threadIdx.x == 0) {
            int spins = 0;
            while (__hip_atomic_load(ready + mb, __ATOMIC_RELAXED, __HIP_MEMORY_SCOPE_AGENT) < target && ++spins < (1 << 22)) __builtin_amdgcn_s_sleep(1);
        }
        __syncthreads();
        __asm__ volatile("" : : : "memory");
        if (st != nullptr && threadIdx.x == 0) st[3] = __builtin_amdgcn_s_memtime();
    });
    if (st != nullptr && threadIdx.x == 0) { st[4] = __builtin_amdgcn_s_memtime(); st[7] = __builtin_amdgcn_s_memrealtime(); }
}

size_t dl_step_lds_bytes(const DlObsDev& oh, int64_t B, int N_pad) {
    const bool generic = !oh.uniform_knots || !(oh.toeplitz || oh.fixed_spline);
    if (oh.theory >= 2 || generic || oh.n_ct > 0 || oh.n_sn > 0 || oh.n_ell > 3 || oh.n_pass != 0 || oh.n_var != 0 || N_pad != 128) return 0;
    if (oh.templ == 5) return 0;
    if (B <= 0 || B > 1024 || B % 256 != 0) return 0;
    const size_t per_point = (dl_fs_shared_doubles_obs(oh, true) + 1) / 2 * 2;
    const size_t bytes = std::max<size_t>(4 * per_point * sizeof(double), DL_CG_LDS_BYTES);
    return bytes <= 160 * 1024 ? bytes : 0;
}

void dl_launch_step(const DlObsDev& oh, const double* theta, int n_params, int64_t B, double* power, int64_t ld_power, const double* Wt, int64_t ldw, const double* bias,
                    double* part, int K_pad, int k_live, int32_t* counters, int32_t* ready, int32_t target, const double* priors, double* loglike, double* logprior, int32_t* status,
                    int post_mode, hipStream_t stream, const uint8_t* panel_ranges) {
    DlChi2Panels panels;
    std::memset(&panels, 0, sizeof(panels));
    if (panel_ranges != nullptr) for (int t = 0; t < 8; ++t) panels.range[t] = (uint32_t)panel_ranges[2 * t] | ((uint32_t)panel_ranges[2 * t + 1] << 8);
    const size_t per_point = (dl_fs_shared_doubles_obs(oh, true) + 1) / 2 * 2;
    const size_t shm = dl_step_lds_bytes(oh, B, 128);
    static bool optin = false;
    if (!optin) { (void)hipFuncSetAttribute((const void*)dl_step_kernel<3>, hipFuncAttributeMaxDynamicSharedMemorySize, 160 * 1024); optin = true; }
    DlChi2Fin fin;
    fin.counters = counters; fin.theta = theta; fin.priors = priors; fin.loglike = loglike; fin.logprior = logprior; fin.status = status;
    fin.n_params = n_params; fin.post_mode = post_mode; fin.ready = ready;
    const unsigned grid = (unsigned)(B / 4);
    static const char* stamp_file = getenv("DL_STEP_STAMPS");
    static unsigned long long* stamps_dev = nullptr;
    static int stamp_launches = 0;
    if (stamp_file && !stamps_dev) (void)hipMalloc((void**)&stamps_dev, (size_t)256 * 8 * sizeof(unsigned long long));
    fin.stamps = (stamp_file && stamp_launches >= 30 && stamp_launches < 34) ? stamps_dev : nullptr;
    if (stamp_file) stamp_launches++;
    if (fin.stamps) (void)hipMemsetAsync(fin.stamps, 0, (size_t)256 * 8 * sizeof(unsigned long long), stream);
    DL_LAUNCH(dl_step_kernel<3>, dim3(grid), dim3(1024), shm, stream, oh, theta, n_params, power, ld_power, Wt, ldw, bias, part, (int)B, K_pad, fin, panels, k_live > 0 ? k_live : K_pad,
              ready, target, (int)per_point);
    if (fin.stamps) {
        (void)hipStreamSynchronize(stream);
        std::vector<unsigned long long> h((size_t)grid * 8);
        (void)hipMemcpy(h.data(), fin.stamps, h.size() * sizeof(unsigned long long), hipMemcpyDeviceToHost);
        if (FILE* f = fopen(stamp_file, "a")) {
            for (unsigned w = 0; w < grid; ++w) { for (int q = 0; q < 8; ++q) fprintf(f, "%llu ", h[(size_t)w * 8 + q]); fprintf(f, "\n"); }
            fprintf(f, "#\n");
            fclose(f);
        }
    }
}

__global__ __launch_bounds__(64) void dl_finalize_part_kernel(const double* __restrict__ part, int n_tiles, const double* __restrict__ theta, int n_params,
                                                               const double* __restrict__ priors, int64_t B, double* __restrict__ loglike,
                                                               double* __restrict__ logprior, int32_t* __restrict__ status, int post_mode) {
    extern __shared__ __attribute__((aligned(16))) double dl_fp_priors[];
    dl_kernarg_prefetch<96>();
    const int64_t b = (int64_t)blockIdx.x * blockDim.x + threadIdx.x;
    const int64_t bb = b < B ? b : B - 1;
    double pv[2];
#pragma unroll
    for (int q = 0; q < 2; ++q) pv[q] = priors[(int)threadIdx.x + q * 64 < 5 * n_params ? (int)threadIdx.x + q * 64 : 0];
    double x0[8];
    dl_load_theta8(theta + (size_t)bb * n_params, n_params, 0, x0);
    const double chi2 = dl_chi2_of_parts(part + (size_t)bb * n_tiles, n_tiles);
#pragma unroll
    for (int q = 0; q < 2; ++q)
        if ((int)threadIdx.x + q * 64 < 5 * n_params) dl_fp_priors[threadIdx.x + q * 64] = pv[q];
    for (int e = threadIdx.x + 128; e < 5 * n_params; e += 64) dl_fp_priors[e] = priors[e];
    __syncthreads();
    if (b >= B) return;
    const double inf = __builtin_huge_val();
    double ll, lp;
    int st;
    dl_finalize_from_chi2(chi2, x0, theta + (size_t)b * n_params, n_params, dl_fp_priors, ll, lp, st);
    if (loglike) loglike[b] = post_mode ? (st == DL_ST_OK ? ll + lp : -inf) : ll;
    if (logprior) logprior[b] = lp;
    if (status) status[b] = st;
}

void dl_launch_finalize_part(const double* part, int n_tiles, const double* theta, int n_params, const double* priors, int64_t B, double* loglike, double* logprior,
                             int32_t* status, int post_mode, hipStream_t stream) {
    const size_t shm = (size_t)5 * n_params * sizeof(double);
    if (shm > 48 * 1024) (void)hipFuncSetAttribute((const void*)dl_finalize_part_kernel, hipFuncAttributeMaxDynamicSharedMemorySize, (int)shm);
    DL_LAUNCH(dl_finalize_part_kernel, dim3((unsigned)((B + 63) / 64)), dim3(64), shm, stream, part, n_tiles, theta, n_params, priors, B, loglike, logprior, status, post_mode);
}

__device__ __forceinline__ double dl_readlane(double v, int l) {
    int lo = __double2loint(v), hi = __double2hiint(v);
    lo = __builtin_amdgcn_readlane(lo, l);
    hi = __builtin_amdgcn_readlane(hi, l);
    return __hiloint2double(hi, lo);
}

__device__ __forceinline__ double dl_grouplane(double v, int j) {
    int lo = __double2loint(v), hi = __double2hiint(v);
    switch (j) {
        case 0: lo = __builtin_amdgcn_update_dpp(0, lo, 0x150 + 0, 0xf, 0xf, false); hi = __builtin_amdgcn_update_dpp(0, hi, 0x150 + 0, 0xf, 0xf, false); break;
        case 1: lo = __builtin_amdgcn_update_dpp(0, lo, 0x150 + 1, 0xf, 0xf, false); hi = __builtin_amdgcn_update_dpp(0, hi, 0x150 + 1, 0xf, 0xf, false); break;
        case 2: lo = __builtin_amdgcn_update_dpp(0, lo, 0x150 + 2, 0xf, 0xf, false); hi = __builtin_amdgcn_update_dpp(0, hi, 0x150 + 2, 0xf, 0xf, false); break;
        case 3: lo = __builtin_amdgcn_update_dpp(0, lo, 0x150 + 3, 0xf, 0xf, false); hi = __builtin_amdgcn_update_dpp(0, hi, 0x150 + 3, 0xf, 0xf, false); break;
        case 4: lo = __builtin_amdgcn_update_dpp(0, lo, 0x150 + 4, 0xf, 0xf, false); hi = __builtin_amdgcn_update_dpp(0, hi, 0x150 + 4, 0xf, 0xf, false); break;
        case 5: lo = __builtin_amdgcn_update_dpp(0, lo, 0x150 + 5, 0xf, 0xf, false); hi = __builtin_amdgcn_update_dpp(0, hi, 0x150 + 5, 0xf, 0xf, false); break;
        case 6: lo = __builtin_amdgcn_update_dpp(0, lo, 0x150 + 6, 0xf, 0xf, false); hi = __builtin_amdgcn_update_dpp(0, hi, 0x150 + 6, 0xf, 0xf, false); break;
        case 7: lo = __builtin_amdgcn_update_dpp(0, lo, 0x150 + 7, 0xf, 0xf, false); hi = __builtin_amdgcn_update_dpp(0, hi, 0x150 + 7, 0xf, 0xf, false); break;
        case 8: lo = __builtin_amdgcn_update_dpp(0, lo, 0x150 + 8, 0xf, 0xf, false); hi = __builtin_amdgcn_update_dpp(0, hi, 0x150 + 8, 0xf, 0xf, false); break;
        case 9: lo = __builtin_amdgcn_update_dpp(0, lo, 0x150 + 9, 0xf, 0xf, false); hi = __builtin_amdgcn_update_dpp(0, hi, 0x150 + 9, 0xf, 0xf, false); break;
        case 10: lo = __builtin_amdgcn_update_dpp(0, lo, 0x150 + 10, 0xf, 0xf, false); hi = __builtin_amdgcn_update_dpp(0, hi, 0x150 + 10, 0xf, 0xf, false); break;
        case 11: lo = __builtin_amdgcn_update_dpp(0, lo, 0x150 + 11, 0xf, 0xf, false); hi = __builtin_amdgcn_update_dpp(0, hi, 0x150 + 11, 0xf, 0xf, false); break;
        case 12: lo = __builtin_amdgcn_update_dpp(0, lo, 0x150 + 12, 0xf, 0xf, false); hi = __builtin_amdgcn_update_dpp(0, hi, 0x150 + 12, 0xf, 0xf, false); break;
        case 13: lo = __builtin_amdgcn_update_dpp(0, lo, 0x150 + 13, 0xf, 0xf, false); hi = __builtin_amdgcn_update_dpp(0, hi, 0x150 + 13, 0xf, 0xf, false); break;
        case 14: lo = __builtin_amdgcn_update_dpp(0, lo, 0x150 + 14, 0xf, 0xf, false); hi = __builtin_amdgcn_update_dpp(0, hi, 0x150 + 14, 0xf, 0xf, false); break;
        case 15: lo = __builtin_amdgcn_update_dpp(0, lo, 0x150 + 15, 0xf, 0xf, false); hi = __builtin_amdgcn_update_dpp(0, hi, 0x150 + 15, 0xf, 0xf, false); break;
        default: break;
    }
    return __hiloint2double(hi, lo);
}

template <bool PACK = false>
__device__ __forceinline__ double dl_lane_cholesky(double (&a)[16], double (&invc)[16], int m, int lane, bool& ok) {
    double dmine = 1.;
#pragma unroll
    for (int j = 0; j < 16; ++j) {
        invc[j] = 1.;
        if (j < m) {
            double djj = PACK ? dl_grouplane(a[j], j) : dl_readlane(a[j], j);
            if (!(djj > 0.)) { ok = false; djj = 1.; }
            const double inv = 1. / sqrt(djj);
            invc[j] = inv;
            if (lane == j) dmine = djj;
            const double cij = (lane > j) ? a[j] * inv : (lane == j ? djj * inv : 0.);
            a[j] = cij;
#pragma unroll
            for (int k = j + 1; k < 16; ++k) a[k] -= cij * (PACK ? dl_grouplane(cij, k) : dl_readlane(cij, k));
        }
    }
    const double lg = log(dmine);
    double logdet = 0.;
#pragma unroll
    for (int j = 0; j < 16; ++j) if (j < m) logdet += PACK ? dl_grouplane(lg, j) : dl_readlane(lg, j);
    return logdet;
}

template <bool LANES, bool STAGED>
__global__ __launch_bounds__(256, 4) void dl_finalize_marg_kernel(const double* __restrict__ dtilde, int64_t ld, int n, int rows_per_point, int n_slabs, int64_t slab_stride,
                                                               const double* __restrict__ bias, DlMargDev mg,
                                                               const double* __restrict__ theta, int n_params, const double* __restrict__ priors, int64_t B,
                                                               double* __restrict__ loglike, double* __restrict__ logprior, int32_t* __restrict__ status,
                                                               double* __restrict__ solved, double* __restrict__ hessian, int post_mode,
                                                               unsigned long long* __restrict__ stamps, const double* __restrict__ gram) {
    const int lane = threadIdx.x & 63, wave = threadIdx.x >> 6;
#define DL_FM_STAMP(slot) if (stamps != nullptr && threadIdx.x == 0) stamps[(size_t)blockIdx.x * 8 + (slot)] = __builtin_amdgcn_s_memtime();
    DL_FM_STAMP(0)
    if (stamps != nullptr && threadIdx.x == 0) stamps[(size_t)blockIdx.x * 8 + 6] = __builtin_amdgcn_s_memrealtime();
    int64_t b = (int64_t)blockIdx.x * 4 + wave;
    if (post_mode & 0x100) {
        const int64_t w = blockIdx.x, xcd = w & 7, r = w >> 3;
        b = 16 * (xcd + 8 * (r >> 2)) + 4 * (r & 3) + wave;
    }
    post_mode &= 0xff;
    bool active = b < B;
    if (!active) b = B - 1;
    const int ns = mg.n_s;
    const double* row0 = dtilde + (size_t)b * rows_per_point * ld;
    double chi2 = 0.;
    double HL[DL_MAX_SOLVED * (DL_MAX_SOLVED + 1) / 2];
    double gL[DL_MAX_SOLVED];
    double lp = 0.;
// ... 494 lines not shown
```

desilike_amd/csrc/dl_prior.h:

```cpp
#pragma once
#include <hip/hip_runtime.h>

#define DL_PRIOR_MAX_KIND 9

__device__ __forceinline__ double dl_prior_family(int kind, double y) {
    const double inf = __builtin_huge_val();
    switch (kind) {
        case 2: return y >= 0. ? -y : -inf;
        case 3: return -fabs(y);
        case 4: return -log1p(y * y);
        case 5: { const double a = fabs(y); return (-a - 2. * log1p(exp(-a))) + 1.3862943611198906; }
        case 6: return y >= 0. ? -0.5 * (y * y) : -inf;
        case 7: return y >= 0. ? -log1p(y * y) : -inf;
        case 8: return 1. - (y + exp(-y));
        case 9: return (y - exp(y)) + 1.;
        default: return 0.;
    }
}

__device__ __forceinline__ double dl_prior_logpdf(const double* __restrict__ pr, double x) {
    const double inf = __builtin_huge_val();
    const double kind = pr[0], lo = pr[1], hi = pr[2], loc = pr[3], scale = pr[4];
    const bool isin = (lo <= x) & (x <= hi);
    double v = 0.;
    if (kind == 1.) { const double t = x - loc; v = -0.5 * (t * t) / (scale * scale); }
    else if (kind >= 2.) v = dl_prior_family((int)kind, (x - loc) / scale);
    return isin ? v : -inf;
}
```

Before: 45.17 million evals/s.

## Compute log-prior inside full-shape kernel and record it for chi2 finalize

Moves prior evaluation out of the chi2 GEMM prologue and finalize kernels into the full-shape theory kernel. There each point's log-prior and NaN flag are computed across lanes and stored to a per-point workspace. The fused chi2 GEMM, step kernel and a new finalize kernel read the recorded values, and the fused path now also covers general prior kinds. It also batches the partial-chi2 atomic loads in groups of 16 in the fused finish. In exchange it adds a small per-point buffer and cross-kernel reads through agent-scope atomics.

```diff
diff --git a/desilike_amd/csrc/dl_api.hip b/desilike_amd/csrc/dl_api.hip
--- a/desilike_amd/csrc/dl_api.hip
+++ b/desilike_amd/csrc/dl_api.hip
@@ -58,6 +58,7 @@
     std::vector<DlObsDev> obs_kernarg;
     DlObsDev* obs_array_dev = nullptr;
     double* priors_dev = nullptr;
+    double* prior_rec_ws = nullptr;
     int32_t* gemm_counters = nullptr;
     int32_t* step_ready = nullptr;
     double* wt_white_dev = nullptr;
@@ -513,7 +514,7 @@
     if (ctx->data_index_ws) (void)hipFree(ctx->data_index_ws);
     void* ptrs[] = {ctx->arena_dev, ctx->priors_dev, ctx->wt_white_dev, ctx->wt_frag_dev, ctx->bias_white_dev, ctx->wt_full_dev, ctx->bias_full_dev, ctx->wh_dev,
                     ctx->bias_wh_dev, ctx->flatdata_dev, ctx->transform_dev, ctx->tconst_dev, ctx->power_ws, ctx->delta_ws, ctx->flat_ws, ctx->stencil_ws, ctx->theta_stage, ctx->out_stage,
-                    ctx->status_stage, ctx->gemm_counters, ctx->obs_array_dev, ctx->ws_scratch};
+                    ctx->status_stage, ctx->gemm_counters, ctx->obs_array_dev, ctx->ws_scratch, ctx->prior_rec_ws};
     for (void* p : ptrs) if (p) (void)hipFree(p);
     for (double* p : ctx->gfrag_dev) if (p) (void)hipFree(p);
     for (auto& ob : ctx->obs) if (ob.tns) { dl_tns_destroy(ob.tns); ob.tns = nullptr; }
@@ -561,7 +562,7 @@
     if (need <= ctx->cap) return 0;
     need = std::min<int64_t>(std::max<int64_t>(need, 1024), DL_CHUNK);
     if (ctx->cap > 0) DL_HIP_CHECK(ctx, hipDeviceSynchronize());
-    for (double** p : {&ctx->power_ws, &ctx->delta_ws, &ctx->flat_ws, &ctx->feat_ws, &ctx->stencil_ws, &ctx->ws_scratch}) if (*p) { (void)hipFree(*p); *p = nullptr; }
+    for (double** p : {&ctx->power_ws, &ctx->delta_ws, &ctx->flat_ws, &ctx->feat_ws, &ctx->stencil_ws, &ctx->ws_scratch, &ctx->prior_rec_ws}) if (*p) { (void)hipFree(*p); *p = nullptr; }
     ctx->cap = 0;
     const size_t R = 1 + ctx->n_var;
     DL_HIP_CHECK(ctx, hipMalloc((void**)&ctx->power_ws, (size_t)need * R * ctx->K_pad * sizeof(double)));
@@ -569,6 +570,7 @@
     DL_HIP_CHECK(ctx, hipMalloc((void**)&ctx->flat_ws, (size_t)need * ctx->N_pad * sizeof(double)));
     if (ctx->feat_ok) DL_HIP_CHECK(ctx, hipMalloc((void**)&ctx->feat_ws, (size_t)need * ctx->feat_ld * sizeof(double)));
     DL_HIP_CHECK(ctx, hipMalloc((void**)&ctx->stencil_ws, (size_t)need * ctx->n_params * sizeof(double)));
+    DL_HIP_CHECK(ctx, hipMalloc((void**)&ctx->prior_rec_ws, (size_t)need * 2 * sizeof(double)));
     if (ctx->ws_ld > 0) {
         DL_HIP_CHECK(ctx, hipMalloc((void**)&ctx->ws_scratch, (size_t)need * ctx->ws_ld * sizeof(double)));
         DL_HIP_CHECK(ctx, hipMemset(ctx->ws_scratch, 0, (size_t)need * ctx->ws_ld * sizeof(double)));
@@ -584,6 +586,7 @@
     DL_HIP_CHECK(ctx, hipMemset(ctx->flat_ws, 0, (size_t)need * ctx->N_pad * sizeof(double)));
     if (ctx->feat_ok) DL_HIP_CHECK(ctx, hipMemset(ctx->feat_ws, 0, (size_t)need * ctx->feat_ld * sizeof(double)));
     DL_HIP_CHECK(ctx, hipMemset(ctx->stencil_ws, 0, (size_t)need * ctx->n_params * sizeof(double)));
+    DL_HIP_CHECK(ctx, hipMemset(ctx->prior_rec_ws, 0, (size_t)need * 2 * sizeof(double)));
     DL_HIP_CHECK(ctx, hipDeviceSynchronize());
     ctx->cap = need;
     return 0;
@@ -626,23 +629,26 @@
         const bool chi2_path = !data && !feat_path && !ctx->any_transform && ctx->n_solved == 0 && nb <= chi2_max_rows;
         const int xcd_local = dl_options().xcd_local;
         const bool chi2_fused_env_early = dl_options().chi2_fused;
-        const bool chi2_fused_early = chi2_fused_env_early && !ctx->priors_general;
+        const bool chi2_fused_early = chi2_fused_env_early && chi2_path && !dl_options().fs_no_prior;
         const int xcd_block = !xcd_local ? 0 : chi2_path ? (chi2_fused_early ? 32 : dl_chi2_gemm_row_tile(nb, ctx->N_pad)) : (xcd_local > 1 && !feat_path && !ctx->any_transform && ctx->n_solved == 0 && ctx->N_pad == 128) ? 64 : 0;
         const bool step_kernel_allowed = dl_options().step_kernel;
-        if (step_kernel_allowed && chi2_path && !need_flat && ctx->n_obs == 1 && !ctx->priors_general && ctx->K_pad % 128 == 0 &&
+        DlPriorRec prior_rec;
+        if (chi2_path && !dl_options().fs_no_prior) { prior_rec.priors = ctx->priors_dev; prior_rec.lp = ctx->prior_rec_ws; prior_rec.flag = reinterpret_cast<int32_t*>(ctx->prior_rec_ws + ctx->cap); }
+        if (step_kernel_allowed && chi2_path && prior_rec.lp != nullptr && !need_flat && ctx->n_obs == 1 && ctx->K_pad % 128 == 0 &&
             dl_step_lds_bytes(ctx->obs_kernarg[0], nb, ctx->N_pad) != 0) {
             prof_phase(0);
             dl_launch_step(ctx->obs_kernarg[0], th, P, nb, ctx->power_ws, ctx->K_pad, ctx->wt_white_dev, ctx->K_pad, ctx->bias_white_dev, ctx->delta_ws, ctx->K_pad, ctx->K_live,
-                           ctx->gemm_counters, ctx->step_ready, 8, ctx->priors_dev, loglike_dev ? loglike_dev + b0 : nullptr, logprior_dev ? logprior_dev + b0 : nullptr,
+                           ctx->gemm_counters, ctx->step_ready, 8, prior_rec, loglike_dev ? loglike_dev + b0 : nullptr, logprior_dev ? logprior_dev + b0 : nullptr,
                            status_dev ? status_dev + b0 : nullptr, post_mode, stream, ctx->panel_ranges.empty() ? nullptr : ctx->panel_ranges.data());
             prof_phase(-1);
             if (prof) ctx->prof_calls++;
             continue;
         }
         prof_phase(0);
+        bool have_rec = false;
         if (!(feat_path && emu_fused))
-            dl_launch_fullshape(ctx->obs_kernarg.data(), ctx->n_obs, th, P, nb, ctx->power_ws, ctx->K_pad, nullptr, 0, stream, feat_path ? ctx->feat_ws : nullptr, ctx->feat_ld,
-                                xcd_block, ctx->obs_array_dev);
+            have_rec = dl_launch_fullshape(ctx->obs_kernarg.data(), ctx->n_obs, th, P, nb, ctx->power_ws, ctx->K_pad, nullptr, 0, stream, feat_path ? ctx->feat_ws : nullptr, ctx->feat_ld,
+                                           xcd_block, ctx->obs_array_dev, true, &prior_rec);
         prof_phase(1);
         int n_slabs = 1, cps = 0;
         int64_t slab_stride = 0;
@@ -689,11 +695,11 @@
                               dl_gemm_tiled_splits(nb, ctx->N_pad, ctx->K_pad, &cps_probe) == 1;
         int part_tiles = ctx->N_pad / 16;
         const bool chi2_fused_env = dl_options().chi2_fused;
-        const bool chi2_fused = chi2_fused_env && !ctx->priors_general;
+        const bool chi2_fused = chi2_fused_env && have_rec;
         if (chi2_path) {
             if (nb > 16384) { prof_phase(-1); return dl_fail(ctx, "dl_eval_batch: DL_CHI2_GEMM_MAX above 16384 rows"); }
             dl_launch_chi2_gemm(ctx->power_ws, ctx->K_pad, ctx->wt_white_dev, ctx->K_pad, ctx->bias_white_dev, ctx->delta_ws, nb, ctx->N_pad, ctx->K_pad,
-                                chi2_fused ? ctx->gemm_counters : nullptr, th, P, ctx->priors_dev, loglike_dev ? loglike_dev + b0 : nullptr,
+                                chi2_fused ? ctx->gemm_counters : nullptr, chi2_fused ? &prior_rec : nullptr, loglike_dev ? loglike_dev + b0 : nullptr,
                                 logprior_dev ? logprior_dev + b0 : nullptr, status_dev ? status_dev + b0 : nullptr, post_mode, stream,
                                 ctx->panel_ranges.empty() ? nullptr : ctx->panel_ranges.data(), ctx->K_live, nullptr, 0, ctx->wt_frag_dev);
         } else if (chi2_big) {
@@ -717,7 +723,10 @@
                                     status_dev ? status_dev + b0 : nullptr, stream);
         else if (chi2_path && chi2_fused) {
         } else if (finalized_in_kernel) {
-        } else if (chi2_path || chi2_big)
+        } else if (chi2_path && have_rec)
+            dl_launch_finalize_rec(ctx->delta_ws, part_tiles, prior_rec, nb, loglike_dev ? loglike_dev + b0 : nullptr, logprior_dev ? logprior_dev + b0 : nullptr,
+                                   status_dev ? status_dev + b0 : nullptr, post_mode, stream);
+        else if (chi2_path || chi2_big)
             dl_launch_finalize_part(ctx->delta_ws, part_tiles, th, P, ctx->priors_dev, nb, loglike_dev ? loglike_dev + b0 : nullptr, logprior_dev ? logprior_dev + b0 : nullptr,
                                     status_dev ? status_dev + b0 : nullptr, post_mode, stream);
         else if (ctx->n_solved > 0)
@@ -984,7 +993,7 @@
         const int64_t nc = std::min<int64_t>(per_pass, B - b0), nr = nc * P;
         const double* th = centers_dev + (size_t)b0 * P;
         dl_launch_fullshape(ctx->obs_kernarg.data(), ctx->n_obs, th, P, nc, ctx->power_ws, Kp, nullptr, 0, stream, nullptr, 0, xcd_local ? dl_chi2_gemm_row_tile(nc, Np) : 0, ctx->obs_array_dev);
-        dl_launch_chi2_gemm(ctx->power_ws, Kp, ctx->wt_white_dev, Kp, ctx->bias_white_dev, ctx->delta_ws, nc, Np, Kp, nullptr, th, P, ctx->priors_dev, nullptr, nullptr, nullptr, 1, stream,
+        dl_launch_chi2_gemm(ctx->power_ws, Kp, ctx->wt_white_dev, Kp, ctx->bias_white_dev, ctx->delta_ws, nc, Np, Kp, nullptr, nullptr, nullptr, nullptr, nullptr, 1, stream,
                             ctx->panel_ranges.empty() ? nullptr : ctx->panel_ranges.data(), ctx->K_live, ctx->fa_resid, Np, ctx->wt_frag_dev);
         dl_launch_fullshape_jac(ctx->obs_kernarg.data(), ctx->n_obs, ctx->obs_array_dev, th, P, nc, ctx->K_live, Kp, ctx->fa_jac, Kp, stream);
         int cps = 0;
@@ -1119,7 +1128,7 @@
         int32_t* st = status_dev ? status_dev + b0 : ctx->grad_status;
         dl_launch_fullshape(ctx->obs_kernarg.data(), ctx->n_obs, th, P, nb, ctx->power_ws, ctx->K_pad, nullptr, 0, stream, nullptr, 0, xcd_local ? dl_chi2_gemm_row_tile(nb, Np) : 0, ctx->obs_array_dev,
                             false);
-        dl_launch_chi2_gemm(ctx->power_ws, Kp, ctx->wt_white_dev, Kp, ctx->bias_white_dev, ctx->delta_ws, nb, Np, Kp, nullptr, th, P, ctx->priors_dev, nullptr, nullptr, nullptr, 1, stream,
+        dl_launch_chi2_gemm(ctx->power_ws, Kp, ctx->wt_white_dev, Kp, ctx->bias_white_dev, ctx->delta_ws, nb, Np, Kp, nullptr, nullptr, nullptr, nullptr, nullptr, 1, stream,
                             ctx->panel_ranges.empty() ? nullptr : ctx->panel_ranges.data(), ctx->K_live, ctx->grad_delta, Np, ctx->wt_frag_dev);
         dl_launch_finalize_part(ctx->delta_ws, Np / 16, th, P, ctx->priors_dev, nb, logposterior_dev + b0, nullptr, st, 1, stream);
         dl_launch_window_gemm_tiled(ctx->grad_delta, Np, ctx->grad_wtT, Np, ctx->grad_y, 0, Kp, nb, Kp, Np, 1, Np / 16, stream, 0);
@@ -1400,8 +1409,8 @@
     if (dl_reserve(ctx, B)) return 1;
     const int xcd_local = dl_options().xcd_local;
     if (!dl_launch_fullshape_ens(ctx->obs_kernarg.data(), ctx->n_obs, ctx->obs_array_dev, fold, B, ctx->power_ws, ctx->K_pad, xcd_local ? dl_chi2_gemm_row_tile(B, ctx->N_pad) : 0, stream)) return 2;
-    dl_launch_chi2_gemm(ctx->power_ws, ctx->K_pad, ctx->wt_white_dev, ctx->K_pad, ctx->bias_white_dev, part_out, B, ctx->N_pad, ctx->K_pad, nullptr, nullptr, ctx->n_params,
-                        ctx->priors_dev, nullptr, nullptr, nullptr, 1, stream, ctx->panel_ranges.empty() ? nullptr : ctx->panel_ranges.data(), ctx->K_live, nullptr, 0, ctx->wt_frag_dev);
+    dl_launch_chi2_gemm(ctx->power_ws, ctx->K_pad, ctx->wt_white_dev, ctx->K_pad, ctx->bias_white_dev, part_out, B, ctx->N_pad, ctx->K_pad, nullptr, nullptr,
+                        nullptr, nullptr, nullptr, 1, stream, ctx->panel_ranges.empty() ? nullptr : ctx->panel_ranges.data(), ctx->K_live, nullptr, 0, ctx->wt_frag_dev);
     DL_HIP_CHECK(ctx, hipGetLastError());
     return 0;
 }
@@ -1417,8 +1426,8 @@
     if (dl_reserve(ctx, B)) return 1;
     const int xcd_local = dl_options().xcd_local;
     dl_launch_fullshape(ctx->obs_kernarg.data(), ctx->n_obs, theta_dev, ctx->n_params, B, ctx->power_ws, ctx->K_pad, nullptr, 0, stream, nullptr, 0, xcd_local ? dl_chi2_gemm_row_tile(B, ctx->N_pad) : 0, ctx->obs_array_dev);
-    dl_launch_chi2_gemm(ctx->power_ws, ctx->K_pad, ctx->wt_white_dev, ctx->K_pad, ctx->bias_white_dev, ctx->delta_ws, B, ctx->N_pad, ctx->K_pad, nullptr, theta_dev, ctx->n_params,
-                        ctx->priors_dev, nullptr, nullptr, nullptr, 1, stream, ctx->panel_ranges.empty() ? nullptr : ctx->panel_ranges.data(), ctx->K_live, nullptr, 0, ctx->wt_frag_dev);
+    dl_launch_chi2_gemm(ctx->power_ws, ctx->K_pad, ctx->wt_white_dev, ctx->K_pad, ctx->bias_white_dev, ctx->delta_ws, B, ctx->N_pad, ctx->K_pad, nullptr, nullptr,
+                        nullptr, nullptr, nullptr, 1, stream, ctx->panel_ranges.empty() ? nullptr : ctx->panel_ranges.data(), ctx->K_live, nullptr, 0, ctx->wt_frag_dev);
     *part = ctx->delta_ws;
     *n_tiles = ctx->N_pad / 16;
     *priors = ctx->priors_dev;
diff --git a/desilike_amd/csrc/dl_chi2_gemm.h b/desilike_amd/csrc/dl_chi2_gemm.h
--- a/desilike_amd/csrc/dl_chi2_gemm.h
+++ b/desilike_amd/csrc/dl_chi2_gemm.h
@@ -20,12 +20,12 @@
 
 struct DlChi2Fin {
     int32_t* counters;
-    const double* theta;
-    const double* priors;
+    const double* lp_rec;
+    const int32_t* flag_rec;
     double* loglike;
     double* logprior;
     int32_t* status;
-    int32_t n_params, post_mode;
+    int32_t post_mode;
     unsigned long long* stamps;
     int32_t* ready;
 };
@@ -38,7 +38,7 @@
 #define DL_CG_STAMP(slot, fn) if (fin.stamps != nullptr && tid == 0) fin.stamps[(size_t)blockIdx.x * 8 + (slot)] = fn();
 template <int MT, bool RESID>
 __device__ __forceinline__ void dl_chi2_gemm_finish(dl_cg_double4 acc0, dl_cg_double4 acc1, double bj, double* __restrict__ part, int M, int n_tiles, const DlChi2Fin& fin,
-                                                    double* __restrict__ resid, int64_t ldr, double* lds, int mb, int nt, double fin_lp, int fin_nan) {
+                                                    double* __restrict__ resid, int64_t ldr, double* lds, int mb, int nt) {
     const int tid = threadIdx.x, lane = tid & 63, wave = __builtin_amdgcn_readfirstlane(tid >> 6);
     const int r16 = lane & 15, g = lane >> 4;
     constexpr int MTILES = MT / 16;
@@ -76,12 +76,20 @@
     if (lane == 0 && fin.ready != nullptr) __hip_atomic_store(fin.ready + mb, 0, __ATOMIC_RELAXED, __HIP_MEMORY_SCOPE_AGENT);
     const int row = m0 + lane;
     if (lane < MT && row < M) {
+        const double lp = __hip_atomic_load(fin.lp_rec + row, __ATOMIC_RELAXED, __HIP_MEMORY_SCOPE_AGENT);
+        const int fin_flag = __hip_atomic_load(fin.flag_rec + row, __ATOMIC_RELAXED, __HIP_MEMORY_SCOPE_AGENT);
         double chi2 = 0.;
-        for (int t = 0; t < n_tiles; ++t) chi2 += __hip_atomic_load(part + (size_t)row * n_tiles + t, __ATOMIC_RELAXED, __HIP_MEMORY_SCOPE_AGENT);
+        for (int t0 = 0; t0 < n_tiles; t0 += 16) {
+            double v[16];
+#pragma unroll
+            for (int t = 0; t < 16; ++t) v[t] = __hip_atomic_load(part + (size_t)row * n_tiles + (t0 + t < n_tiles ? t0 + t : n_tiles - 1), __ATOMIC_RELAXED, __HIP_MEMORY_SCOPE_AGENT);
+#pragma unroll
+            for (int t = 0; t < 16; ++t) chi2 = t0 + t < n_tiles ? chi2 + v[t] : chi2;
+        }
         const double inf = __builtin_huge_val();
-        const double lp = fin_lp, ll = -0.5 * chi2;
+        const double ll = -0.5 * chi2;
         int st = 0;
-        if (fin_nan) st = 3;
+        if (fin_flag == 3) st = 3;
         else if (lp == -inf) st = 1;
         else if (!(ll == ll) || ll == inf || ll == -inf) st = 2;
         if (fin.loglike) fin.loglike[row] = fin.post_mode ? (st == 0 ? ll + lp : -inf) : ll;
@@ -125,20 +133,6 @@
     const double* la = lds + r16 * DL_CG_LD + g;
     wait();
     if (DO_LOAD) { DL_CG_DMA(0) if (n_panels > 1) { DL_CG_DMA(1) } }
-    double fin_lp = 0.;
-    int fin_nan = 0;
-    if (fin.counters != nullptr && wave == 0 && lane < MT && m0 + lane < M) {
-        const double inf = __builtin_huge_val();
-        for (int p = 0; p < fin.n_params; ++p) {
-            double x = fin.theta[(size_t)(m0 + lane) * fin.n_params + p];
-            const double* pr = fin.priors + 5 * p;
-            if (x != x) fin_nan = 1;
-            bool isin = (pr[1] <= x) && (x <= pr[2]);
-            double v = 0.;
-            if (pr[0] == 1.) { double t = x - pr[3]; v = -0.5 * (t * t) / (pr[4] * pr[4]); }
-            fin_lp += isin ? v : -inf;
-        }
-    }
     if (n_panels > 1) __asm__ volatile("s_waitcnt vmcnt(%0)" : : "n"(VPT) : "memory");
     else __asm__ volatile("s_waitcnt vmcnt(0)" : : : "memory");
     __builtin_amdgcn_s_barrier();
@@ -180,7 +174,7 @@
 #undef DL_CG_MULTIPLY
 #undef DL_CG_MULTIPLY_LIM
 #undef DL_CG_DMA
-    dl_chi2_gemm_finish<MT, RESID>(acc0, acc1, bj, part, M, n_tiles, fin, resid, ldr, lds, mb, nt, fin_lp, fin_nan);
+    dl_chi2_gemm_finish<MT, RESID>(acc0, acc1, bj, part, M, n_tiles, fin, resid, ldr, lds, mb, nt);
 }
 
 #define DL_CG_PMAX 12
@@ -223,20 +217,6 @@
     dl_cg_double4 acc0 = {0., 0., 0., 0.}, acc1 = {0., 0., 0., 0.};
     const double* la = lds + r16 * DL_CG_LD + g;
     if (DO_LOAD) { DL_CG_DMA_A(0) if (n_panels > 1) { DL_CG_DMA_A(1) } }
-    double fin_lp = 0.;
-    int fin_nan = 0;
-    if (fin.counters != nullptr && wave == 0 && lane < MT && m0 + lane < M) {
-        const double inf = __builtin_huge_val();
-        for (int p = 0; p < fin.n_params; ++p) {
-            double x = fin.theta[(size_t)(m0 + lane) * fin.n_params + p];
-            const double* pr = fin.priors + 5 * p;
-            if (x != x) fin_nan = 1;
-            bool isin = (pr[1] <= x) && (x <= pr[2]);
-            double v = 0.;
-            if (pr[0] == 1.) { double t = x - pr[3]; v = -0.5 * (t * t) / (pr[4] * pr[4]); }
-            fin_lp += isin ? v : -inf;
-        }
-    }
     if (n_panels > 1) __asm__ volatile("s_waitcnt vmcnt(%0)" : : "n"(VPT) : "memory");
     else __asm__ volatile("s_waitcnt vmcnt(0)" : : : "memory");
     __builtin_amdgcn_s_barrier();
@@ -266,7 +246,7 @@
         }
     }
 #undef DL_CG_DMA_A
-    dl_chi2_gemm_finish<MT, RESID>(acc0, acc1, bj, part, M, n_tiles, fin, resid, ldr, lds, mb, nt, fin_lp, fin_nan);
+    dl_chi2_gemm_finish<MT, RESID>(acc0, acc1, bj, part, M, n_tiles, fin, resid, ldr, lds, mb, nt);
 }
 
 template <bool DO_LOAD, bool DO_MMA, int MT = DL_CG_M, bool RESID = false>
diff --git a/desilike_amd/csrc/dl_kernels.h b/desilike_amd/csrc/dl_kernels.h
--- a/desilike_amd/csrc/dl_kernels.h
+++ b/desilike_amd/csrc/dl_kernels.h
@@ -4,6 +4,7 @@
 #include <stdint.h>
 
 #include "dl_fullshape.h"
+#include "dl_prior.h"
 
 struct DlProfEvents { hipEvent_t start = nullptr, stop = nullptr; };
 extern thread_local DlProfEvents dl_prof_events;
@@ -21,6 +22,7 @@
     bool ens_global, ens_force_comm, ens_no_defer, ens_no_fold, ens_stamps, ens_fold_stamps;
     bool no_emu_fused, no_gram_epilogue, step_kernel, chi2_fused, no_chi2_big;
     bool fs_no_moments;
+    bool fs_no_prior;
     bool fs_mu_prio;
     int xcd_local;
     long long chi2_max_rows;
@@ -34,10 +36,11 @@
 #define DL_ST_NONFINITE 2
 #define DL_ST_NAN_INPUT 3
 
-void dl_launch_fullshape(const DlObsDev* obs_host, int n_obs, const double* theta, int n_params, int64_t B, double* power, int64_t ld_power, double* tables,
+bool dl_launch_fullshape(const DlObsDev* obs_host, int n_obs, const double* theta, int n_params, int64_t B, double* power, int64_t ld_power, double* tables,
                          int64_t ld_tables, hipStream_t stream, double* feat = nullptr, int64_t feat_ld = 0, int xcd_block = 0,
                          const DlObsDev* obs_dev = nullptr,
-                         bool moments = true);
+                         bool moments = true,
+                         const DlPriorRec* prior_rec = nullptr);
 void dl_launch_window_gemm(const double* A, int64_t lda, const double* Wt, int64_t ldw, const double* bias, double* C, int64_t ldc, int64_t M, int N_valid, int N_pad,
                            int K_pad, int bias_period, hipStream_t stream);
 
@@ -61,10 +64,12 @@
                         const double* priors, int64_t B, double* loglike, double* logprior, int32_t* status, int post_mode, hipStream_t stream);
 int dl_chi2_gemm_row_tile(int64_t M, int N_pad);
 void dl_launch_chi2_gemm(const double* A, int64_t lda, const double* Wt, int64_t ldw, const double* bias, double* part, int64_t M, int N_pad, int K_pad, int32_t* counters,
-                         const double* theta, int n_params, const double* priors, double* loglike, double* logprior, int32_t* status, int post_mode, hipStream_t stream,
+                         const DlPriorRec* rec, double* loglike, double* logprior, int32_t* status, int post_mode, hipStream_t stream,
                          const uint8_t* panel_ranges = nullptr, int k_live = 0, double* resid = nullptr, int64_t ldr = 0, const double* wfrag = nullptr);
 void dl_launch_finalize_part(const double* part, int n_tiles, const double* theta, int n_params, const double* priors, int64_t B, double* loglike, double* logprior,
                              int32_t* status, int post_mode, hipStream_t stream);
+void dl_launch_finalize_rec(const double* part, int n_tiles, const DlPriorRec& rec, int64_t B, double* loglike, double* logprior, int32_t* status, int post_mode,
+                            hipStream_t stream);
 #ifndef DL_FG_NM
 #define DL_FG_NM 19
 #define DL_FG_MONO_LD 20
@@ -77,7 +82,7 @@
                                 hipStream_t stream);
 size_t dl_step_lds_bytes(const DlObsDev& obs, int64_t B, int N_pad);
 void dl_launch_step(const DlObsDev& obs, const double* theta, int n_params, int64_t B, double* power, int64_t ld_power, const double* Wt, int64_t ldw, const double* bias,
-                    double* part, int K_pad, int k_live, int32_t* counters, int32_t* ready, int32_t target, const double* priors, double* loglike, double* logprior, int32_t* status,
+                    double* part, int K_pad, int k_live, int32_t* counters, int32_t* ready, int32_t target, const DlPriorRec& rec, double* loglike, double* logprior, int32_t* status,
                     int post_mode, hipStream_t stream, const uint8_t* panel_ranges);
 bool dl_emulated_stacked_ok(const DlObsDev& obs);
 struct DlGramFinalize;
diff --git a/desilike_amd/csrc/dl_kernels.hip b/desilike_amd/csrc/dl_kernels.hip
--- a/desilike_amd/csrc/dl_kernels.hip
+++ b/desilike_amd/csrc/dl_kernels.hip
@@ -44,7 +44,7 @@
     o.host_mode = std::getenv("DL_HOST_MODE") ? atoi(std::getenv("DL_HOST_MODE")) : -1;
     auto flag = [](const char* name) { const char* v = std::getenv(name); return v != nullptr && atoi(v) != 0; };
     o.no_emu_fused = on("DL_NO_EMU_FUSED"); o.no_gram_epilogue = on("DL_NO_GRAM_EPILOGUE"); o.no_chi2_big = on("DL_NO_CHI2_BIG");
-    o.fs_no_moments = flag("DL_FS_NO_MOMENTS");
+    o.fs_no_moments = flag("DL_FS_NO_MOMENTS"); o.fs_no_prior = flag("DL_FS_NO_PRIOR");
     o.fs_mu_prio = std::getenv("DL_FS_MU_PRIO") ? atoi(std::getenv("DL_FS_MU_PRIO")) != 0 : true;
     o.step_kernel = flag("DL_STEP_KERNEL"); o.chi2_fused = flag("DL_CHI2_FUSED"); o.chi2_bfrag = flag("DL_CHI2_BFRAG");
     o.xcd_local = std::getenv("DL_XCD_LOCAL") ? atoi(std::getenv("DL_XCD_LOCAL")) : 1;
@@ -68,7 +68,8 @@
 __device__ __forceinline__ void dl_fullshape_body(const DlObsDev& o, const double* __restrict__ theta, int n_params, double* __restrict__ power,
                                                   int64_t ld_power, double* __restrict__ tables, int64_t ld_tables, int stop_after, unsigned long long* __restrict__ stamps,
                                                   const double* th_row = nullptr,
-                                                  double* lds_sub = nullptr, int tid_sub = 0, int b_sub = 0) {
+                                                  double* lds_sub = nullptr, int tid_sub = 0, int b_sub = 0,
+                                                  const DlPriorRec& rec = DlPriorRec{}) {
     extern __shared__ __attribute__((aligned(16))) double lds_wg[];
     double* lds = SUB ? lds_sub : lds_wg;
     const int flags = (SUB || (stop_after & ~0xff) == 0 || stop_after < 0) ? 0 : stop_after;
@@ -87,6 +88,8 @@
     const bool direct = MOM && dl_fs_mom_direct(o);
     const double* th = TH_ROW ? th_row : theta + (size_t)b * n_params;
     if (stop_after == -1) return;
+    const bool rec_on = !TH_ROW && rec.lp != nullptr && blockIdx.y == 0, rec_late = FAST && MOM && !o.fixed_spline;
+    if (rec_on && !rec_late && __builtin_amdgcn_readfirstlane(tid >> 6) == NT / 64 - 2) dl_prior_record(rec, th, n_params, tid & 63, b);
     double lk_pref[DL_P3_PREF];
 #pragma unroll
     for (int it = 0; it < DL_P3_PREF; ++it) lk_pref[it] = (tid + it * nthr < o.n_kin) ? o.lkin[tid + it * nthr] : 0.;
@@ -130,7 +133,10 @@
             if (mu_wave) {
                 if (mu_lane) dl_fs_mu_partC(o, s, m, c, false);
                 if (scalar_lane) dl_fs_scalars(o, th, s, c, false);
-            } else if (MOM) { if (tid < 64) dl_fs_mom_fixup(tid, o, s); }
+            } else if (MOM) {
+                if (tid < 64) dl_fs_mom_fixup(tid, o, s);
+                else if (rec_on && __builtin_amdgcn_readfirstlane(tid >> 6) == 1) dl_prior_record(rec, th, n_params, tid & 63, b);
+            }
             else dl_fs_phase2d_toep(tid, KT, o, s, dlt_pref);
             __syncthreads();
             DL_STAMP(3)
@@ -189,9 +195,10 @@
 
 template <bool FAST, int NL, bool EFT, bool DENSE = false, bool MOM = false>
 __global__ __launch_bounds__(DL_FS_THREADS, DENSE ? 5 : 4) void dl_fullshape_kernel(const DlObsDev o, const double* __restrict__ theta, int n_params, double* __restrict__ power,
-                                                                     int64_t ld_power, double* __restrict__ tables, int64_t ld_tables, int stop_after, unsigned long long* __restrict__ stamps) {
+                                                                     int64_t ld_power, double* __restrict__ tables, int64_t ld_tables, int stop_after, unsigned long long* __restrict__ stamps,
+                                                                     const DlPriorRec rec) {
     dl_obs_prefetch((const void*)__builtin_amdgcn_kernarg_segment_ptr());
-    dl_fullshape_body<FAST, NL, EFT, DENSE, false, false, DL_FS_THREADS, MOM>(o, theta, n_params, power, ld_power, tables, ld_tables, stop_after, stamps);
+    dl_fullshape_body<FAST, NL, EFT, DENSE, false, false, DL_FS_THREADS, MOM>(o, theta, n_params, power, ld_power, tables, ld_tables, stop_after, stamps, nullptr, nullptr, 0, 0, rec);
 }
 
 static bool dl_fs_use_moments(const DlObsDev* obs_host, int n_obs) {
@@ -204,9 +211,9 @@
 
 template <int NL, bool MOM = false>
 __global__ __launch_bounds__(512, 2) void dl_fullshape_wide_kernel(const DlObsDev o, const double* __restrict__ theta, int n_params, double* __restrict__ power,
-                                                                 int64_t ld_power, int stop_after, unsigned long long* __restrict__ stamps) {
+                                                                 int64_t ld_power, int stop_after, unsigned long long* __restrict__ stamps, const DlPriorRec rec) {
     dl_obs_prefetch((const void*)__builtin_amdgcn_kernarg_segment_ptr());
-    dl_fullshape_body<true, NL, false, false, false, false, 512, MOM>(o, theta, n_params, power, ld_power, nullptr, 0, stop_after, stamps);
+    dl_fullshape_body<true, NL, false, false, false, false, 512, MOM>(o, theta, n_params, power, ld_power, nullptr, 0, stop_after, stamps, nullptr, nullptr, 0, 0, rec);
 }
 
 
@@ -256,8 +263,8 @@
 
 template <bool FAST, int NL, bool EFT, bool DENSE = false, bool MOM = false>
 __global__ __launch_bounds__(DL_FS_THREADS, DENSE ? 5 : 4) void dl_fullshape_multi_kernel(const DlObsDev* __restrict__ obs, const double* __restrict__ theta, int n_params,
-                                                                           double* __restrict__ power, int64_t ld_power, int stop_after) {
-    dl_fullshape_body<FAST, NL, EFT, DENSE, false, false, DL_FS_THREADS, MOM>(obs[blockIdx.y], theta, n_params, power, ld_power, nullptr, 0, stop_after, nullptr);
+                                                                           double* __restrict__ power, int64_t ld_power, int stop_after, const DlPriorRec rec) {
+    dl_fullshape_body<FAST, NL, EFT, DENSE, false, false, DL_FS_THREADS, MOM>(obs[blockIdx.y], theta, n_params, power, ld_power, nullptr, 0, stop_after, nullptr, nullptr, nullptr, 0, 0, rec);
 }
 
 #define DL_ENS_MAXP 32
@@ -603,10 +610,13 @@
     }
 }
 
-void dl_launch_fullshape(const DlObsDev* obs_host, int n_obs, const double* theta, int n_params, int64_t B, double* power, int64_t ld_power, double* tables,
-                         int64_t ld_tables, hipStream_t stream, double* feat, int64_t feat_ld, int xcd_block, const DlObsDev* obs_dev, bool moments) {
+bool dl_launch_fullshape(const DlObsDev* obs_host, int n_obs, const double* theta, int n_params, int64_t B, double* power, int64_t ld_power, double* tables,
+                         int64_t ld_tables, hipStream_t stream, double* feat, int64_t feat_ld, int xcd_block, const DlObsDev* obs_dev, bool moments, const DlPriorRec* prior_rec) {
     dl_launch_ws_templates(obs_host, n_obs, theta, n_params, B, stream);
     static const int stop_after = getenv("DL_FS_STOP") ? atoi(getenv("DL_FS_STOP")) : 0;
+    const bool rec_ok = prior_rec != nullptr && prior_rec->lp != nullptr && stop_after == 0 && obs_host[0].templ != 5;
+    const DlPriorRec rec_on = rec_ok ? *prior_rec : DlPriorRec{};
+    bool rec_written = false;
     static const char* stamp_file = getenv("DL_FS_STAMPS");
     static unsigned long long* stamps_dev = nullptr;
     static int stamp_launches = 0;
@@ -629,11 +639,11 @@
             auto launch = [&](auto kernel) {
                 if (shmem > 48 * 1024) (void)hipFuncSetAttribute((const void*)kernel, hipFuncAttributeMaxDynamicSharedMemorySize, (int)shmem);
                 const int flags = dl_fs_launch_flags((xcd_block > 0 && B % (8 * xcd_block) == 0) ? xcd_block : 0, 0);
-                DL_LAUNCH(kernel, dim3((unsigned)B, (unsigned)n_obs), dim3(DL_FS_THREADS), shmem, stream, obs_dev, theta, n_params, power, ld_power, flags);
+                DL_LAUNCH(kernel, dim3((unsigned)B, (unsigned)n_obs), dim3(DL_FS_THREADS), shmem, stream, obs_dev, theta, n_params, power, ld_power, flags, rec_on);
             };
             if (nl3) { if (dense) launch(dl_fullshape_multi_kernel<true, 3, false, true>); else if (mom) launch(dl_fullshape_multi_kernel<true, 3, false, false, true>); else launch(dl_fullshape_multi_kernel<true, 3, false>); }
             else { if (dense) launch(dl_fullshape_multi_kernel<true, 5, false, true>); else if (mom) launch(dl_fullshape_multi_kernel<true, 5, false, false, true>); else launch(dl_fullshape_multi_kernel<true, 5, false>); }
-            return;
+            return rec_ok;
         }
     }
     for (int i = 0; i < n_obs; ++i) {
@@ -679,6 +689,8 @@
             continue;
         }
         const DlObsDev& oh = obs_host[i];
+        const DlPriorRec rec = i == 0 ? rec_on : DlPriorRec{};
+        rec_written = rec_written || (i == 0 && rec_ok);
         const bool generic = tables || !oh.uniform_knots || !(oh.toeplitz || oh.fixed_spline);
         static const int64_t dense_min = getenv("DL_FS_DENSE_MIN") ? atoll(getenv("DL_FS_DENSE_MIN")) : 4096;
         bool nl3 = oh.n_ell <= 3, eft = oh.n_ct > 0 || oh.n_sn > 0;
@@ -689,7 +701,7 @@
         auto launch = [&](auto kernel) {
             if (shmem > 48 * 1024) (void)hipFuncSetAttribute((const void*)kernel, hipFuncAttributeMaxDynamicSharedMemorySize, (int)shmem);
             const int flags = dl_fs_launch_flags((xcd_block > 0 && B % (8 * xcd_block) == 0) ? xcd_block : 0, stop_after);
-            DL_LAUNCH(kernel, dim3((unsigned)B), dim3(DL_FS_THREADS), shmem, stream, obs_host[i], theta, n_params, power, ld_power, tables, ld_tables, flags, stamps);
+            DL_LAUNCH(kernel, dim3((unsigned)B), dim3(DL_FS_THREADS), shmem, stream, obs_host[i], theta, n_params, power, ld_power, tables, ld_tables, flags, stamps, rec);
             if (stamps) {
                 (void)hipStreamSynchronize(stream);
                 std::vector<unsigned long long> h((size_t)B * DL_FS_STAMP_SLOTS);
@@ -705,7 +717,7 @@
             auto launch_wide = [&](auto kernel) {
                 if (shmem > 48 * 1024) (void)hipFuncSetAttribute((const void*)kernel, hipFuncAttributeMaxDynamicSharedMemorySize, (int)shmem);
                 const int flags = dl_fs_launch_flags((xcd_block > 0 && B % (8 * xcd_block) == 0) ? xcd_block : 0, stop_after);
-                DL_LAUNCH(kernel, dim3((unsigned)B), dim3(512), shmem, stream, obs_host[i], theta, n_params, power, ld_power, flags, stamps);
+                DL_LAUNCH(kernel, dim3((unsigned)B), dim3(512), shmem, stream, obs_host[i], theta, n_params, power, ld_power, flags, stamps, rec);
             };
             if (nl3) { if (mom) launch_wide(dl_fullshape_wide_kernel<3, true>); else launch_wide(dl_fullshape_wide_kernel<3>); }
             else { if (mom) launch_wide(dl_fullshape_wide_kernel<5, true>); else launch_wide(dl_fullshape_wide_kernel<5>); }
@@ -717,6 +729,7 @@
         else if (!eft) { if (B > dense_min) launch(dl_fullshape_kernel<true, 5, false, true>); else if (mom) launch(dl_fullshape_kernel<true, 5, false, false, true>); else launch(dl_fullshape_kernel<true, 5, false>); }
         else launch(dl_fullshape_kernel<true, 5, true>);
     }
+    return rec_written;
 }
 
 typedef double dl_double4 __attribute__((ext_vector_type(4)));
@@ -1110,8 +1123,9 @@
 }
 
 void dl_launch_chi2_gemm(const double* A, int64_t lda, const double* Wt, int64_t ldw, const double* bias, double* part, int64_t M, int N_pad, int K_pad, int32_t* counters,
-                         const double* theta, int n_params, const double* priors, double* loglike, double* logprior, int32_t* status, int post_mode, hipStream_t stream,
+                         const DlPriorRec* rec, double* loglike, double* logprior, int32_t* status, int post_mode, hipStream_t stream,
                          const uint8_t* panel_ranges, int k_live, double* resid, int64_t ldr, const double* wfrag) {
+    if (rec == nullptr || rec->lp == nullptr) counters = nullptr;
     const int n_tiles = N_pad / DL_CG_N;
     const int mt = counters == nullptr ? dl_chi2_gemm_row_tile(M, N_pad) : DL_CG_M;
     const int64_t mblocks = (M + mt - 1) / mt;
@@ -1125,8 +1139,8 @@
         optin = true;
     }
     DlChi2Fin fin;
-    fin.counters = counters; fin.theta = theta; fin.priors = priors; fin.loglike = loglike; fin.logprior = logprior; fin.status = status;
-    fin.n_params = n_params; fin.post_mode = post_mode; fin.ready = nullptr;
+    fin.counters = counters; fin.lp_rec = counters ? rec->lp : nullptr; fin.flag_rec = counters ? rec->flag : nullptr; fin.loglike = loglike; fin.logprior = logprior; fin.status = status;
+    fin.post_mode = post_mode; fin.ready = nullptr;
     static const char* stamp_file = getenv("DL_CG_STAMPS");
     static unsigned long long* stamps_dev = nullptr;
     static int stamp_launches = 0;
@@ -1172,14 +1186,14 @@
 template <int NL>
 __global__ __launch_bounds__(1024) void dl_step_kernel(const DlObsDev o, const double* __restrict__ theta, int n_params, double* __restrict__ power, int64_t ld_power,
                                                        const double* __restrict__ Wt, int64_t ldw, const double* __restrict__ bias, double* __restrict__ part, int M, int K_pad,
-                                                       DlChi2Fin fin, DlChi2Panels panels, int k_live, int32_t* __restrict__ ready, int32_t target, int lds_per_point) {
+                                                       DlChi2Fin fin, DlChi2Panels panels, int k_live, int32_t* __restrict__ ready, int32_t target, int lds_per_point, const DlPriorRec rec) {
     extern __shared__ __attribute__((aligned(16))) double lds[];
     const int L = blockIdx.x, xcd = L & 7, j = L >> 3;
     const int q = j >> 3, c = j & 7, mb = xcd + 8 * q;
     const int sub = threadIdx.x >> 8, tid = threadIdx.x & 255;
     unsigned long long* st = fin.stamps != nullptr ? fin.stamps + (size_t)blockIdx.x * 8 : nullptr;
     if (st != nullptr && threadIdx.x == 0) { st[0] = __builtin_amdgcn_s_memtime(); st[6] = __builtin_amdgcn_s_memrealtime(); }
-    dl_fullshape_body<true, NL, false, false, false, true>(o, theta, n_params, power, ld_power, nullptr, 0, 0, nullptr, nullptr, lds + (size_t)sub * lds_per_point, tid, 32 * mb + 4 * c + sub);
+    dl_fullshape_body<true, NL, false, false, false, true>(o, theta, n_params, power, ld_power, nullptr, 0, 0, nullptr, nullptr, lds + (size_t)sub * lds_per_point, tid, 32 * mb + 4 * c + sub, rec);
     if (st != nullptr && threadIdx.x == 0) st[1] = __builtin_amdgcn_s_memtime();
     __asm__ volatile("s_waitcnt vmcnt(0)" : : : "memory");
     __syncthreads();
@@ -1210,7 +1224,7 @@
 }
 
 void dl_launch_step(const DlObsDev& oh, const double* theta, int n_params, int64_t B, double* power, int64_t ld_power, const double* Wt, int64_t ldw, const double* bias,
-                    double* part, int K_pad, int k_live, int32_t* counters, int32_t* ready, int32_t target, const double* priors, double* loglike, double* logprior, int32_t* status,
+                    double* part, int K_pad, int k_live, int32_t* counters, int32_t* ready, int32_t target, const DlPriorRec& rec, double* loglike, double* logprior, int32_t* status,
                     int post_mode, hipStream_t stream, const uint8_t* panel_ranges) {
     DlChi2Panels panels;
     std::memset(&panels, 0, sizeof(panels));
@@ -1220,8 +1234,8 @@
     static bool optin = false;
     if (!optin) { (void)hipFuncSetAttribute((const void*)dl_step_kernel<3>, hipFuncAttributeMaxDynamicSharedMemorySize, 160 * 1024); optin = true; }
     DlChi2Fin fin;
-    fin.counters = counters; fin.theta = theta; fin.priors = priors; fin.loglike = loglike; fin.logprior = logprior; fin.status = status;
-    fin.n_params = n_params; fin.post_mode = post_mode; fin.ready = ready;
+    fin.counters = counters; fin.lp_rec = rec.lp; fin.flag_rec = rec.flag; fin.loglike = loglike; fin.logprior = logprior; fin.status = status;
+    fin.post_mode = post_mode; fin.ready = ready;
     const unsigned grid = (unsigned)(B / 4);
     static const char* stamp_file = getenv("DL_STEP_STAMPS");
     static unsigned long long* stamps_dev = nullptr;
@@ -1231,7 +1245,7 @@
     if (stamp_file) stamp_launches++;
     if (fin.stamps) (void)hipMemsetAsync(fin.stamps, 0, (size_t)256 * 8 * sizeof(unsigned long long), stream);
     DL_LAUNCH(dl_step_kernel<3>, dim3(grid), dim3(1024), shm, stream, oh, theta, n_params, power, ld_power, Wt, ldw, bias, part, (int)B, K_pad, fin, panels, k_live > 0 ? k_live : K_pad,
-              ready, target, (int)per_point);
+              ready, target, (int)per_point, rec);
     if (fin.stamps) {
         (void)hipStreamSynchronize(stream);
         std::vector<unsigned long long> h((size_t)grid * 8);
@@ -1277,6 +1291,28 @@
     const size_t shm = (size_t)5 * n_params * sizeof(double);
     if (shm > 48 * 1024) (void)hipFuncSetAttribute((const void*)dl_finalize_part_kernel, hipFuncAttributeMaxDynamicSharedMemorySize, (int)shm);
     DL_LAUNCH(dl_finalize_part_kernel, dim3((unsigned)((B + 63) / 64)), dim3(64), shm, stream, part, n_tiles, theta, n_params, priors, B, loglike, logprior, status, post_mode);
+}
+
+__global__ __launch_bounds__(64) void dl_finalize_rec_kernel(const double* __restrict__ part, int n_tiles, const double* __restrict__ lp_rec, const int32_t* __restrict__ flag_rec,
+                                                              int64_t B, double* __restrict__ loglike, double* __restrict__ logprior, int32_t* __restrict__ status, int post_mode) {
+    dl_kernarg_prefetch<96>();
+    const int64_t b = (int64_t)blockIdx.x * 64 + threadIdx.x;
+    if (b >= B) return;
+    const double lp = lp_rec[b];
+    const int fl = flag_rec[b];
+    const double chi2 = dl_chi2_of_parts(part + (size_t)b * n_tiles, n_tiles);
+    const double inf = __builtin_huge_val();
+    double ll;
+    int st;
+    dl_finalize_status(chi2, lp, fl == DL_ST_NAN_INPUT, ll, st);
+    if (loglike) loglike[b] = post_mode ? (st == DL_ST_OK ? ll + lp : -inf) : ll;
+    if (logprior) logprior[b] = lp;
+    if (status) status[b] = st;
+}
+
+void dl_launch_finalize_rec(const double* part, int n_tiles, const DlPriorRec& rec, int64_t B, double* loglike, double* logprior, int32_t* status, int post_mode,
+                            hipStream_t stream) {
+    DL_LAUNCH(dl_finalize_rec_kernel, dim3((unsigned)((B + 63) / 64)), dim3(64), 0, stream, part, n_tiles, (const double*)rec.lp, (const int32_t*)rec.flag, B, loglike, logprior, status, post_mode);
 }
 
 __device__ __forceinline__ double dl_readlane(double v, int l) {
diff --git a/desilike_amd/csrc/dl_prior.h b/desilike_amd/csrc/dl_prior.h
--- a/desilike_amd/csrc/dl_prior.h
+++ b/desilike_amd/csrc/dl_prior.h
@@ -1,5 +1,6 @@
 #pragma once
 #include <hip/hip_runtime.h>
+#include <stdint.h>
 
 #define DL_PRIOR_MAX_KIND 9
 
@@ -27,3 +28,32 @@
     else if (kind >= 2.) v = dl_prior_family((int)kind, (x - loc) / scale);
     return isin ? v : -inf;
 }
+
+struct DlPriorRec {
+    const double* priors = nullptr;
+    double* lp = nullptr;
+    int32_t* flag = nullptr;
+};
+
+__device__ __forceinline__ void dl_prior_record(const DlPriorRec& rec, const double* __restrict__ th, int n_params, int lane, int64_t b) {
+    const double inf = __builtin_huge_val();
+    double lp = 0.;
+    bool nan_in = false;
+    for (int p0 = 0; p0 < n_params; p0 += 64) {
+        const bool live = p0 + lane < n_params;
+        const int p = live ? p0 + lane : n_params - 1;
+        double pr[5];
+#pragma unroll
+        for (int c = 0; c < 5; ++c) pr[c] = rec.priors[5 * p + c];
+        const double x = th[p];
+        const double v = dl_prior_logpdf(pr, x);
+        nan_in = nan_in || __ballot(live && x != x) != 0;
+        const int n = n_params - p0 < 64 ? n_params - p0 : 64;
+        const int v_lo = __double2loint(v), v_hi = __double2hiint(v);
+        for (int q = 0; q < n; ++q) lp += __hiloint2double(__builtin_amdgcn_readlane(v_hi, q), __builtin_amdgcn_readlane(v_lo, q));
+    }
+    if (lane == 0) {
+        __hip_atomic_store(rec.lp + b, lp, __ATOMIC_RELAXED, __HIP_MEMORY_SCOPE_AGENT);
+        __hip_atomic_store(rec.flag + b, nan_in ? 3 : (lp == -inf ? 1 : 0), __ATOMIC_RELAXED, __HIP_MEMORY_SCOPE_AGENT);
+    }
+}
```

After: 46.05 million evals/s (median of 6 runs). 1.02x the previous value.
